# Fabri000/Maze-Solving-Agent-Gymnasium

Hardware: AMD Instinct MI355X
Metric: env steps/sec (whole node) + DQN win-rate, 40x40 r-prim mazes (higher is better)
Workload: dtype int32

## Files before the change

include/mazerl.h:

```cpp
#ifndef MAZERL_H
#define MAZERL_H
#include <stdint.h>

#ifdef __cplusplus
extern "C" {
#endif

#define MZ_OK 0
#define MZ_EINVAL (-1)
#define MZ_EINVAL_SHAPE (-2)
#define MZ_EHIP (-3)
#define MZ_ENOMEM (-4)
#define MZ_EALIGN (-5)

#define MZ_MAX_DIM 127
#define MZ_BANK_MAX_DIMS 64
#define MZ_MAX_CANDIDATES 64
#define MZ_WINDOW 15
#define MZ_WINDOW_BITS 675
#define MZ_WINDOW_WORDS 22

#define MZ_ALGO_RPRIM 0
#define MZ_ALGO_DFS 1
#define MZ_ALGO_PRIMKILL 2

typedef struct mz_handle mz_handle;

typedef struct {
  int32_t num_envs;
  int32_t max_dim;
  int32_t toroidal;
  int32_t enrich;
  int32_t device;
  int32_t reserved[7];
} mz_config;

typedef struct {
  float* reward;
  double* reward64;
  uint8_t* terminated;
  uint8_t* truncated;
  int32_t* pos;
  int32_t* best_dir;
  float* obs6;
  uint32_t* window_bits;
  float* window;
  int32_t* done_idx;
  int32_t* done_count;
} mz_step_out;

typedef struct {
  int32_t n, start_r, start_c, goal_r, goal_c, max_steps;
  int32_t r, c, steps, invalid_streak, nmoves, last_action, done;
} mz_env_info;

const char* mz_last_error(void);
int mz_device_count(int* n);

int mz_create(const mz_config* cfg, mz_handle** out);
int mz_destroy(mz_handle* h);

int mz_load_mazes(mz_handle* h, const uint8_t* grids_host, int32_t dim,
                  const int32_t* start_goal_host, const int32_t* env_ids_host, int32_t n,
                  void* stream);

int mz_generate(mz_handle* h, const int32_t* env_ids_dev, int32_t n, const uint8_t* algo_dev,
                int32_t algo_all, int32_t dim, uint64_t seed, void* stream);

int mz_generate_best(mz_handle* h, const int32_t* env_ids_dev, int32_t n, const uint8_t* algo_dev,
                     int32_t algo_all, int32_t dim, uint64_t seed, int32_t candidates,
                     void* stream);
int mz_select_stats(mz_handle* h, int32_t* out3_dev, int32_t reset, void* stream);
#define MZ_SELECT_STATS 5
int mz_select_stats_ex(mz_handle* h, int32_t* out_dev, int32_t n, int32_t reset, void* stream);
int mz_set_debug(mz_handle* h, int32_t flags);
int mz_set_regen_dims(mz_handle* h, const uint8_t* dims_dev);

#define MZ_RNG_PHILOX 0
#define MZ_RNG_CPYTHON 1
int mz_generate_ex(mz_handle* h, const int32_t* env_ids_dev, int32_t n, const uint8_t* algo_dev,
                   int32_t algo_all, int32_t dim, uint64_t seed, int32_t rng, void* stream);

int mz_generate_state(mz_handle* h, int32_t env, int32_t dim, int32_t algo, uint32_t* state_host,
                      void* stream);

int mz_reset_all(mz_handle* h, const mz_step_out* out, void* stream);
int mz_reset_list(mz_handle* h, const int32_t* idx_dev, const int32_t* count_dev,
                  int32_t max_count, int32_t regen_won, uint64_t seed, uint32_t epoch,
                  const mz_step_out* out, void* stream);

int mz_reset_done(mz_handle* h, int32_t regen_won, uint64_t seed, uint32_t epoch,
                  const mz_step_out* out, void* stream);

int mz_step(mz_handle* h, const int32_t* actions_dev, const mz_step_out* out, void* stream);

#define MZ_STEP_COUNT_ZEROED 1
#define MZ_STEP_AUTORESET 2
int mz_step_ex(mz_handle* h, const int32_t* actions_dev, const mz_step_out* out, int32_t flags,
               void* stream);

int mz_step_act(mz_handle* h, const float* eps_dev, float eps_all, const int64_t* greedy_dev,
                uint64_t seed, uint64_t counter, int32_t* actions_out_dev, const mz_step_out* out,
                int32_t flags, void* stream);

int mz_direction_mask(mz_handle* h, int32_t probs, float* out4_dev, void* stream);

int mz_act(mz_handle* h, const float* eps_dev, float eps_all, const int64_t* greedy_dev,
           uint64_t seed, uint64_t counter, int32_t* actions_dev, void* stream);

int mz_expand_window(const uint32_t* bits_dev, float* out_dev, int32_t n, void* stream);

int mz_bank_create(mz_handle* h, int32_t slots, int32_t dim, uint32_t algo_mask);
int mz_bank_create_dims(mz_handle* h, int32_t slots, const int32_t* dims, int32_t ndims,
                        uint32_t algo_mask);
int mz_bank_create_ex(mz_handle* h, int32_t slots, const int32_t* dims, int32_t ndims,
                      uint32_t algo_mask, int32_t candidates);
int mz_bank_fill(mz_handle* h, int32_t bank, uint64_t seed, void* stream);
int mz_bank_slot_grid(mz_handle* h, int32_t bank, int32_t algo, int32_t size_index, int32_t slot,
                      uint8_t* grid_host, int32_t* info4_host);
int mz_bank_use(mz_handle* h, int32_t bank);
int mz_bank_consumed(mz_handle* h, int32_t bank, int32_t* out3_dev, void* stream);

#define MZ_STATE_HEADER_BYTES 256
int mz_state_bytes(mz_handle* h, uint64_t* bytes_out);
int mz_state_save(mz_handle* h, void* dst_dev, uint64_t bytes, void* stream);
int mz_state_load(mz_handle* h, const void* src_dev, uint64_t bytes, void* stream);

int mz_q_front(const uint32_t* bits_dev, const float* obs6_dev, int32_t n, const float* conv_w_dev,
               const float* conv_b_dev, float drop_p, uint64_t seed, uint64_t counter,
               uint16_t* feat_dev, int32_t ld, void* stream);

int mz_q_front_rows(const uint32_t* bits_dev, const float* obs6_dev, const int32_t* rows_dev,
                    const int32_t* count_dev, int32_t n, const float* conv_w_dev,
                    const float* conv_b_dev, float drop_p, uint64_t seed, uint64_t counter,
                    uint16_t* feat_dev, int32_t ld, void* stream);

int mz_greedy_rows(const float* eps_dev, float eps_all, uint64_t seed, uint64_t counter, int32_t n,
                   int32_t* scratch_dev, int32_t* rows_dev, int32_t* count_dev,
                   int32_t* count_host, void* stream);

int mz_stem_forward(const uint32_t* bits_dev, const float* obs6_dev, int32_t n,
                    const float* conv_w_dev, const float* conv_b_dev, float drop_p,
                    const uint64_t* rng_dev, uint32_t salt, float* feat_dev, int32_t ld,
                    uint8_t* code_dev, void* stream);
int mz_stem_backward(const uint32_t* bits_dev, const uint8_t* code_dev, const float* gfeat_dev,
                     int32_t ld, int32_t n, float drop_p, float* partial_dev, float* dw_dev,
                     float* db_dev, void* stream);
int mz_stem_backward_ex(const uint32_t* bits_dev, const uint8_t* code_dev, const float* gfeat_dev,
                        int32_t ld, int32_t n, float drop_p, float* partial_dev, float* dw_dev,
                        float* db_dev, uint64_t* rng_advance_dev, void* stream);
int mz_stem_workspace_floats(int32_t n);

int mz_leaky_relu_bf16(uint16_t* x_dev, int64_t n, float slope, void* stream);

int mz_colsum_f32(const float* g_dev, int32_t n, int32_t m, int32_t ld, float* out_dev,
                  void* stream);

int mz_replay_gather(const int64_t* idx_dev, int32_t b, int64_t capacity,
                     const float* s6_dev, const int32_t* sw_dev, const int64_t* a_dev,
                     const float* r_dev, const float* s6n_dev, const int32_t* swn_dev,
                     float* out_s6_dev,
                     int32_t* out_sw_dev, int64_t* out_a_dev, float* out_r_dev, void* stream);

int mz_pair_surrogate(const float* lp_new_dev, const float* lp_old_dev, const float* adv_dev,
                      int32_t b, float clip, float* part_dev, float* dsum_dev, void* stream);

int mz_adamw_flat(float* param_dev, float* exp_avg_dev, float* exp_avg_sq_dev,
                  const float* const* grads_dev, const int64_t* seg_len, int32_t nseg,
                  const float* lr_dev, float* step_dev, double beta1, double beta2, double eps,
                  double weight_decay, float clamp, float grad_scale, int32_t write_grad,
                  void* stream);

int mz_set_algorithm(mz_handle* h, const uint8_t* algo_dev, int32_t algo_all, void* stream);

int mz_get_meta(mz_handle* h, int32_t* meta_dev, void* stream);

int mz_discounted_returns(const double* rew_dev, int32_t ld, const int32_t* rows_dev,
                          const int32_t* lens_dev, int32_t n, double gamma, float* out_dev,
                          int32_t ldo, void* stream);

int mz_difficulty(const uint8_t* grid_host, int32_t h, int32_t w, int32_t sr, int32_t sc,
                  int32_t gr, int32_t gc, double* out_host);

int mz_maze_complexity(const uint8_t* grid_host, int32_t h, int32_t w, int32_t sr, int32_t sc,
                       int32_t gr, int32_t gc, double* difficulty_out, double* complexity_out);

int mz_difficulty_batch(mz_handle* h, const int32_t* env_ids_dev, int32_t n, double* out_dev,
                        int32_t* status_dev, void* stream);
int mz_screen_batch(mz_handle* h, const int32_t* env_ids_dev, int32_t n, double* out_dev,
                    int32_t* status_dev, void* stream);

int mz_maze_metrics(mz_handle* h, const int32_t* env_ids_dev, int32_t n, double* out_dev,
                    void* stream);

int mz_query(mz_handle* h, int32_t env, mz_env_info* info_host);
int mz_get_grid(mz_handle* h, int32_t env, uint8_t* grid_host );

int mz_host_alloc(uint64_t bytes, int32_t device, void** host_out, void** dev_out);
int mz_host_free(void* host);


int mz_trainer_tick(const uint8_t* term_dev, const uint8_t* trunc_dev, float* steps_done_dev,
                    double eps_start, double eps_final, double eps_decay, float* eps_out_dev,
                    int64_t* wins_dev, int64_t* episodes_dev, uint64_t seed, uint64_t counter,
                    int32_t n, int32_t* scratch_dev, int32_t* rows_dev, int32_t* count_dev,
                    void* stream);

int mz_greedy_scatter(const uint16_t* q_dev, int32_t ldq, const int32_t* rows_dev,
                      const int32_t* count_dev, int32_t m, int64_t* greedy_dev, void* stream);

int mz_head_bf16(const float* w0, const float* b0, const float* w1, const float* b1,
                 const float* w2, const float* b2, int32_t out0, int32_t in0, int32_t out1,
                 int32_t in1, int32_t out2, int32_t in2, int32_t ld0, int32_t conv_out,
                 int32_t conv_ch, uint16_t* dw0, uint16_t* db0, uint16_t* dw1, uint16_t* db1,
                 uint16_t* dw2, uint16_t* db2, void* stream);

int mz_replay_push(int32_t n, int64_t capacity, int64_t ptr, const float* obs6_src,
                   const int32_t* bits_src, const int32_t* act_src, const float* rew_src,
                   const float* obs6n_src, const int32_t* bitsn_src, float* s6_dev,
                   int32_t* sw_dev, int64_t* a_dev, float* r_dev, float* s6n_dev,
                   int32_t* swn_dev, int32_t obs_dim, int32_t window_words, void* stream);

int mz_replay_sample_idx(uint64_t seed, uint64_t counter, int64_t newest, int64_t n_avail,
                         int64_t capacity, int64_t* out_dev, int32_t n, void* stream);

int mz_q_loss(const float* q_dev, int32_t ldq, const float* q_next_dev, int32_t ldn,
              const float* q_tgt_dev, int32_t ldt, const int64_t* action_dev,
              const float* reward_dev, double gamma, int32_t b, float* loss_dev, float* diff_dev,
              void* stream);

int mz_q_loss_backward(const float* grad_dev, const float* diff_dev, const int64_t* action_dev,
                       int32_t b, int32_t rows, float* dq_dev, void* stream);

int mz_head_loss_workspace_floats(int32_t b);
int mz_head_loss(const float* z2s_dev, int32_t lds, const float* w3s_dev, const float* b3s_dev,
                 const float* z2t_dev, int32_t ldt, const float* w3t_dev, const float* b3t_dev,
                 int32_t hidden, int32_t act, int32_t stacked, const int64_t* action_dev,
                 const float* reward_dev, double gamma, int32_t b, float* part_dev,
                 uint32_t* ticket_dev, float* loss_dev, float* diff_dev, void* stream);

int mz_head_loss_backward_workspace_floats(int32_t b, int32_t hidden);
int mz_head_loss_backward(const float* grad_dev, const float* diff_dev, const int64_t* action_dev,
                          int32_t b, const float* z2s_dev, int32_t lds, const float* w3s_dev,
                          int32_t hidden, int32_t act, float* dz2_dev, int32_t ldd,
                          float* part_dev, void* stream);

int mz_adamw_groups(float* param_dev, float* exp_avg_dev, float* exp_avg_sq_dev,
                    const float* const* grads_dev, const int64_t* seg_len,
                    const int32_t* seg_group, int32_t nseg, const float* lr_dev, float* step_dev,
                    double beta1, double beta2, double eps, double weight_decay, float max_norm,
                    float* scratch_dev, void* stream);


int mz_ppo_act(const float* logits_dev, int32_t ldl, const float* value_dev, int32_t ldv,
               const float* obs6_dev, const uint32_t* bits_dev, int32_t B, int32_t L, uint64_t seed,
               uint64_t counter, const int32_t* t_dev, float* rec_s6_dev, uint32_t* rec_w_dev,
               int64_t* rec_a_dev, float* rec_lp_dev, float* rec_v_dev, int32_t* act_out_dev,
               void* stream);

int mz_ppo_scan(const double* reward64_dev, const uint8_t* term_dev, const uint8_t* trunc_dev,
                int32_t B, int32_t L, int32_t* t_dev, double* rec_r_dev, int32_t* fin_id_dev,
                int64_t* fin_off_dev, int32_t* fin_len_dev, int32_t* fin_count_dev,
                int64_t* pool_fill_dev, int64_t* pool_total_dev, int64_t* stats_dev,
                void* stream);

int mz_ppo_finish(const double* rec_r_dev, const float* rec_s6_dev, const uint32_t* rec_w_dev,
                  const int64_t* rec_a_dev, const float* rec_lp_dev, const float* rec_v_dev,
                  int32_t B, int32_t L, const int32_t* fin_id_dev, const int64_t* fin_off_dev,
                  const int32_t* fin_len_dev, const int32_t* fin_count_dev, double gamma,
                  int64_t capacity, float* pool_s6_dev, uint32_t* pool_w_dev, int64_t* pool_a_dev,
                  float* pool_lp_dev, float* pool_adv_dev, float* pool_ret_dev, void* stream);

int mz_ppo_head_loss(const float* logits_dev, int32_t ldl, const float* value_dev, int32_t ldv,
                     const int64_t* action_dev, const float* lp_old_dev, const float* adv_dev,
                     const float* ret_dev, const float* coef_dev, int32_t b, float clip,
                     float* scratch_dev, float* loss_dev, float* dlogits_dev, int32_t ldg,
                     float* dvalue_dev, int32_t ldvg, void* stream);


int mz_rf_act(const float* logits_dev, int32_t ldl, float temperature, const float* obs6_dev,
              const uint32_t* bits_dev, int32_t B, int32_t L, uint64_t seed, uint64_t counter,
              const int32_t* t_dev, float* rec_s6_dev, uint32_t* rec_w_dev, int64_t* rec_a_dev,
              int32_t* act_out_dev, void* stream);

int mz_rf_finish(const double* rec_r_dev, const float* rec_s6_dev, const uint32_t* rec_w_dev,
                 const int64_t* rec_a_dev, int32_t B, int32_t L, const int32_t* fin_id_dev,
                 const int64_t* fin_off_dev, const int32_t* fin_len_dev,
                 const int32_t* fin_count_dev, double gamma, int64_t capacity, float* pool_s6_dev,
                 uint32_t* pool_w_dev, int64_t* pool_a_dev, float* pool_adv_dev,
                 int32_t* pool_len_dev, int32_t* episodes_dev, void* stream);

int mz_rf_head_loss(const float* logits_dev, int32_t ldl, const int64_t* action_dev,
                    const float* adv_dev, const int32_t* len_dev, const int32_t* episodes_dev,
                    int32_t b, float temperature, float entropy_coef, float* loss_dev,
                    float* dlogits_dev, int32_t ldg, void* stream);


int mz_drqn_act(const float* const* params_dev, int32_t hidden, const float* obs6_dev, int32_t B,
                int32_t L, float epsilon, int32_t explore_actions, uint64_t seed, uint64_t counter,
                const int32_t* t_dev, float* h_dev, float* c_dev, float* rec_x_dev,
                int32_t* rec_a_dev, int32_t* act_out_dev, float* q_out_dev, void* stream);

int mz_drqn_store(const float* obs6_dev, const uint8_t* term_dev, int32_t B, int32_t L,
                  const int32_t* fin_id_dev, const int32_t* fin_len_dev,
                  const int32_t* fin_count_dev, float* rec_x_dev, const int32_t* rec_a_dev,
                  const double* rec_r_dev, int64_t capacity, uint32_t* mem_dev,
                  int32_t* mem_len_dev, int32_t* mem_term_dev, int64_t* ring_dev, void* stream);

int mz_drqn_sample(uint64_t seed, uint64_t counter, int32_t E, int32_t L, int64_t capacity,
                   int64_t filled, const int64_t* ring_dev, const int32_t* mem_len_dev,
                   int32_t* dir_slot_dev, int32_t* dir_len_dev, int64_t* dir_off_dev,
                   int64_t* dir_tot_dev, void* stream);

int mz_drqn_seq_forward(const float* const* params_dev, int32_t hidden, int32_t target, int32_t E,
                        int32_t L, int64_t capacity, float gamma, const uint32_t* mem_dev,
                        const int32_t* mem_term_dev, const int32_t* dir_slot_dev,
                        const int32_t* dir_len_dev, const int64_t* dir_off_dev,
                        const int64_t* dir_tot_dev, float* qmax_dev, float* stash_dev,
                        float* qa_dev, float* y_dev, float* d_dev, double* ep_loss_dev,
                        void* stream);

int mz_drqn_seq_backward(const float* const* params_dev, int32_t hidden, int32_t E, int32_t L,
                         int64_t capacity, const uint32_t* mem_dev, const int32_t* dir_slot_dev,
                         const int32_t* dir_len_dev, const int64_t* dir_off_dev,
                         const int64_t* dir_tot_dev, const float* stash_dev, const float* d_dev,
                         const double* ep_loss_dev, float* gpart_dev, float* const* grads_dev,
                         float* loss_dev, void* stream);


int mz_qact_prepare(const float* fc1_w_dev, const float* fc2_w_dev, uint16_t* w1_hi_dev,
                    uint16_t* w1_lo_dev, uint16_t* w2_hi_dev, uint16_t* w2_lo_dev, void* stream);

int64_t mz_qact_workspace_floats(int32_t n);
int mz_qact(const uint32_t* bits_dev, const float* obs6_dev, const int32_t* rows_dev,
            const int32_t* count_dev, int32_t n, const float* conv_w_dev, const float* conv_b_dev,
            const uint16_t* w1_hi_dev, const uint16_t* w1_lo_dev, const float* b1_dev,
            const uint16_t* w2_hi_dev, const uint16_t* w2_lo_dev, const float* b2_dev,
            const float* w3_dev, const float* b3_dev, int32_t relu, float drop_p, uint64_t seed,
            uint64_t counter, float* h1_dev, int64_t* greedy_dev, float* q_out_dev, void* stream);


int mz_qtab_states(int32_t max_dim, int64_t* rows);

int mz_qtab_act(const float* obs6_dev, int32_t n, int32_t max_dim, const int32_t* table_of_dev,
                int32_t ntables, const uint8_t* active_dev, const double* q_dev,
                int64_t* steps_done_dev, const double* eps_init_dev, const double* eps_final_dev,
                const double* eps_decay_dev, uint64_t seed, uint64_t counter, int32_t* actions_dev,
                int64_t* sidx_dev, void* stream);

int mz_qtab_update(const float* obs6_dev, int32_t n, int32_t max_dim, const int32_t* table_of_dev,
                   int32_t ntables, double* q_dev, const int64_t* sidx_dev,
                   const int32_t* actions_dev, const double* reward64_dev,
                   const uint8_t* terminated_dev, const uint8_t* truncated_dev, double* gamma_dev,
                   const double* lr_dev, const double* eta_dev, double* cum_dev,
                   int64_t* episodes_dev, int64_t* wins_dev, double* td_dev, int32_t episode_end,
                   void* stream);


int mz_qtab_hash_act(const float* obs6_dev, int32_t n, int32_t max_dim,
                     const int32_t* table_of_dev, int32_t ntables, const uint8_t* active_dev,
                     const int32_t* keys_dev, const double* vals_dev, int64_t capacity,
                     int64_t* steps_done_dev, const double* eps_init_dev,
                     const double* eps_final_dev, const double* eps_decay_dev, uint64_t seed,
                     uint64_t counter, int32_t* actions_dev, int64_t* sidx_dev, void* stream);

int mz_qtab_hash_update(const float* obs6_dev, int32_t n, int32_t max_dim,
                        const int32_t* table_of_dev, int32_t ntables, int32_t* keys_dev,
                        double* vals_dev, int64_t capacity, int32_t* load_dev,
                        int64_t* overflow_dev, const int64_t* sidx_dev, const int32_t* actions_dev,
                        const double* reward64_dev, const uint8_t* terminated_dev,
                        const uint8_t* truncated_dev, double* gamma_dev, const double* lr_dev,
                        const double* eta_dev, double* cum_dev, int64_t* episodes_dev,
                        int64_t* wins_dev, double* td_dev, int32_t episode_end, void* stream);

// ... 80 lines not shown
```

maze-solving-agent-gymnasium_amd/csrc/mz_api.hip:

```cpp
#include <algorithm>
#include <cmath>
#include <cstdarg>
#include <cstdio>
#include <cstdlib>
#include <cstring>
#include <string>
#include <vector>

#include "../../include/mazerl.h"
#include "mz_archive.h"
#include "mz_common.h"
#include "mz_learner.h"
#include "mz_mcclendon.h"

struct MzHostFallback {
  int cap = 0, gstride = 0;
  uint8_t *grid_h = nullptr, *grid_d = nullptr;
  int32_t *info_h = nullptr, *info_d = nullptr;
  double *prod_h = nullptr, *prod_d = nullptr;
  int32_t *ok_h = nullptr, *ok_d = nullptr;
  int32_t* count_h = nullptr;
  int* count_d = nullptr;
  int32_t* map = nullptr;
};
// ... 735 lines not shown
  }
  b.epoch[bank] += 1;
  return MZ_OK;
}

int mz_bank_use(mz_handle* h, int32_t bank) {
  if (!h) return fail(MZ_EINVAL, "null handle");
  MzDev& d = h->d;
  if (bank < 0) {
    d.bk_K = 0;
    return MZ_OK;
  }
  const MzBankStore& b = h->bank;
  if (!b.K) return fail(MZ_EINVAL, "no maze bank (mz_bank_create)");
  if (bank > 1) return fail(MZ_EINVAL, "bank %d", bank);
  const size_t blk = (size_t)bank * b.nA * b.nD * b.K, P = (size_t)d.P;
  d.bk_K = b.K;
  d.bk_nd = b.nD;
  for (int i = 0; i < 128; ++i) d.bk_didx[i] = -1;
  for (int i = 0; i < b.nD; ++i) d.bk_didx[b.dims[i]] = (int8_t)i;
  d.bk_amask = b.amask;
  d.bk_cells = b.cells + blk * P * P;
  d.bk_planes = b.planes + blk * d.PW;
  d.bk_meta0 = b.meta0 + blk;
  d.bk_meta1 = b.meta1 + blk;
  d.bk_head = b.heads + 3 * bank * b.nD;
  d.bk_slot = b.slot;
  d.bk_code = b.code;
  d.bk_G = (d.B + 63) / 64;
  return MZ_OK;
}

int mz_bank_slot_grid(mz_handle* h, int32_t bank, int32_t algo, int32_t size_index, int32_t slot,
                      uint8_t* grid_host, int32_t* info4_host) {
  if (!h || !h->bank.K || !grid_host || !info4_host) return fail(MZ_EINVAL, "bad arguments");
  const MzBankStore& b = h->bank;
  if (bank < 0 || bank > 1 || algo < 0 || algo > 2 || !((b.amask >> algo) & 1u) ||
      size_index < 0 || size_index >= b.nD || slot < 0 || slot >= b.K)
    return fail(MZ_EINVAL, "no such bank slot");
  DeviceGuard g(h->cfg.device);
  MZ_HIP(hipDeviceSynchronize());
  const size_t P = (size_t)h->d.P;
  const size_t i = (((size_t)bank * b.nA + mz_bank_aidx(b.amask, algo)) * b.nD + size_index) * b.K + slot;
  uint32_t m0, m1;
  MZ_HIP(hipMemcpy(&m0, b.meta0 + i, 4, hipMemcpyDeviceToHost));
  MZ_HIP(hipMemcpy(&m1, b.meta1 + i, 4, hipMemcpyDeviceToHost));
  std::vector<uint32_t> cw(P * P);
  MZ_HIP(hipMemcpy(cw.data(), b.cells + i * P * P, 4 * cw.size(), hipMemcpyDeviceToHost));
  const int N = m0 & 0xFF, gr = m1 & 0xFF, gc = (m1 >> 8) & 0xFF;
  if (N < 5 || N > (int)P) return fail(MZ_EINVAL, "bank slot not built");
  for (int r = 0; r < N; ++r)
    for (int c = 0; c < N; ++c) {
      const bool open = (cw[(size_t)r * P + c] & MZ_CELL_OPEN) != 0;
      grid_host[r * N + c] = !open ? 0 : ((r == gr && c == gc) ? 2 : 1);
    }
  info4_host[0] = (m0 >> 16) & 0xFF;
  info4_host[1] = m0 >> 24;
  info4_host[2] = gr;
  info4_host[3] = gc;
  return MZ_OK;
}

int mz_set_regen_dims(mz_handle* h, const uint8_t* dims_dev) {
  if (!h) return fail(MZ_EINVAL, "null handle");
  h->d.regen_dim = dims_dev;
  return MZ_OK;
}

int mz_generate_best(mz_handle* h, const int32_t* env_ids_dev, int32_t n, const uint8_t* algo_dev,
                     int32_t algo_all, int32_t dim, uint64_t seed, int32_t candidates,
                     void* stream) {
  if (!h) return fail(MZ_EINVAL, "null handle");
  if (candidates < 1 || candidates > MZ_MAX_CANDIDATES)
    return fail(MZ_EINVAL, "candidates %d outside [1, %d]", candidates, MZ_MAX_CANDIDATES);
  if (candidates == 1)
    return mz_generate_ex(h, env_ids_dev, n, algo_dev, algo_all, dim, seed, MZ_RNG_PHILOX, stream);
  if (!env_ids_dev) n = h->d.B;
  if (n < 0 || n > h->d.B) return fail(MZ_EINVAL, "n out of range");
  if (!algo_dev && (algo_all < 0 || algo_all > 2)) return fail(MZ_EINVAL, "algorithm id %d", algo_all);
  int rc = check_dim(h, dim);
  if (rc) return rc;
  int mm = 0;
  if (mz_mcclendon_lds(h->d.P, h->d.toroidal != 0, &mm) > 160 * 1024)
    return fail(MZ_EINVAL_SHAPE, "best-of-%d generation scores with the difficulty kernel: maze "
                "pitch %d beyond its LDS plan", candidates, h->d.P);
  if (n == 0) return MZ_OK;
  DeviceGuard g(h->cfg.device);
  hipStream_t s = static_cast<hipStream_t>(stream);
  const int chunk = std::max(1, std::min(n, 49152 / candidates));
  if (h->gen.cap < chunk * candidates) {
    if (h->gen.cap) MZ_HIP(hipStreamSynchronize(s));
    if ((rc = cand_alloc(h, h->gen, chunk * candidates))) return rc;
  }
  for (int j0 = 0; j0 < n; j0 += chunk) {
    const int m = std::min(chunk, n - j0);
    const int32_t* ids = env_ids_dev ? env_ids_dev + j0 : nullptr;
    const uint8_t* al = algo_dev ? algo_dev + j0 : nullptr;
    if ((rc = bestof_run(h, h->gen, h->d, ids, j0, nullptr, m, candidates, al, algo_all, dim, seed,
                         0u, s)))
      return rc;
  }
  return MZ_OK;
}

int mz_select_stats(mz_handle* h, int32_t* out3_dev, int32_t reset, void* stream) {
  return mz_select_stats_ex(h, out3_dev, 3, reset, stream);
}

int mz_select_stats_ex(mz_handle* h, int32_t* out_dev, int32_t n, int32_t reset, void* stream) {
  if (!h || n < 0 || n > MZ_SELECT_STATS) return fail(MZ_EINVAL, "bad arguments");
  DeviceGuard g(h->cfg.device);
  hipStream_t s = static_cast<hipStream_t>(stream);
  if (out_dev && n) MZ_HIP(hipMemcpyAsync(out_dev, h->sel_stats, n * sizeof(int32_t), hipMemcpyDeviceToDevice, s));
  if (reset) MZ_HIP(hipMemsetAsync(h->sel_stats, 0, 8 * sizeof(int32_t), s));
  return MZ_OK;
}

int mz_set_debug(mz_handle* h, int32_t flags) {
  if (!h) return fail(MZ_EINVAL, "null handle");
  if (flags & ~7) return fail(MZ_EINVAL, "debug flags %d", flags);
  h->dbg = flags;
  return MZ_OK;
}

int mz_screen_batch(mz_handle* h, const int32_t* env_ids_dev, int32_t n, double* out_dev,
                    int32_t* status_dev, void* stream) {
  if (!h || !out_dev || !status_dev) return fail(MZ_EINVAL, "bad arguments");
  if (h->d.toroidal) return fail(MZ_EINVAL, "the screen scores euclidean mazes");
  if (!env_ids_dev) n = h->d.B;
  if (n < 0 || (!env_ids_dev && n > h->d.B)) return fail(MZ_EINVAL, "n out of range");
  if (n == 0) return MZ_OK;
  DeviceGuard g(h->cfg.device);
  hipStream_t s = static_cast<hipStream_t>(stream);
  if (h->scr_cap < n) {
    if (h->scr_cap) MZ_HIP(hipStreamSynchronize(s));
    int rc = compact_alloc(h, h->scr, n);
    if (rc) return rc;
    h->scr_cap = n;
  }
  MZ_HIP(mz_launch_compact_from_handle(h->d, env_ids_dev, n, h->scr, s));
  MZ_HIP(mz_launch_screen(h->scr, h->d.P, n, out_dev, status_dev, s));
  return MZ_OK;
}

int mz_bank_consumed(mz_handle* h, int32_t bank, int32_t* out3_dev, void* stream) {
  if (!h || !h->bank.K || !out3_dev || bank < 0 || bank > 1) return fail(MZ_EINVAL, "bad arguments");
  DeviceGuard g(h->cfg.device);
  const int nd = h->bank.nD;
  MZ_HIP(hipMemcpyAsync(out3_dev, h->bank.heads + 3 * bank * nd, 3 * nd * sizeof(int32_t),
                        hipMemcpyDeviceToDevice, static_cast<hipStream_t>(stream)));
  return MZ_OK;
}

}

namespace {

constexpr uint32_t kStateMagic = 0x54535A4Du;
constexpr uint32_t kStateVersion = 1u;
enum : int { SH_MAGIC, SH_VER, SH_B, SH_P, SH_TOR, SH_ENRICH, SH_NS, SH_PW, SH_BK_K, SH_BK_NA,
             SH_BK_ND, SH_BK_AMASK, SH_BK_ACTIVE, SH_BK_EPOCH0, SH_BK_EPOCH1, SH_DIMS = 16 };
static_assert(SH_DIMS * 4 + MZ_BANK_MAX_DIMS <= MZ_STATE_HEADER_BYTES, "header too small");

struct Section {
  void* p;
  size_t bytes;
};

std::vector<Section> state_sections(mz_handle* h) {
  const MzDev& d = h->d;
  const size_t B = (size_t)d.B, P = (size_t)d.P;
  std::vector<Section> s = {
      {d.cells, B * P * P * 4}, {d.planes, (B * (size_t)d.PW + 16) * 4}, {d.meta0, B * 4},
      {d.meta1, B * 4}, {d.posw, B * 4}, {d.stw, B * 4}, {d.curw, B * 4}, {d.algo, B},
      {d.last_term, B}};
  const MzBankStore& b = h->bank;
  if (b.K) {
    const size_t S = 2 * (size_t)b.nA * b.nD * b.K;
    s.push_back({b.cells, S * P * P * 4});
    s.push_back({b.planes, S * (size_t)d.PW * 4});
    s.push_back({b.meta0, S * 4});
    s.push_back({b.meta1, S * 4});
    s.push_back({b.heads, (size_t)6 * b.nD * 4});
  }
  return s;
}

size_t state_size(mz_handle* h) {
  size_t n = MZ_STATE_HEADER_BYTES;
  for (const Section& s : state_sections(h)) n += (s.bytes + 255) & ~(size_t)255;
  return n;
}

int active_bank(const mz_handle* h) {
  const MzDev& d = h->d;
  if (!d.bk_K || !h->bank.K) return -1;
  return d.bk_cells == h->bank.cells ? 0 : 1;
}

}

extern "C" {

int mz_state_bytes(mz_handle* h, uint64_t* bytes_out) {
  if (!h || !bytes_out) return fail(MZ_EINVAL, "bad arguments");
  *bytes_out = state_size(h);
  return MZ_OK;
}

int mz_state_save(mz_handle* h, void* dst_dev, uint64_t bytes, void* stream) {
  if (!h || !dst_dev) return fail(MZ_EINVAL, "bad arguments");
  if (bytes < state_size(h)) return fail(MZ_EINVAL, "state buffer of %llu bytes, %zu needed",
                                         (unsigned long long)bytes, state_size(h));
  DeviceGuard g(h->cfg.device);
  hipStream_t s = static_cast<hipStream_t>(stream);
  const MzDev& d = h->d;
  const MzBankStore& b = h->bank;
  uint32_t hdr[MZ_STATE_HEADER_BYTES / 4] = {};
  hdr[SH_MAGIC] = kStateMagic;
  hdr[SH_VER] = kStateVersion;
  hdr[SH_B] = (uint32_t)d.B;
  hdr[SH_P] = (uint32_t)d.P;
  hdr[SH_TOR] = (uint32_t)d.toroidal;
  hdr[SH_ENRICH] = (uint32_t)d.enrich;
  hdr[SH_NS] = (uint32_t)d.NS;
  hdr[SH_PW] = (uint32_t)d.PW;
  hdr[SH_BK_K] = (uint32_t)b.K;
  hdr[SH_BK_NA] = (uint32_t)b.nA;
  hdr[SH_BK_ND] = (uint32_t)b.nD;
  hdr[SH_BK_AMASK] = b.amask;
  hdr[SH_BK_ACTIVE] = (uint32_t)active_bank(h);
  hdr[SH_BK_EPOCH0] = b.epoch[0];
  hdr[SH_BK_EPOCH1] = b.epoch[1];
  uint8_t* dims = reinterpret_cast<uint8_t*>(hdr + SH_DIMS);
  for (int i = 0; i < b.nD; ++i) dims[i] = (uint8_t)b.dims[i];
  uint8_t* dst = static_cast<uint8_t*>(dst_dev);
  MZ_HIP(hipMemcpyAsync(dst, hdr, sizeof hdr, hipMemcpyHostToDevice, s));
  MZ_HIP(hipStreamSynchronize(s));
  size_t off = MZ_STATE_HEADER_BYTES;
  for (const Section& sec : state_sections(h)) {
    MZ_HIP(hipMemcpyAsync(dst + off, sec.p, sec.bytes, hipMemcpyDeviceToDevice, s));
    off += (sec.bytes + 255) & ~(size_t)255;
  }
  return MZ_OK;
}

int mz_state_load(mz_handle* h, const void* src_dev, uint64_t bytes, void* stream) {
  if (!h || !src_dev) return fail(MZ_EINVAL, "bad arguments");
  if (bytes < MZ_STATE_HEADER_BYTES) return fail(MZ_EINVAL, "state buffer too small");
  DeviceGuard g(h->cfg.device);
  hipStream_t s = static_cast<hipStream_t>(stream);
  uint32_t hdr[MZ_STATE_HEADER_BYTES / 4];
  MZ_HIP(hipMemcpyAsync(hdr, src_dev, sizeof hdr, hipMemcpyDeviceToHost, s));
  MZ_HIP(hipStreamSynchronize(s));
  const MzDev& d = h->d;
  MzBankStore& b = h->bank;
  if (hdr[SH_MAGIC] != kStateMagic || hdr[SH_VER] != kStateVersion)
    return fail(MZ_EINVAL, "not an env state (magic %08x version %u)", hdr[SH_MAGIC], hdr[SH_VER]);
  if (hdr[SH_B] != (uint32_t)d.B || hdr[SH_P] != (uint32_t)d.P ||
      hdr[SH_TOR] != (uint32_t)d.toroidal || hdr[SH_ENRICH] != (uint32_t)d.enrich ||
      hdr[SH_NS] != (uint32_t)d.NS || hdr[SH_PW] != (uint32_t)d.PW)
    return fail(MZ_EINVAL, "env state of %u instances, max_dim %u, toroidal %u, enrich %u does not "
                "fit this handle (%d, %d, %d, %d)", hdr[SH_B], hdr[SH_P], hdr[SH_TOR],
                hdr[SH_ENRICH], d.B, d.P, d.toroidal, d.enrich);
  const uint8_t* dims = reinterpret_cast<const uint8_t*>(hdr + SH_DIMS);
  bool same_bank = hdr[SH_BK_K] == (uint32_t)b.K && hdr[SH_BK_NA] == (uint32_t)b.nA &&
                   hdr[SH_BK_ND] == (uint32_t)b.nD && hdr[SH_BK_AMASK] == b.amask;
  for (int i = 0; same_bank && i < b.nD; ++i) same_bank = dims[i] == (uint8_t)b.dims[i];
  if (!same_bank)
    return fail(MZ_EINVAL, "env state has a maze bank of %u slots x %u algorithms x %u sizes "
                "(mask %u); this handle's is %d x %d x %d (mask %u)", hdr[SH_BK_K], hdr[SH_BK_NA],
                hdr[SH_BK_ND], hdr[SH_BK_AMASK], b.K, b.nA, b.nD, b.amask);
  if (bytes < state_size(h)) return fail(MZ_EINVAL, "state buffer of %llu bytes, %zu needed",
                                         (unsigned long long)bytes, state_size(h));
  const uint8_t* src = static_cast<const uint8_t*>(src_dev);
  size_t off = MZ_STATE_HEADER_BYTES;
  for (const Section& sec : state_sections(h)) {
    MZ_HIP(hipMemcpyAsync(sec.p, src + off, sec.bytes, hipMemcpyDeviceToDevice, s));
    off += (sec.bytes + 255) & ~(size_t)255;
  }
  if (b.K) {
    b.epoch[0] = hdr[SH_BK_EPOCH0];
    b.epoch[1] = hdr[SH_BK_EPOCH1];
  }
  return mz_bank_use(h, (int32_t)hdr[SH_BK_ACTIVE]);
}

int mz_maze_metrics(mz_handle* h, const int32_t* env_ids_dev, int32_t n, double* out_dev,
                    void* stream) {
  if (!h || !out_dev) return fail(MZ_EINVAL, "bad arguments");
  if (h->d.toroidal) return fail(MZ_EINVAL, "maze metrics are defined for euclidean mazes");
  if (!env_ids_dev) n = h->d.B;
  if (n < 0 || n > h->d.B) return fail(MZ_EINVAL, "n out of range");
  DeviceGuard g(h->cfg.device);
  MZ_HIP(mz_launch_metrics(h->d, env_ids_dev, n, out_dev, static_cast<hipStream_t>(stream)));
  return MZ_OK;
}

int mz_difficulty_batch(mz_handle* h, const int32_t* env_ids_dev, int32_t n, double* out_dev,
                        int32_t* status_dev, void* stream) {
  if (!h || !out_dev || !status_dev) return fail(MZ_EINVAL, "bad arguments");
  if (!env_ids_dev) n = h->d.B;
  if (n < 0 || (!env_ids_dev && n > h->d.B)) return fail(MZ_EINVAL, "n out of range");
  int mm = 0;
  if (mz_mcclendon_lds(h->d.P, h->d.toroidal != 0, &mm) > 160 * 1024)
    return fail(MZ_EINVAL_SHAPE, "maze pitch beyond the difficulty kernel's LDS plan");
// ... 7 lines not shown
  if (!h) return fail(MZ_EINVAL, "null handle");
  DeviceGuard g(h->cfg.device);
  hipStream_t s = static_cast<hipStream_t>(stream);
  if (algo_dev) MZ_HIP(hipMemcpyAsync(h->d.algo, algo_dev, h->d.B, hipMemcpyDeviceToDevice, s));
  else {
    if (algo_all < 0 || algo_all > 2) return fail(MZ_EINVAL, "algorithm id %d", algo_all);
    MZ_HIP(hipMemsetAsync(h->d.algo, algo_all, h->d.B, s));
  }
  return MZ_OK;
}

int mz_get_meta(mz_handle* h, int32_t* meta_dev, void* stream) {
  if (!h || !meta_dev) return fail(MZ_EINVAL, "bad arguments");
  DeviceGuard g(h->cfg.device);
  MZ_HIP(mz_launch_meta(h->d, meta_dev, static_cast<hipStream_t>(stream)));
  return MZ_OK;
}

int mz_discounted_returns(const double* rew_dev, int32_t ld, const int32_t* rows_dev,
                          const int32_t* lens_dev, int32_t n, double gamma, float* out_dev,
                          int32_t ldo, void* stream) {
  if (!rew_dev || !rows_dev || !lens_dev || !out_dev || n < 0) return fail(MZ_EINVAL, "bad arguments");
  StreamGuard g(stream);
  MZ_HIP(mz_launch_returns(rew_dev, ld, rows_dev, lens_dev, n, gamma, out_dev, ldo,
                           static_cast<hipStream_t>(stream)));
  return MZ_OK;
}

int mz_query(mz_handle* h, int32_t env, mz_env_info* info) {
  if (!h || !info || env < 0 || env >= h->d.B) return fail(MZ_EINVAL, "bad arguments");
  DeviceGuard g(h->cfg.device);
  MZ_HIP(hipDeviceSynchronize());
  uint32_t m0, m1, pw, sw;
  MZ_HIP(hipMemcpy(&m0, h->d.meta0 + env, 4, hipMemcpyDeviceToHost));
  MZ_HIP(hipMemcpy(&m1, h->d.meta1 + env, 4, hipMemcpyDeviceToHost));
  MZ_HIP(hipMemcpy(&pw, h->d.posw + env, 4, hipMemcpyDeviceToHost));
  MZ_HIP(hipMemcpy(&sw, h->d.stw + env, 4, hipMemcpyDeviceToHost));
  info->n = m0 & 0xFF;
  info->start_r = (m0 >> 16) & 0xFF; info->start_c = m0 >> 24;
  info->goal_r = m1 & 0xFF; info->goal_c = (m1 >> 8) & 0xFF; info->max_steps = m1 >> 16;
  info->r = pw & 0xFF; info->c = (pw >> 8) & 0xFF; info->nmoves = (pw >> 16) & 3;
  info->last_action = (pw >> 18) & 3; info->done = (pw >> 20) & 1;
  info->steps = sw & 0xFFFF; info->invalid_streak = (sw >> 16) & 0xFF;
  return MZ_OK;
}

int mz_get_grid(mz_handle* h, int32_t env, uint8_t* grid_host) {
  if (!h || !grid_host || env < 0 || env >= h->d.B) return fail(MZ_EINVAL, "bad arguments");
  mz_env_info info;
  int rc = mz_query(h, env, &info);
  if (rc) return rc;
  const int P = h->d.P, N = info.n;
  std::vector<uint32_t> cw((size_t)P * P);
  DeviceGuard g(h->cfg.device);
  MZ_HIP(hipMemcpy(cw.data(), h->d.cells + (size_t)env * P * P, 4 * cw.size(), hipMemcpyDeviceToHost));
  for (int r = 0; r < N; ++r)
    for (int c = 0; c < N; ++c) {
      const bool open = (cw[(size_t)r * P + c] & MZ_CELL_OPEN) != 0;
      grid_host[r * N + c] = !open ? 0 : ((r == info.goal_r && c == info.goal_c) ? 2 : 1);
    }
  return MZ_OK;
}

int mz_host_alloc(uint64_t bytes, int32_t device, void** host_out, void** dev_out) {
  if (!host_out || !dev_out || bytes == 0) return fail(MZ_EINVAL, "bad arguments");
  int ndev = 0;
  MZ_HIP(hipGetDeviceCount(&ndev));
  if (device < 0 || device >= ndev) return fail(MZ_EINVAL, "device %d not present", device);
  DeviceGuard g(device);
  void* hp = nullptr;
  MZ_HIP(hipHostMalloc(&hp, (size_t)bytes, hipHostMallocMapped | hipHostMallocCoherent));
  void* dp = nullptr;
  const hipError_t e = hipHostGetDevicePointer(&dp, hp, 0);
  if (e != hipSuccess) {
    (void)hipHostFree(hp);
    return fail(MZ_EHIP, "hipHostGetDevicePointer: %s", hipGetErrorString(e));
  }
  std::memset(hp, 0, (size_t)bytes);
  *host_out = hp;
  *dev_out = dp;
  return MZ_OK;
}

int mz_host_free(void* host) {
  if (!host) return MZ_OK;
  MZ_HIP(hipHostFree(host));
  return MZ_OK;
}

}


int mz_trainer_tick(const uint8_t* term_dev, const uint8_t* trunc_dev, float* steps_done_dev,
                    double eps_start, double eps_final, double eps_decay, float* eps_out_dev,
                    int64_t* wins_dev, int64_t* episodes_dev, uint64_t seed, uint64_t counter,
                    int32_t n, int32_t* scratch_dev, int32_t* rows_dev, int32_t* count_dev,
                    void* stream) {
  if (n < 0 || (n > 0 && (!term_dev || !trunc_dev || !steps_done_dev || !eps_out_dev ||
                          !scratch_dev || !rows_dev || !count_dev)))
    return fail(MZ_EINVAL, "bad arguments");
  if (!(eps_decay > 0.0)) return fail(MZ_EINVAL, "eps_decay %g", eps_decay);
  const float inv_decay = 1.0f / (float)eps_decay;
  MZ_HIP(mz_launch_tick(term_dev, trunc_dev, steps_done_dev, (float)eps_final,
                        (float)(eps_start - eps_final), inv_decay, eps_out_dev,
                        reinterpret_cast<unsigned long long*>(wins_dev),
                        reinterpret_cast<unsigned long long*>(episodes_dev), seed, counter, n,
                        scratch_dev, rows_dev, count_dev, static_cast<hipStream_t>(stream)));
  return MZ_OK;
}

int mz_greedy_scatter(const uint16_t* q_dev, int32_t ldq, const int32_t* rows_dev,
                      const int32_t* count_dev, int32_t m, int64_t* greedy_dev, void* stream) {
  if (m < 0 || ldq < 4 || (m > 0 && (!q_dev || !rows_dev || !count_dev || !greedy_dev)))
    return fail(MZ_EINVAL, "bad arguments");
  MZ_HIP(mz_launch_greedy_scatter(q_dev, ldq, rows_dev, count_dev, m, greedy_dev,
                                  static_cast<hipStream_t>(stream)));
  return MZ_OK;
}

int mz_head_bf16(const float* w0, const float* b0, const float* w1, const float* b1,
                 const float* w2, const float* b2, int32_t out0, int32_t in0, int32_t out1,
                 int32_t in1, int32_t out2, int32_t in2, int32_t ld0, int32_t conv_out,
                 int32_t conv_ch, uint16_t* dw0, uint16_t* db0, uint16_t* dw1, uint16_t* db1,
                 uint16_t* dw2, uint16_t* db2, void* stream) {
  if (!w0 || !b0 || !w1 || !b1 || !w2 || !b2 || !dw0 || !db0 || !dw1 || !db1 || !dw2 || !db2)
    return fail(MZ_EINVAL, "bad arguments");
  if (out0 <= 0 || out1 <= 0 || out2 <= 0 || in1 != out0 || in2 != out1 || in0 > ld0 ||
      conv_ch <= 0 || conv_out < 0 || conv_out > in0 || conv_out % conv_ch != 0 || in0 > 2048)
    return fail(MZ_EINVAL, "head shapes");
  MzHeadBf16 h{{w0, w1, w2}, {b0, b1, b2}, {dw0, dw1, dw2}, {db0, db1, db2},
               {out0, out1, out2}, {in0, in1, in2}, ld0, conv_out, conv_ch};
  MZ_HIP(mz_launch_head_bf16(h, static_cast<hipStream_t>(stream)));
  return MZ_OK;
}

int mz_replay_push(int32_t n, int64_t capacity, int64_t ptr, const float* obs6_src,
                   const int32_t* bits_src, const int32_t* act_src, const float* rew_src,
                   const float* obs6n_src, const int32_t* bitsn_src, float* s6_dev,
                   int32_t* sw_dev, int64_t* a_dev, float* r_dev, float* s6n_dev,
                   int32_t* swn_dev, int32_t obs_dim, int32_t window_words, void* stream) {
  if (n < 0 || n > capacity || ptr < 0 || ptr >= capacity || obs_dim <= 0 || window_words <= 0)
    return fail(MZ_EINVAL, "bad arguments");
  const void* src[6] = {obs6_src, bits_src, act_src, rew_src, obs6n_src, bitsn_src};
  void* dst[6] = {s6_dev, sw_dev, a_dev, r_dev, s6n_dev, swn_dev};
  for (int j = 0; j < 6; ++j)
    if (src[j] && !dst[j]) return fail(MZ_EINVAL, "replay array %d missing", j);
  MzReplayPush p{{src[0], src[1], src[2], src[3], src[4], src[5]},
                 {dst[0], dst[1], dst[2], dst[3], dst[4], dst[5]},
                 {obs_dim, window_words, 1, 1, obs_dim, window_words}, n, capacity, ptr};
  MZ_HIP(mz_launch_replay_push(p, static_cast<hipStream_t>(stream)));
  return MZ_OK;
}

int mz_replay_sample_idx(uint64_t seed, uint64_t counter, int64_t newest, int64_t n_avail,
                         int64_t capacity, int64_t* out_dev, int32_t n, void* stream) {
  if (n < 0 || capacity <= 0 || n_avail <= 0 || n_avail > capacity || (n > 0 && !out_dev))
    return fail(MZ_EINVAL, "bad arguments");
  MZ_HIP(mz_launch_replay_idx(seed, counter, newest, n_avail, capacity, out_dev, n,
                              static_cast<hipStream_t>(stream)));
  return MZ_OK;
}

int mz_q_loss(const float* q_dev, int32_t ldq, const float* q_next_dev, int32_t ldn,
              const float* q_tgt_dev, int32_t ldt, const int64_t* action_dev,
              const float* reward_dev, double gamma, int32_t b, float* loss_dev, float* diff_dev,
              void* stream) {
  if (b <= 0 || !q_dev || !q_tgt_dev || !action_dev || !reward_dev || !loss_dev || !diff_dev ||
      ldq < 4 || ldt < 4 || (q_next_dev && ldn < 4))
    return fail(MZ_EINVAL, "bad arguments");
  MZ_HIP(mz_launch_q_loss(q_dev, ldq, q_next_dev, ldn, q_tgt_dev, ldt, action_dev, reward_dev,
                          (float)gamma, b, loss_dev, diff_dev, static_cast<hipStream_t>(stream)));
  return MZ_OK;
}

int mz_q_loss_backward(const float* grad_dev, const float* diff_dev, const int64_t* action_dev,
                       int32_t b, int32_t rows, float* dq_dev, void* stream) {
  if (b <= 0 || rows < b || !grad_dev || !diff_dev || !action_dev || !dq_dev)
    return fail(MZ_EINVAL, "bad arguments");
  const float norm = (float)(2.0 / (double)b);
  MZ_HIP(mz_launch_q_loss_bwd(grad_dev, diff_dev, action_dev, b, rows, norm, dq_dev,
                              static_cast<hipStream_t>(stream)));
  return MZ_OK;
}

int mz_head_loss_workspace_floats(int32_t b) {
  return b <= 0 ? 0 : mz_head_loss_blocks(b);
}

int mz_head_loss(const float* z2s_dev, int32_t lds, const float* w3s_dev, const float* b3s_dev,
                 const float* z2t_dev, int32_t ldt, const float* w3t_dev, const float* b3t_dev,
                 int32_t hidden, int32_t act, int32_t stacked, const int64_t* action_dev,
                 const float* reward_dev, double gamma, int32_t b, float* part_dev,
                 uint32_t* ticket_dev, float* loss_dev, float* diff_dev, void* stream) {
  if (b <= 0 || hidden <= 0 || hidden % 4 || (act != 0 && act != 1) || !z2s_dev || !w3s_dev ||
      !b3s_dev || !z2t_dev || !w3t_dev || !b3t_dev || !action_dev || !reward_dev || !part_dev ||
      !loss_dev || !diff_dev || lds < hidden || ldt < hidden)
    return fail(MZ_EINVAL, "bad arguments");
  MzHeadLoss p{z2s_dev, w3s_dev, b3s_dev, z2t_dev, w3t_dev, b3t_dev, lds, ldt, stacked ? 1 : 0, b,
               hidden, act, action_dev, reward_dev, (float)gamma, part_dev, ticket_dev, loss_dev,
               diff_dev};
  MZ_HIP(mz_launch_head_loss(p, static_cast<hipStream_t>(stream)));
  return MZ_OK;
}

int mz_head_loss_backward_workspace_floats(int32_t b, int32_t hidden) {
  return b <= 0 ? 0 : mz_head_loss_bwd_blocks(b) * (4 * hidden + 4);
}

int mz_head_loss_backward(const float* grad_dev, const float* diff_dev, const int64_t* action_dev,
                          int32_t b, const float* z2s_dev, int32_t lds, const float* w3s_dev,
                          int32_t hidden, int32_t act, float* dz2_dev, int32_t ldd,
                          float* part_dev, void* stream) {
  if (b <= 0 || hidden <= 0 || hidden % 4 || (act != 0 && act != 1) || !grad_dev || !diff_dev ||
      !action_dev || !z2s_dev || !w3s_dev || !dz2_dev || !part_dev || lds < hidden || ldd < hidden)
    return fail(MZ_EINVAL, "bad arguments");
  const float norm = (float)(2.0 / (double)b);
  MZ_HIP(mz_launch_head_loss_bwd(grad_dev, diff_dev, action_dev, b, norm, z2s_dev, lds, w3s_dev,
                                 hidden, act, dz2_dev, ldd, part_dev,
                                 static_cast<hipStream_t>(stream)));
  return MZ_OK;
}

int mz_adamw_groups(float* param_dev, float* exp_avg_dev, float* exp_avg_sq_dev,
                    const float* const* grads_dev, const int64_t* seg_len,
                    const int32_t* seg_group, int32_t nseg, const float* lr_dev, float* step_dev,
                    double beta1, double beta2, double eps, double weight_decay, float max_norm,
                    float* scratch_dev, void* stream) {
  if (!param_dev || !exp_avg_dev || !exp_avg_sq_dev || !grads_dev || !seg_len || !seg_group ||
      !lr_dev || !step_dev || !scratch_dev)
    return fail(MZ_EINVAL, "bad arguments");
  if (nseg < 1 || nseg > MZ_OPT_MAX_SEGS) return fail(MZ_EINVAL, "segment count %d", nseg);
  const uintptr_t al = reinterpret_cast<uintptr_t>(param_dev) |
                       reinterpret_cast<uintptr_t>(exp_avg_dev) |
                       reinterpret_cast<uintptr_t>(exp_avg_sq_dev);
  if (al & 15) return fail(MZ_EALIGN, "flat buffers must be 16-byte aligned");
  for (int k = 0; k < nseg; ++k) {
    if (!grads_dev[k] || seg_len[k] <= 0 || (seg_len[k] & 3))
      return fail(MZ_EINVAL, "segment %d: length %lld (multiple of 4 required)", k,
                  (long long)seg_len[k]);
    if (reinterpret_cast<uintptr_t>(grads_dev[k]) & 15)
      return fail(MZ_EALIGN, "gradient %d must be 16-byte aligned", k);
    if (seg_group[k] < 0) return fail(MZ_EINVAL, "segment %d: group %d", k, seg_group[k]);
  }
  MZ_HIP(mz_launch_adamw_groups(param_dev, exp_avg_dev, exp_avg_sq_dev, grads_dev, seg_len,
                                seg_group, nseg, lr_dev, step_dev, beta1, beta2, eps,
                                weight_decay, max_norm, scratch_dev,
                                static_cast<hipStream_t>(stream)));
  return MZ_OK;
}

int mz_ppo_act(const float* logits_dev, int32_t ldl, const float* value_dev, int32_t ldv,
               const float* obs6_dev, const uint32_t* bits_dev, int32_t B, int32_t L, uint64_t seed,
               uint64_t counter, const int32_t* t_dev, float* rec_s6_dev, uint32_t* rec_w_dev,
               int64_t* rec_a_dev, float* rec_lp_dev, float* rec_v_dev, int32_t* act_out_dev,
               void* stream) {
  if (!logits_dev || !value_dev || !obs6_dev || !bits_dev || !t_dev || !rec_s6_dev || !rec_w_dev ||
      !rec_a_dev || !rec_lp_dev || !rec_v_dev || !act_out_dev || B < 0 || L < 1 || ldl < 4 ||
      ldv < 1)
    return fail(MZ_EINVAL, "bad arguments");
  StreamGuard g(stream);
  MzPpoAct q{logits_dev, ldl, value_dev, ldv, obs6_dev, bits_dev, B, L, seed, counter, t_dev,
             rec_s6_dev, rec_w_dev, rec_a_dev, rec_lp_dev, rec_v_dev, act_out_dev};
  MZ_HIP(mz_launch_ppo_act(q, static_cast<hipStream_t>(stream)));
  return MZ_OK;
}

int mz_ppo_scan(const double* reward64_dev, const uint8_t* term_dev, const uint8_t* trunc_dev,
                int32_t B, int32_t L, int32_t* t_dev, double* rec_r_dev, int32_t* fin_id_dev,
                int64_t* fin_off_dev, int32_t* fin_len_dev, int32_t* fin_count_dev,
                int64_t* pool_fill_dev, int64_t* pool_total_dev, int64_t* stats_dev,
                void* stream) {
  if (!reward64_dev || !term_dev || !trunc_dev || !t_dev || !rec_r_dev || !fin_id_dev ||
      !fin_off_dev || !fin_len_dev || !fin_count_dev || !pool_fill_dev || !pool_total_dev ||
      !stats_dev || B < 0 || L < 1)
    return fail(MZ_EINVAL, "bad arguments");
  StreamGuard g(stream);
  MzPpoScan q{reward64_dev, term_dev, trunc_dev, B, L, t_dev, rec_r_dev, fin_id_dev, fin_off_dev,
              fin_len_dev, fin_count_dev, pool_fill_dev, pool_total_dev,
              reinterpret_cast<long long*>(stats_dev)};
  MZ_HIP(mz_launch_ppo_scan(q, static_cast<hipStream_t>(stream)));
  return MZ_OK;
}

int mz_ppo_finish(const double* rec_r_dev, const float* rec_s6_dev, const uint32_t* rec_w_dev,
                  const int64_t* rec_a_dev, const float* rec_lp_dev, const float* rec_v_dev,
                  int32_t B, int32_t L, const int32_t* fin_id_dev, const int64_t* fin_off_dev,
                  const int32_t* fin_len_dev, const int32_t* fin_count_dev, double gamma,
                  int64_t capacity, float* pool_s6_dev, uint32_t* pool_w_dev, int64_t* pool_a_dev,
                  float* pool_lp_dev, float* pool_adv_dev, float* pool_ret_dev, void* stream) {
  if (!rec_r_dev || !rec_s6_dev || !rec_w_dev || !rec_a_dev || !rec_lp_dev || !rec_v_dev ||
      !fin_id_dev || !fin_off_dev || !fin_len_dev || !fin_count_dev || !pool_s6_dev ||
      !pool_w_dev || !pool_a_dev || !pool_lp_dev || !pool_adv_dev || !pool_ret_dev || B < 0 ||
      L < 1 || capacity < 0)
    return fail(MZ_EINVAL, "bad arguments");
  StreamGuard g(stream);
  MzPpoFinish q{rec_r_dev, rec_s6_dev, rec_w_dev, rec_a_dev, rec_lp_dev, rec_v_dev, L, fin_id_dev,
                fin_off_dev, fin_len_dev, fin_count_dev, gamma, capacity, pool_s6_dev, pool_w_dev,
                pool_a_dev, pool_lp_dev, pool_adv_dev, pool_ret_dev};
  MZ_HIP(mz_launch_ppo_finish(q, B, static_cast<hipStream_t>(stream)));
  return MZ_OK;
}

int mz_ppo_head_loss(const float* logits_dev, int32_t ldl, const float* value_dev, int32_t ldv,
                     const int64_t* action_dev, const float* lp_old_dev, const float* adv_dev,
                     const float* ret_dev, const float* coef_dev, int32_t b, float clip,
                     float* scratch_dev, float* loss_dev, float* dlogits_dev, int32_t ldg,
// ... 577 lines not shown
```

maze-solving-agent-gymnasium_amd/csrc/mz_env.hip:

```cpp
#include "mz_common.h"
#include "mz_kernels.h"
#include "mz_build.inc.h"

#include "../../include/mazerl.h"

#define WAVE 64
#ifndef MZ_IPW
#define MZ_IPW 16
#endif
#define IPW MZ_IPW
#ifndef MZ_SPW
#define MZ_SPW 1
#endif
#ifndef MZ_PROBE
#define MZ_PROBE 0
#endif
__host__ __device__ constexpr int cat_words(int ipw) { return ipw * 675 / 32 + 2; }

namespace {

__device__ inline uint32_t wrap_colmask(int col, int C0, int N) {
  uint32_t m = 0;
  for (int j = mz_wrapn(col - C0, N); j < 15; j += N) m |= 1u << j;
  return m;
// ... 755 lines not shown
  const int lane = threadIdx.x;
  for (int t = blockIdx.x; t < used * C; t += gridDim.x) {
    const bool decl = status[t] != 0 || ((dbg & MZ_DBG_DECLINE_EVEN) && ((t % C) & 1) == 0);
    if (!decl) {
      if (lane == 0) hmap[t] = -1;
      continue;
    }
    int slot = 0;
    if (lane == 0) slot = atomicAdd(hcount, 1);
    slot = __shfl(slot, 0);
    if (lane == 0) hmap[t] = slot < hcap ? slot : -1;
    if (slot >= hcap) continue;
    const bool tor = cd.toroidal;
    const int P = cd.P, o = tor ? 1 : 0;
    const uint32_t m0 = cd.meta0[t], m1 = cd.meta1[t];
    const int Nm = m0 & 0xFF, N = tor ? Nm + 2 : Nm;
    const int gr = (m1 & 0xFF) + o, gc = ((m1 >> 8) & 0xFF) + o;
    const uint32_t* cw = cd.cells + (size_t)t * P * P;
    uint8_t* g = hgrid + (size_t)slot * gstride;
    for (int q = lane; q < N * N; q += WAVE) {
      const int r = q / N, c = q - r * N;
      const bool in = r >= o && r < o + Nm && c >= o && c < o + Nm;
      const bool op = in && (cw[(r - o) * P + (c - o)] & MZ_CELL_OPEN);
      g[q] = !op ? 0 : ((r == gr && c == gc) ? 2 : 1);
    }
    if (lane == 0) {
      int32_t* in = hinfo + 5 * (size_t)slot;
      in[0] = N;
      in[1] = (int)((m0 >> 16) & 0xFF) + o;
      in[2] = (int)(m0 >> 24) + o;
      in[3] = gr;
      in[4] = gc;
    }
  }
}

__global__ __launch_bounds__(WAVE) void k_compact_from_handle(MzDev d, const int32_t* ids, int n,
                                                              MzCompact cc) {
  const int lane = threadIdx.x;
  for (int i = blockIdx.x; i < n; i += gridDim.x) {
    const int e = ids ? ids[i] : i;
    const uint32_t m0 = d.meta0[e], m1 = d.meta1[e];
    const int N = m0 & 0xFF, sr = (m0 >> 16) & 0xFF, sc = m0 >> 24, gr = m1 & 0xFF, gc = (m1 >> 8) & 0xFF;
    const int W = (N - 1) / 2, Q = W * W, P = d.P;
    const uint32_t* cw = d.cells + (size_t)e * P * P;
    auto open = [&](int r, int c) { return r >= 0 && c >= 0 && r < N && c < N && (cw[r * P + c] & MZ_CELL_OPEN); };
    bool lattice = !d.toroidal && (N & 1) && N < 128 && (sr & 1) && (sc & 1) && (gr & 1) && (gc & 1);
    uint8_t* gp = cc.pas + (size_t)i * cc.Qp;
    uint16_t* ga = cc.dist + (size_t)i * cc.Qp;
    uint32_t* gs = cc.sol + (size_t)i * cc.QWp;
    for (int q = lane; q < Q && lattice; q += WAVE) {
      const int r = 2 * (q / W) + 1, c = 2 * (q % W) + 1;
      gp[q] = (uint8_t)((open(r, c + 1) && c + 2 < N ? 1 : 0) | (open(r + 1, c) && r + 2 < N ? 2 : 0));
      ga[q] = (uint16_t)(cw[r * P + c] & MZ_CELL_D_MASK);
    }
    for (int k = lane; k < cc.QWp; k += WAVE) gs[k] = 0u;
    __syncthreads();
    if (lane == 0 && lattice) {
      int r = sr, c = sc;
      for (int it = 0; it <= N * N; ++it) {
        if ((r & 1) && (c & 1)) {
          const int q = (r >> 1) * W + (c >> 1);
          gs[q >> 5] |= 1u << (q & 31);
        }
        if (r == gr && c == gc) break;
        const int D = (int)(cw[r * P + c] & MZ_CELL_D_MASK);
        int nr = -1, nc = -1;
        for (int k = 0; k < 4; ++k) {
          const int rr = r + mz_dr(k), cc2 = c + mz_dc(k);
          if (open(rr, cc2) && (int)(cw[rr * P + cc2] & MZ_CELL_D_MASK) == D - 1) { nr = rr; nc = cc2; }
        }
        if (nr < 0) { lattice = false; break; }
        r = nr;
        c = nc;
      }
    }
    lattice = __shfl((int)lattice, 0) != 0;
    if (lane == 0)
      cc.meta[i] = (uint32_t)(N & 0x7F) | (lattice ? 0u : MZ_CMETA_NOSOL) |
                   ((uint32_t)((sr >> 1) * W + (sc >> 1)) << 8) | ((uint32_t)((gr >> 1) * W + (gc >> 1)) << 20);
    __syncthreads();
  }
}

__global__ __launch_bounds__(WAVE) void k_cand_select(MzDev cd, MzDev dst, const int32_t* dst_ids,
                                                      int base, const int* count, int n, int C,
                                                      const double* score, const int32_t* status,
                                                      int* stats, const int32_t* xlist,
                                                      const int32_t* hmap, const double* hprod,
                                                      const int32_t* hok, int hcap,
                                                      int count_groups, int dbg) {
  const int used = count ? min(*count, n) : n;
  const int lane = threadIdx.x;
  for (int j = blockIdx.x; j < used; j += gridDim.x) {
    const int t0 = j * C;
    bool ok = false, host = false;
    double p = 0.0;
    if (lane < C) {
      const int t = t0 + lane;
      const bool decl = status[t] != 0 || ((dbg & MZ_DBG_DECLINE_EVEN) && (lane & 1) == 0);
      if (!decl) {
        ok = true;
        p = score[2 * t];
      } else if (hmap) {
        const int h = hmap[t];
        if (h >= 0 && h < hcap && hok[h]) {
          ok = host = true;
          p = hprod[h];
        }
      }
    }
    const unsigned long long okm = __ballot(ok);
    const unsigned long long hostm = __ballot(host);
    int pick = 0;
    double best = 0.0;
    bool have = false;
    for (int c = 0; c < C; ++c) {
      if (!((okm >> c) & 1ull)) continue;
      const double pc = __shfl(p, c);
      if (!have || pc < best) { best = pc; pick = c; have = true; }
    }
    const bool near = ok && lane < pick && p != best && p <= best * (1.0 + 0x1p-40);
    const unsigned long long nearm = __ballot(near);
    if (lane == 0) {
      if (okm != ((C >= 64) ? ~0ull : ((1ull << C) - 1ull))) atomicAdd(stats + 0, 1);
      if (nearm) atomicAdd(stats + 1, 1);
      if (hostm) atomicAdd(stats + 4, __popcll(hostm));
      if (count_groups) atomicAdd(stats + 2, 1);
    }
    const size_t src = (size_t)(t0 + pick);
    const int jd = xlist ? xlist[j] : j;
    const size_t de = (size_t)(dst_ids ? dst_ids[jd] : base + jd);
    const size_t pp = (size_t)cd.P * cd.P, pw = (size_t)cd.PW;
    wave_copy(dst.cells + de * pp, cd.cells + src * pp, pp);
    wave_copy(dst.planes + de * pw, cd.planes + src * pw, pw);
    if (lane == 0) {
      dst.meta0[de] = cd.meta0[src];
      dst.meta1[de] = cd.meta1[src];
      dst.posw[de] = cd.posw[src];
      dst.stw[de] = cd.stw[src];
      dst.curw[de] = cd.curw[src];
      dst.last_term[de] = cd.last_term[src];
      dst.algo[de] = cd.algo[src];
    }
  }
}

__device__ __noinline__ void reset_build_cold(MzDev d, int e, bool tor, uint64_t seed, uint8_t* lds) {
  mz_build_one(d, e, tor, true, d.algo[e], seed, mz_regen_dim(d, e), nullptr, 0, 0, 0, 0, lds);
}

template <bool TOR, bool ENRICH>
__global__ __launch_bounds__(WAVE) void k_reset_done(MzDev d, int regen, uint64_t seed,
                                                     uint32_t epoch, MzOut o, int split) {
  extern __shared__ __align__(16) uint8_t lds[];
  __shared__ __align__(16) uint32_t wsh[32];
  const int grp = blockIdx.x / split, part = blockIdx.x - grp * split;
  const int lane = threadIdx.x, e = grp * WAVE + lane;
  const bool done = e < d.B && ((d.posw[e] >> 20) & 1u);
  bool win = regen && done && d.last_term[e] && mz_regen_dim(d, e) != 0;
  int cls = -1, slot = 0;
  if (regen && d.bk_K) {
    const int code = e < d.B ? (int)d.bk_code[e] : -2;
    win = code != -2;
    cls = code;
    if (cls < 0) cls = -1;
    unsigned long long pend = __ballot(cls >= 0);
    while (pend) {
      const int cj = __shfl(cls, __ffsll((long long)pend) - 1);
      const unsigned long long m = __ballot(cls == cj);
      if (cls == cj) slot = d.bk_slot[cj * d.bk_G + grp] + __popcll(m & ((1ull << lane) - 1ull));
      pend &= ~m;
    }
  }
  const int SH = WAVE / split;
  const unsigned long long share = (~0ull >> (WAVE - SH)) << (part * SH);
  unsigned long long bal = __ballot(done) & share;
  while (bal) {
    const int j = __ffsll((long long)bal) - 1;
    bal &= bal - 1;
    const int ej = grp * WAVE + j;
    const int cj = __shfl(cls, j), sj = __shfl(slot, j);
    uint2 meta;
    bool have_meta = false;
    if (__shfl((int)win, j)) {
      have_meta = bank_take(d, ej, cj, sj, meta);
      if (!have_meta)
        reset_build_cold(d, ej, TOR, seed + (uint64_t)ej + ((uint64_t)epoch << 32), lds);
      __syncthreads();
    }
    reset_one<TOR, ENRICH>(d, ej, o, wsh, have_meta ? &meta : nullptr);
    __syncthreads();
  }
}

__global__ __launch_bounds__(WAVE) void k_build(MzDev d, const int32_t* env_ids, int32_t n,
                                                int generate, const uint8_t* algo_list,
                                                int32_t algo_all, int32_t dim, uint64_t seed,
                                                const uint8_t* grids, const int32_t* sg,
                                                int pymode, uint32_t* py_state) {
  extern __shared__ __align__(16) uint8_t lds[];
  for (int j = blockIdx.x; j < n; j += gridDim.x) {
    const int e = env_ids ? env_ids[j] : j;
    if (generate) {
      const int algo = algo_list ? algo_list[j] : algo_all;
      if (threadIdx.x == 0) d.algo[e] = (uint8_t)algo;
      mz_build_one(d, e, d.toroidal, true, algo, seed + (uint64_t)e, dim, nullptr, 0, 0, 0, 0, lds,
                   pymode, py_state, d.ticket + MZ_TICKET_PYERR);
    } else {
      mz_build_one(d, e, d.toroidal, false, 0, 0, dim, grids + (size_t)j * dim * dim,
                   sg[4 * j], sg[4 * j + 1], sg[4 * j + 2], sg[4 * j + 3], lds);
    }
    __syncthreads();
  }
}

__global__ __launch_bounds__(WAVE) void k_regen_list(MzDev d, const int32_t* idx,
                                                     const int32_t* count, int32_t n_static,
                                                     uint64_t seed, uint32_t epoch) {
  extern __shared__ __align__(16) uint8_t lds[];
  const int n = count ? min(*count, n_static) : n_static;
  for (int j = blockIdx.x; j < n; j += gridDim.x) {
    const int e = idx ? idx[j] : j;
    const int dim = mz_regen_dim(d, e);
    if (!d.last_term[e] || dim == 0) continue;
    mz_build_one(d, e, d.toroidal, true, d.algo[e], seed + (uint64_t)e + ((uint64_t)epoch << 32),
                 dim, nullptr, 0, 0, 0, 0, lds);
    __syncthreads();
  }
}

__global__ void k_mask(MzDev d, int probs, float* out4) {
  const int e = blockIdx.x * blockDim.x + threadIdx.x;
  if (e >= d.B) return;
  float m[4];
  dir_mask(d.posw[e], d.curw[e], d.toroidal, probs, m);
  reinterpret_cast<float4*>(out4)[e] = make_float4(m[0], m[1], m[2], m[3]);
}

constexpr int GR_BLOCK = MZ_GR_BLOCK;
__device__ inline bool greedy_needed(const MzAct& ap, int e) {
  uint32_t u[4];
  act_u(ap, e, u);
  return act_greedy(u, ap.eps ? ap.eps[e] : ap.eps_all);
}

__global__ __launch_bounds__(GR_BLOCK) void k_greedy_count(MzAct ap, int n, int32_t* blk) {
  const int e = blockIdx.x * GR_BLOCK + threadIdx.x;
  const int c = __syncthreads_count(e < n && greedy_needed(ap, e));
  if (threadIdx.x == 0) blk[blockIdx.x] = c;
}

__global__ __launch_bounds__(GR_BLOCK) void k_greedy_list(MzAct ap, int n,
                                                          const int32_t* __restrict__ blk,
                                                          int32_t* rows, int32_t* count,
                                                          int32_t* count_host) {
  __shared__ int wsum[GR_BLOCK / WAVE];
  __shared__ int base;
  const int lane = threadIdx.x & (WAVE - 1), w = threadIdx.x / WAVE;
  const int e = blockIdx.x * GR_BLOCK + threadIdx.x;
  const bool need = e < n && greedy_needed(ap, e);
  const unsigned long long bal = __ballot(need);
  if (lane == 0) wsum[w] = __popcll(bal);
  if (w == 0) {
    int pre = 0, tot = 0;
    for (int i = lane; i < (int)gridDim.x; i += WAVE) {
      const int v = blk[i];
      pre += i < (int)blockIdx.x ? v : 0;
      tot += v;
    }
    for (int o = WAVE / 2; o; o >>= 1) {
      pre += __shfl_xor(pre, o);
      tot += __shfl_xor(tot, o);
    }
    if (lane == 0) {
      base = pre;
      if (blockIdx.x == 0) {
        *count = tot;
        if (count_host) *count_host = tot;
      }
    }
  }
  __syncthreads();
  int off = base;
  for (int i = 0; i < w; ++i) off += wsum[i];
  if (need) rows[off + __popcll(bal & ((1ull << lane) - 1ull))] = e;
}

__global__ void k_act(MzDev d, MzAct ap) {
  const int e = blockIdx.x * blockDim.x + threadIdx.x;
  if (e >= d.B) return;
  ap.act_out[e] = act_sample(ap, e, d.posw[e], d.curw[e], d.toroidal);
}

__global__ void k_expand(const uint32_t* bits, float* out, int n) {
  const long t = (long)blockIdx.x * blockDim.x + threadIdx.x;
  const long total = (long)n * 675;
  if (t >= total) return;
  const long i = t / 675, f = t - i * 675;
  out[t] = (float)((bits[i * MZ_WINDOW_WORDS + (f >> 5)] >> (f & 31)) & 1u);
}

__global__ void k_meta(MzDev d, int32_t* out) {
  const int e = blockIdx.x * blockDim.x + threadIdx.x;
  if (e >= d.B) return;
  const uint32_t m0 = d.meta0[e], m1 = d.meta1[e];
  int32_t* o = out + 6 * (size_t)e;
  o[0] = m0 & 0xFF; o[1] = (m0 >> 16) & 0xFF; o[2] = m0 >> 24;
  o[3] = m1 & 0xFF; o[4] = (m1 >> 8) & 0xFF; o[5] = m1 >> 16;
}

__global__ void k_returns(const double* rew, int ld, const int32_t* rows, const int32_t* lens,
                          int n, double gamma, float* out, int ldo) {
  const int k = blockIdx.x * blockDim.x + threadIdx.x;
  if (k >= n) return;
  const double* r = rew + (size_t)rows[k] * ld;
  float* o = out + (size_t)k * ldo;
  double acc = 0.0;
  for (int t = lens[k] - 1; t >= 0; --t) {
    acc = __dadd_rn(r[t], __dmul_rn(acc, gamma));
    o[t] = (float)acc;
  }
}

hipError_t mz_lds_attr(const void* fn, size_t bytes) {
  if (bytes <= 65536) return hipSuccess;
  return hipFuncSetAttribute(fn, hipFuncAttributeMaxDynamicSharedMemorySize, (int)bytes);
}

#ifndef MZ_LITE
#define MZ_LITE 1
#endif
#ifndef MZ_LITE_DFS
#define MZ_LITE_DFS 1
#endif

#ifndef MZ_PACK_DFS
#define MZ_PACK_DFS 1
#endif
#ifndef MZ_BANK_WGS
#define MZ_BANK_WGS 0
#endif
#ifndef MZ_LITE_WGS
#define MZ_LITE_WGS 1280
#endif
#ifndef MZ_EXPAND_WGS
#define MZ_EXPAND_WGS 0
#endif
size_t mz_build_lds_launch(int P, bool tor, bool generate, int pymode) {
  if (MZ_CELL_BUILD && generate && pymode == MZ_PY_PHILOX)
    return tor ? mz_torus_lds_bytes(P) : mz_cell_lds_bytes(P);
  return mz_build_lds_bytes_mode(P, generate ? pymode : 0);
}
int mz_build_grid(int n, size_t lds) {
  const int per_cu = (int)std::min<size_t>(32, std::max<size_t>(1, (160 * 1024) / std::max<size_t>(lds, 1)));
  return std::max(1, std::min(n, std::max(4096, 256 * per_cu)));
}

}

size_t mz_build_lds_size(int P) { return mz_build_lds_bytes(P); }
size_t mz_import_lds(int P, bool tor) { return mz_build_lds_launch(P, tor, false, MZ_PY_PHILOX); }
hipError_t mz_build_lds_attr(const void* fn, size_t bytes) { return mz_lds_attr(fn, bytes); }
int mz_build_launch_grid(int n, size_t lds) { return mz_build_grid(n, lds); }

hipError_t mz_launch_build(const MzDev& d, const int32_t* env_ids, int32_t n, bool generate,
                           const uint8_t* algo_list, int32_t algo_all, int32_t dim, uint64_t seed,
                           const uint8_t* grids, const int32_t* start_goal, int pymode,
                           uint32_t* py_state, hipStream_t s) {
  if (n <= 0) return hipSuccess;
  const size_t lds = mz_build_lds_launch(d.P, d.toroidal, generate, pymode);
  hipError_t ae = mz_lds_attr(reinterpret_cast<const void*>(k_build), lds);
  if (ae != hipSuccess) return ae;
  hipLaunchKernelGGL(k_build, dim3(mz_build_grid(n, lds)), dim3(WAVE), lds, s, d, env_ids, n,
                     (int)generate, algo_list, algo_all, dim, seed, grids, start_goal, pymode,
                     py_state);
  return hipGetLastError();
}

hipError_t mz_launch_regen(const MzDev& d, const int32_t* idx, const int32_t* count,
                           int32_t n_static, uint64_t seed, uint32_t epoch, hipStream_t s) {
  if (n_static <= 0) return hipSuccess;
  const size_t lds = mz_build_lds_launch(d.P, d.toroidal, true, MZ_PY_PHILOX);
  hipError_t ae = mz_lds_attr(reinterpret_cast<const void*>(k_regen_list), lds);
  if (ae != hipSuccess) return ae;
  hipLaunchKernelGGL(k_regen_list, dim3(mz_build_grid(n_static, lds)), dim3(WAVE), lds, s, d, idx,
                     count, n_static, seed, epoch);
  return hipGetLastError();
}

#ifndef MZ_SMALL_B
#define MZ_SMALL_B 16384
#endif
template <int I, bool T, bool E>
void launch_step_ite(const MzDev& d, const int32_t* act, const MzAct& a, bool has_act, bool ar,
                     const MzOut& o, hipStream_t s) {
  dim3 grid((d.B + I * MZ_SPW - 1) / (I * MZ_SPW)), block(WAVE * MZ_SPW);
  if (has_act) {
    if (ar) hipLaunchKernelGGL((k_step<I, T, E, true, true>), grid, block, 0, s, d, act, a, o);
    else hipLaunchKernelGGL((k_step<I, T, E, true, false>), grid, block, 0, s, d, act, a, o);
  } else {
    if (ar) hipLaunchKernelGGL((k_step<I, T, E, false, true>), grid, block, 0, s, d, act, a, o);
    else hipLaunchKernelGGL((k_step<I, T, E, false, false>), grid, block, 0, s, d, act, a, o);
  }
}

template <bool T, bool E>
void launch_step_te(const MzDev& d, const int32_t* act, const MzAct& a, bool has_act, bool ar,
                    const MzOut& o, hipStream_t s) {
  if (d.B <= MZ_SMALL_B) launch_step_ite<4, T, E>(d, act, a, has_act, ar, o, s);
  else launch_step_ite<IPW, T, E>(d, act, a, has_act, ar, o, s);
}

hipError_t mz_launch_step(const MzDev& d, const int32_t* act, const MzAct* ap, bool autoreset,
                          const MzOut& o0, hipStream_t s) {
  MzAct a{};
  if (ap) a = *ap;
  MzOut o = o0;
  o.window_nt = o.window && (size_t)d.B * 675 * sizeof(float) > MZ_WINDOW_NT_BYTES;
  if (d.toroidal) {
    if (d.enrich) launch_step_te<true, true>(d, act, a, ap != nullptr, autoreset, o, s);
    else launch_step_te<true, false>(d, act, a, ap != nullptr, autoreset, o, s);
  } else {
    if (d.enrich) launch_step_te<false, true>(d, act, a, ap != nullptr, autoreset, o, s);
    else launch_step_te<false, false>(d, act, a, ap != nullptr, autoreset, o, s);
  }
  return hipGetLastError();
}

hipError_t mz_launch_reset_list(const MzDev& d, const int32_t* idx, int32_t* count,
                                int32_t n_static, const MzOut& o, hipStream_t s) {
  if (n_static <= 0) return hipSuccess;
  const int blocks = n_static < 1024 ? n_static : 1024;
#define MZ_RL(T, E) \
  hipLaunchKernelGGL((k_reset_list<T, E>), dim3(blocks), dim3(WAVE), 0, s, d, idx, count, n_static, o)
  if (d.toroidal) { if (d.enrich) MZ_RL(true, true); else MZ_RL(true, false); }
  else { if (d.enrich) MZ_RL(false, true); else MZ_RL(false, false); }
#undef MZ_RL
  hipError_t e = hipGetLastError();
  if (e == hipSuccess && count) e = hipMemsetAsync(count, 0, sizeof(int32_t), s);
  return e;
}

hipError_t mz_launch_reset_done(const MzDev& d, int regen, uint64_t seed, uint32_t epoch,
                                const MzOut& o, hipStream_t s) {
  const int groups = (d.B + WAVE - 1) / WAVE;
  int split = 1;
  while (split < WAVE && groups * split < 1024) split <<= 1;
  const int blocks = groups * split;
  size_t lds = 0;
  hipError_t ae = hipSuccess;
  if (regen && d.bk_K) {
    ae = hipMemsetAsync(d.bk_slot, 0, sizeof(int) * 3 * (size_t)d.bk_nd * d.bk_G, s);
    if (ae != hipSuccess) return ae;
    hipLaunchKernelGGL(k_bank_count, dim3(d.bk_G), dim3(WAVE), 0, s, d);
    hipLaunchKernelGGL(k_bank_scan, dim3(3 * d.bk_nd), dim3(BS_T), 0, s, d);
  }
#define MZ_RD(T, E)                                                                           \
  do {                                                                                        \
    if (regen) {                                                                              \
      lds = mz_build_lds_launch(d.P, d.toroidal, true, MZ_PY_PHILOX);                         \
      ae = mz_lds_attr(reinterpret_cast<const void*>(k_reset_done<T, E>), lds);              \
      if (ae != hipSuccess) return ae;                                                        \
    }                                                                                         \
    hipLaunchKernelGGL((k_reset_done<T, E>), dim3(blocks), dim3(WAVE), lds, s, d, regen, seed, \
                       epoch, o, split);                                                      \
  } while (0)
  if (d.toroidal) { if (d.enrich) MZ_RD(true, true); else MZ_RD(true, false); }
  else { if (d.enrich) MZ_RD(false, true); else MZ_RD(false, false); }
#undef MZ_RD
  return hipGetLastError();
}

hipError_t mz_launch_cand_build(const MzDev& cd, const int32_t* ids, int base, const int* count, int n,
                                int C, const uint8_t* algo_list, int algo_all, int dim,
                                uint64_t seed, uint32_t epoch, hipStream_t s, int dbg) {
  if (n <= 0 || C <= 0) return hipSuccess;
  const bool packed = MZ_PACK > 1 && MZ_CELL_BUILD && !cd.toroidal && !algo_list &&
                      (algo_all == MZ_ALGO_RPRIM_DEV || (MZ_PACK_DFS && algo_all == MZ_ALGO_DFS_DEV));
  const size_t stride = packed ? mz_align16(mz_cell_lds_bytes(cd.P)) : 0;
  const size_t lds = packed ? MZ_PACK * stride : mz_build_lds_launch(cd.P, cd.toroidal, true, MZ_PY_PHILOX);
  const void* kfn = packed ? reinterpret_cast<const void*>(k_cand_build_packed)
                           : reinterpret_cast<const void*>(k_cand_build);
  hipError_t ae = mz_lds_attr(kfn, lds);
  if (ae != hipSuccess) return ae;
  const int total = packed ? (n * C + MZ_PACK - 1) / MZ_PACK : n * C;
  const int grid = std::max(1, MZ_BANK_WGS > 0 ? std::min(total, MZ_BANK_WGS) : mz_build_grid(total, lds));
  if (packed)
    hipLaunchKernelGGL(k_cand_build_packed, dim3(grid), dim3(WAVE), lds, s, cd, ids, base, count, n, C,
                       algo_all, dim, seed, epoch, (int)stride, dbg);
  else
    hipLaunchKernelGGL(k_cand_build, dim3(grid), dim3(WAVE), lds, s, cd, ids, base, count, n, C,
                       algo_list, algo_all, dim, seed, epoch, dbg);
  return hipGetLastError();
}

hipError_t mz_launch_cand_compact(const MzCompact& cc, int P, const int32_t* ids, int base,
                                  const int* count, int n, int C, const uint8_t* algo_list,
                                  int algo_all, int dim, uint64_t seed, uint32_t epoch, hipStream_t s,
                                  int dbg) {
  if (n <= 0 || C <= 0) return hipSuccess;
  if (dim > P || cc.Qp < mz_compact_qp(P)) return hipErrorInvalidValue;
  if (MZ_LITE && !algo_list &&
      (algo_all == MZ_ALGO_RPRIM_DEV || (MZ_LITE_DFS && algo_all == MZ_ALGO_DFS_DEV))) {
    const size_t stride = mz_align16(mz_lite_lds_bytes(P, algo_all) + (MZ_RING ? 4 * 4 * (WAVE / MZ_LPACK) : 0));
    const size_t lds = MZ_LPACK * stride + mz_lite_scratch_bytes(P);
    hipError_t ae = mz_lds_attr(reinterpret_cast<const void*>(k_cand_compact_lite), lds);
    if (ae != hipSuccess) return ae;
    const int total = (n * C + MZ_LPACK - 1) / MZ_LPACK;
    const int cap = MZ_BANK_WGS > 0 ? MZ_BANK_WGS : MZ_LITE_WGS;
    const int grid = std::max(1, cap > 0 ? std::min(total, cap) : mz_build_grid(total, lds));
    hipLaunchKernelGGL(k_cand_compact_lite, dim3(grid), dim3(WAVE), lds, s, cc, P, ids, base, count,
                       n, C, algo_all, dim, seed, epoch, (int)stride, dbg);
    return hipGetLastError();
  }
  const bool packed = MZ_PACK > 1 && !algo_list &&
                      (algo_all == MZ_ALGO_RPRIM_DEV || (MZ_PACK_DFS && algo_all == MZ_ALGO_DFS_DEV));
  const size_t stride = mz_align16(mz_cell_lds_bytes(P));
  const size_t lds = packed ? MZ_PACK * stride : stride;
  const void* kfn = packed ? reinterpret_cast<const void*>(k_cand_compact_packed)
                           : reinterpret_cast<const void*>(k_cand_compact);
  hipError_t ae = mz_lds_attr(kfn, lds);
  if (ae != hipSuccess) return ae;
  const int total = packed ? (n * C + MZ_PACK - 1) / MZ_PACK : n * C;
  const int grid = std::max(1, MZ_BANK_WGS > 0 ? std::min(total, MZ_BANK_WGS) : mz_build_grid(total, lds));
  if (packed)
    hipLaunchKernelGGL(k_cand_compact_packed, dim3(grid), dim3(WAVE), lds, s, cc, P, ids, base, count,
                       n, C, algo_all, dim, seed, epoch, (int)stride, dbg);
  else
    hipLaunchKernelGGL(k_cand_compact, dim3(grid), dim3(WAVE), lds, s, cc, P, ids, base, count, n, C,
                       algo_list, algo_all, dim, seed, epoch, dbg);
  return hipGetLastError();
}

hipError_t mz_launch_cand_pick(const int* count, int n, int C, const double* score,
                               const int32_t* status, int32_t* pick, int32_t* xlist, int* xcount,
                               int xcap, int* stats, hipStream_t s, int dbg) {
  if (n <= 0) return hipSuccess;
  if (C < 1 || C > WAVE) return hipErrorInvalidValue;
  hipLaunchKernelGGL(k_cand_pick, dim3(std::min(n, 4096)), dim3(WAVE), 0, s, count, n, C, score,
                     status, pick, xlist, xcount, xcap, stats, dbg);
  return hipGetLastError();
}

hipError_t mz_launch_cand_expand(const MzCompact& cc, const MzDev& dst, const int32_t* dst_ids,
                                 int base, const int* count, int n, int C, const int32_t* pick,
                                 const uint8_t* algo_list, int algo_all, hipStream_t s) {
  if (n <= 0) return hipSuccess;
  const size_t lds = mz_align16(mz_cell_lds_bytes(dst.P));
  hipError_t ae = mz_lds_attr(reinterpret_cast<const void*>(k_cand_expand), lds);
  if (ae != hipSuccess) return ae;
  const int eg = mz_build_grid(n, lds);
  hipLaunchKernelGGL(k_cand_expand, dim3(std::max(1, MZ_EXPAND_WGS > 0 ? std::min(eg, MZ_EXPAND_WGS) : eg)),
                     dim3(WAVE), lds, s, cc,
                     dst, dst_ids, base, count, n, C, pick, algo_list, algo_all);
  return hipGetLastError();
}

hipError_t mz_launch_cand_rebuild(const MzDev& cd, const int32_t* xlist, const int* xcount, int xcap,
                                  const int32_t* ids, int base, int C, const uint8_t* algo_list,
                                  int algo_all, int dim, uint64_t seed, uint32_t epoch, hipStream_t s,
                                  int dbg) {
  if (xcap <= 0 || C <= 0) return hipSuccess;
  const size_t lds = mz_build_lds_launch(cd.P, cd.toroidal, true, MZ_PY_PHILOX);
  hipError_t ae = mz_lds_attr(reinterpret_cast<const void*>(k_cand_rebuild), lds);
  if (ae != hipSuccess) return ae;
  const int grid = std::max(1, std::min(xcap * C, 1024));
  hipLaunchKernelGGL(k_cand_rebuild, dim3(grid), dim3(WAVE), lds, s, cd, xlist, xcount, xcap, ids, base,
                     C, algo_list, algo_all, dim, seed, epoch, dbg);
  return hipGetLastError();
}

hipError_t mz_launch_cand_gather(const MzDev& cd, const int* count, int n, int C,
                                 const int32_t* status, int32_t* hmap, uint8_t* hgrid,
                                 int32_t* hinfo, int* hcount, int hcap, int gstride, hipStream_t s,
                                 int dbg) {
  if (n <= 0 || C <= 0) return hipSuccess;
  hipLaunchKernelGGL(k_cand_gather, dim3(std::max(1, std::min(n * C, 1024))), dim3(WAVE), 0, s, cd,
                     count, n, C, status, hmap, hgrid, hinfo, hcount, hcap, gstride, dbg);
  return hipGetLastError();
}

hipError_t mz_launch_compact_from_handle(const MzDev& d, const int32_t* ids, int n, const MzCompact& cc,
                                        hipStream_t s) {
  if (n <= 0) return hipSuccess;
  if (cc.Qp < mz_compact_qp(d.P)) return hipErrorInvalidValue;
  hipLaunchKernelGGL(k_compact_from_handle, dim3(std::min(n, 4096)), dim3(WAVE), 0, s, d, ids, n, cc);
  return hipGetLastError();
}

hipError_t mz_launch_cand_select(const MzDev& cd, const MzDev& dst, const int32_t* dst_ids,
                                 int base, const int* count, int n, int C, const double* score,
                                 const int32_t* status, int* stats, hipStream_t s,
                                 const int32_t* xlist, const int32_t* hmap, const double* hprod,
                                 const int32_t* hok, int hcap, int count_groups, int dbg) {
  if (n <= 0) return hipSuccess;
  if (C < 1 || C > WAVE) return hipErrorInvalidValue;
  hipLaunchKernelGGL(k_cand_select, dim3(std::min(n, 4096)), dim3(WAVE), 0, s, cd, dst, dst_ids,
                     base, count, n, C, score, status, stats, xlist, hmap, hprod, hok, hcap,
                     count_groups, dbg);
  return hipGetLastError();
}

hipError_t mz_launch_meta(const MzDev& d, int32_t* out, hipStream_t s) {
  hipLaunchKernelGGL(k_meta, dim3((d.B + 255) / 256), dim3(256), 0, s, d, out);
  return hipGetLastError();
}

hipError_t mz_launch_returns(const double* rew, int ld, const int32_t* rows, const int32_t* lens,
                             int n, double gamma, float* out, int ldo, hipStream_t s) {
  if (n <= 0) return hipSuccess;
  hipLaunchKernelGGL(k_returns, dim3((n + 63) / 64), dim3(64), 0, s, rew, ld, rows, lens, n, gamma,
                     out, ldo);
  return hipGetLastError();
}

hipError_t mz_launch_mask(const MzDev& d, int probs, float* out4, hipStream_t s) {
  hipLaunchKernelGGL(k_mask, dim3((d.B + 255) / 256), dim3(256), 0, s, d, probs, out4);
  return hipGetLastError();
}

hipError_t mz_launch_greedy_list(const MzAct& ap, int n, const int32_t* blk, int32_t* rows,
                                 int32_t* count, int32_t* count_host, hipStream_t s) {
  const int blocks = (n + GR_BLOCK - 1) / GR_BLOCK;
  if (blocks == 0) return hipSuccess;
  hipLaunchKernelGGL(k_greedy_list, dim3(blocks), dim3(GR_BLOCK), 0, s, ap, n, blk, rows, count,
                     count_host);
  return hipGetLastError();
}

hipError_t mz_launch_greedy_rows(const MzAct& ap, int n, int32_t* blk, int32_t* rows,
                                 int32_t* count, int32_t* count_host, hipStream_t s) {
  const int blocks = (n + GR_BLOCK - 1) / GR_BLOCK;
  if (blocks == 0) return hipSuccess;
  hipLaunchKernelGGL(k_greedy_count, dim3(blocks), dim3(GR_BLOCK), 0, s, ap, n, blk);
  return mz_launch_greedy_list(ap, n, blk, rows, count, count_host, s);
}

hipError_t mz_launch_act(const MzDev& d, const MzAct& ap, hipStream_t s) {
  hipLaunchKernelGGL(k_act, dim3((d.B + 255) / 256), dim3(256), 0, s, d, ap);
  return hipGetLastError();
}

hipError_t mz_launch_expand(const uint32_t* bits, float* out, int n, hipStream_t s) {
  long total = (long)n * 675;
  if (total == 0) return hipSuccess;
  hipLaunchKernelGGL(k_expand, dim3((unsigned)((total + 255) / 256)), dim3(256), 0, s, bits, out, n);
  return hipGetLastError();
}
```

maze-solving-agent-gymnasium_amd/csrc/mz_kernels.h:

```cpp
#pragma once
#include "mz_common.h"
#include "mz_screen.h"

size_t mz_build_lds_size(int P);
hipError_t mz_launch_build(const MzDev& d, const int32_t* env_ids, int32_t n, bool generate,
                           const uint8_t* algo_list, int32_t algo_all, int32_t dim, uint64_t seed,
                           const uint8_t* grids, const int32_t* start_goal, int pymode,
                           uint32_t* py_state, hipStream_t s);
hipError_t mz_launch_regen(const MzDev& d, const int32_t* idx, const int32_t* count,
                           int32_t n_static, uint64_t seed, uint32_t epoch, hipStream_t s);
hipError_t mz_launch_step(const MzDev& d, const int32_t* act, const MzAct* ap, bool autoreset,
                          const MzOut& o, hipStream_t s);
hipError_t mz_launch_reset_list(const MzDev& d, const int32_t* idx, int32_t* count,
                                int32_t n_static, const MzOut& o, hipStream_t s);
hipError_t mz_launch_meta(const MzDev& d, int32_t* out, hipStream_t s);
hipError_t mz_launch_returns(const double* rew, int ld, const int32_t* rows, const int32_t* lens,
                             int n, double gamma, float* out, int ldo, hipStream_t s);
hipError_t mz_launch_reset_done(const MzDev& d, int regen, uint64_t seed, uint32_t epoch,
                                const MzOut& o, hipStream_t s);
hipError_t mz_launch_mask(const MzDev& d, int probs, float* out4, hipStream_t s);
hipError_t mz_launch_act(const MzDev& d, const MzAct& ap, hipStream_t s);
hipError_t mz_launch_greedy_rows(const MzAct& ap, int n, int32_t* blk, int32_t* rows,
                                 int32_t* count, int32_t* count_host, hipStream_t s);
hipError_t mz_launch_expand(const uint32_t* bits, float* out, int n, hipStream_t s);
hipError_t mz_launch_qfront(const uint32_t* bits, const float* obs6, const int32_t* rows,
                            const int32_t* count, int n, const float* w, const float* b,
                            float drop_p, uint64_t seed, uint64_t counter, uint16_t* out, int ld,
                            hipStream_t s);
hipError_t mz_launch_cand_build(const MzDev& cd, const int32_t* ids, int base, const int* count, int n,
                                int C, const uint8_t* algo_list, int algo_all, int dim,
                                uint64_t seed, uint32_t epoch, hipStream_t s, int dbg = 0);
hipError_t mz_launch_cand_compact(const MzCompact& cc, int P, const int32_t* ids, int base,
                                  const int* count, int n, int C, const uint8_t* algo_list,
                                  int algo_all, int dim, uint64_t seed, uint32_t epoch, hipStream_t s,
                                  int dbg);
hipError_t mz_launch_cand_pick(const int* count, int n, int C, const double* score,
                               const int32_t* status, int32_t* pick, int32_t* xlist, int* xcount,
                               int xcap, int* stats, hipStream_t s, int dbg);
hipError_t mz_launch_cand_expand(const MzCompact& cc, const MzDev& dst, const int32_t* dst_ids,
                                 int base, const int* count, int n, int C, const int32_t* pick,
                                 const uint8_t* algo_list, int algo_all, hipStream_t s);
hipError_t mz_launch_cand_rebuild(const MzDev& cd, const int32_t* xlist, const int* xcount, int xcap,
                                  const int32_t* ids, int base, int C, const uint8_t* algo_list,
                                  int algo_all, int dim, uint64_t seed, uint32_t epoch, hipStream_t s,
                                  int dbg);
hipError_t mz_launch_cand_gather(const MzDev& cd, const int* count, int n, int C,
                                 const int32_t* status, int32_t* hmap, uint8_t* hgrid,
                                 int32_t* hinfo, int* hcount, int hcap, int gstride, hipStream_t s,
                                 int dbg);
hipError_t mz_launch_compact_from_handle(const MzDev& d, const int32_t* ids, int n, const MzCompact& cc,
                                        hipStream_t s);
hipError_t mz_launch_cand_select(const MzDev& cd, const MzDev& dst, const int32_t* dst_ids,
                                 int base, const int* count, int n, int C, const double* score,
                                 const int32_t* status, int* stats, hipStream_t s,
                                 const int32_t* xlist = nullptr, const int32_t* hmap = nullptr,
                                 const double* hprod = nullptr, const int32_t* hok = nullptr,
                                 int hcap = 0, int count_groups = 1, int dbg = 0);
size_t mz_metrics_lds_bytes(int P);
hipError_t mz_launch_metrics(const MzDev& d, const int32_t* env_ids, int32_t n, double* out,
                             hipStream_t s);

constexpr int MZ_GR_BLOCK = 1024;
```

maze-solving-agent-gymnasium_amd/csrc/mz_trainer.hip:

```cpp
#include <hip/hip_runtime.h>
#include <math.h>
#include <stdint.h>

#include "mz_common.h"
#include "mz_learner.h"

namespace {

constexpr int TB = MZ_GR_BLOCK;
constexpr int W = 64;

__device__ inline float eps_of(float sd, float eps_final, float eps_span, float inv_decay) {
  const float x = __fmul_rn(-sd, inv_decay);
  return __fadd_rn(eps_final, __fmul_rn(eps_span, expf(x)));
}

__global__ __launch_bounds__(TB) void k_tick_count(const uint8_t* __restrict__ term,
                                                   const uint8_t* __restrict__ trunc,
                                                   float* __restrict__ steps_done, float eps_final,
                                                   float eps_span, float inv_decay,
                                                   float* __restrict__ eps_out,
                                                   unsigned long long* wins,
                                                   unsigned long long* episodes, uint64_t seed,
                                                   uint64_t counter, int n, int32_t* blk) {
  __shared__ int ws[TB / W], es[TB / W];
  const int e = blockIdx.x * TB + threadIdx.x;
  const int lane = threadIdx.x & (W - 1), w = threadIdx.x / W;
  bool need = false, won = false, done = false;
  if (e < n) {
    won = term[e] != 0;
    done = won || trunc[e] != 0;
    const float sd = won ? 0.0f : steps_done[e] + 1.0f;
    steps_done[e] = sd;
    const float ep = eps_of(sd, eps_final, eps_span, inv_decay);
    eps_out[e] = ep;
    uint32_t u[4];
    mz_philox(seed, MZ_ACT_STREAM ^ ((uint64_t)e << 32), counter, u);
    need = !((float)(u[0] >> 8) * (1.0f / 16777216.0f) < ep);
  }
  const int c = __syncthreads_count(need);
  const unsigned long long bw = __ballot(won), bd = __ballot(done);
  if (lane == 0) {
    ws[w] = __popcll(bw);
    es[w] = __popcll(bd);
  }
  __syncthreads();
  if (threadIdx.x == 0) {
    blk[blockIdx.x] = c;
    int sw = 0, se = 0;
    for (int i = 0; i < TB / W; ++i) {
      sw += ws[i];
      se += es[i];
    }
    if (wins && sw) atomicAdd(wins, (unsigned long long)sw);
    if (episodes && se) atomicAdd(episodes, (unsigned long long)se);
  }
}

__device__ inline float bf16f(uint16_t h) { return __uint_as_float((uint32_t)h << 16); }

__global__ void k_greedy_scatter(const uint16_t* __restrict__ q, int ldq,
                                 const int32_t* __restrict__ rows, const int32_t* __restrict__ count,
                                 int m, int64_t* __restrict__ greedy) {
  const int i = blockIdx.x * blockDim.x + threadIdx.x;
  const int k = min(*count, m);
  if (i >= k) return;
  const uint16_t* r = q + (size_t)i * ldq;
  int best = 0;
  float bv = bf16f(r[0]);
  for (int a = 1; a < 4; ++a) {
    const float v = bf16f(r[a]);
    if (!isnan(bv) && (v > bv || isnan(v))) {
      best = a;
      bv = v;
    }
  }
  greedy[rows[i]] = best;
}

__device__ inline uint16_t bf16_rne(float f) {
  const uint32_t u = __float_as_uint(f);
  if ((u & 0x7FFFFFFFu) > 0x7F800000u) return (uint16_t)((u >> 16) | 0x40u);
  return (uint16_t)((u + 0x7FFFu + ((u >> 16) & 1u)) >> 16);
}

constexpr int HEAD_MAX_IN = 2048;
__global__ __launch_bounds__(256) void k_head_bf16(MzHeadBf16 h) {
  __shared__ float row[HEAD_MAX_IN];
  if ((int)blockIdx.x < h.out[0]) {
    const int o = blockIdx.x;
    const float* src = h.w[0] + (size_t)o * h.in[0];
    for (int j = threadIdx.x; j < h.in[0]; j += blockDim.x) row[j] = src[j];
    __syncthreads();
    const int nq = h.conv_out / h.conv_ch;
    uint16_t* dst = h.dw[0] + (size_t)o * h.ld0;
    for (int j = threadIdx.x; j < h.ld0; j += blockDim.x) {
      float v = 0.0f;
      if (j < h.conv_out) v = row[(j % h.conv_ch) * nq + j / h.conv_ch];
      else if (j < h.in[0]) v = row[j];
      dst[j] = bf16_rne(v);
    }
    return;
  }
  const int64_t n1 = (int64_t)h.out[1] * h.in[1];
  const int64_t n2 = (int64_t)h.out[2] * h.in[2];
  const int64_t total = n1 + n2 + h.out[0] + h.out[1] + h.out[2];
  const int64_t nb = (int64_t)gridDim.x - h.out[0];
  for (int64_t t = ((int64_t)blockIdx.x - h.out[0]) * blockDim.x + threadIdx.x; t < total;
       t += nb * blockDim.x) {
    int64_t k = t;
    if (k < n1) { h.dw[1][k] = bf16_rne(h.w[1][k]); continue; }
    k -= n1;
    if (k < n2) { h.dw[2][k] = bf16_rne(h.w[2][k]); continue; }
    k -= n2;
    for (int l = 0; l < 3; ++l) {
      if (k < h.out[l]) { h.db[l][k] = bf16_rne(h.b[l][k]); break; }
      k -= h.out[l];
    }
  }
}

__global__ __launch_bounds__(256) void k_replay_push(MzReplayPush p) {
  const int64_t stride = (int64_t)gridDim.x * blockDim.x;
  const int64_t t0 = blockIdx.x * (int64_t)blockDim.x + threadIdx.x;
  for (int j = 0; j < 6; ++j) {
    if (!p.src[j]) continue;
    const int wds = p.words[j];
    const int64_t tot = (int64_t)p.n * wds;
    for (int64_t t = t0; t < tot; t += stride) {
      const int64_t r = t / wds, c = t - r * wds;
      int64_t dr = p.ptr + r;
      if (dr >= p.cap) dr -= p.cap;
      if (j == 2) {
        reinterpret_cast<int64_t*>(p.dst[j])[dr] = reinterpret_cast<const int32_t*>(p.src[j])[r];
      } else {
        reinterpret_cast<uint32_t*>(p.dst[j])[dr * wds + c] =
            reinterpret_cast<const uint32_t*>(p.src[j])[t];
      }
    }
  }
}

__global__ void k_replay_idx(uint64_t seed, uint64_t counter, int64_t newest, int64_t n_avail,
                             int64_t cap, int64_t* __restrict__ out, int n) {
  const int i = blockIdx.x * blockDim.x + threadIdx.x;
  if (i >= n) return;
  uint32_t u[4];
  mz_philox(seed, MZ_REPLAY_STREAM ^ ((uint64_t)i << 32), counter, u);
  const double x = (double)(((uint64_t)u[0] << 21) ^ (u[1] >> 11)) * (1.0 / 9007199254740992.0);
  int64_t r = newest - (int64_t)(x * (double)n_avail);
  r %= cap;
  if (r < 0) r += cap;
  out[i] = r;
}

__global__ __launch_bounds__(1024) void k_q_loss_fwd(const float* __restrict__ q, int ldq,
                                                    const float* __restrict__ qn, int ldn,
                                                    const float* __restrict__ qt, int ldt,
                                                    const int64_t* __restrict__ action,
                                                    const float* __restrict__ reward, float gamma,
                                                    int b, float* __restrict__ loss,
                                                    float* __restrict__ diff) {
  __shared__ float part[1024 / W];
  float acc = 0.0f;
  for (int i = threadIdx.x; i < b; i += blockDim.x) {
    const float* t = qt + (size_t)i * ldt;
    float v;
    if (qn) {
      const float* x = qn + (size_t)i * ldn;
      int best = 0;
      for (int k = 1; k < 4; ++k)
        if (!isnan(x[best]) && (isnan(x[k]) || x[k] > x[best])) best = k;
      v = t[best];
    } else {
      v = t[0];
      for (int k = 1; k < 4; ++k)
        if (!isnan(v) && (isnan(t[k]) || t[k] > v)) v = t[k];
    }
    const float expected = __fadd_rn(__fmul_rn(v, gamma), reward[i]);
    const float d = __fsub_rn(q[(size_t)i * ldq + (int)action[i]], expected);
    diff[i] = d;
    acc = __fadd_rn(acc, __fmul_rn(d, d));
  }
  for (int o = W / 2; o; o >>= 1) acc = __fadd_rn(acc, __shfl_xor(acc, o));
  if ((threadIdx.x & (W - 1)) == 0) part[threadIdx.x / W] = acc;
  __syncthreads();
  if (threadIdx.x == 0) {
// ... 273 lines not shown
```

maze-solving-agent-gymnasium_amd/mazerl/_native.py:

```python
import ctypes as C
import os

from . import _build

c_i32p = C.POINTER(C.c_int32)


class Config(C.Structure):
    _fields_ = [("num_envs", C.c_int32), ("max_dim", C.c_int32), ("toroidal", C.c_int32),
                ("enrich", C.c_int32), ("device", C.c_int32), ("reserved", C.c_int32 * 7)]


class StepOut(C.Structure):
    _fields_ = [("reward", C.c_void_p), ("reward64", C.c_void_p), ("terminated", C.c_void_p),
                ("truncated", C.c_void_p), ("pos", C.c_void_p), ("best_dir", C.c_void_p),
                ("obs6", C.c_void_p), ("window_bits", C.c_void_p), ("window", C.c_void_p),
                ("done_idx", C.c_void_p), ("done_count", C.c_void_p)]


class EnvInfo(C.Structure):
    _fields_ = [(k, C.c_int32) for k in ("n", "start_r", "start_c", "goal_r", "goal_c",
                                         "max_steps", "r", "c", "steps", "invalid_streak",
                                         "nmoves", "last_action", "done")]


MZ_STEP_COUNT_ZEROED = 1
MZ_STEP_AUTORESET = 2
MZ_RNG_PHILOX, MZ_RNG_CPYTHON = 0, 1
MZ_ERRORS = {-1: ValueError, -2: ValueError, -3: RuntimeError, -4: MemoryError, -5: ValueError}

EXPORTS = ["mz_last_error", "mz_device_count", "mz_create", "mz_destroy", "mz_load_mazes",
           "mz_generate", "mz_generate_ex", "mz_generate_state", "mz_reset_all", "mz_reset_list", "mz_reset_done", "mz_step", "mz_step_ex", "mz_direction_mask",
           "mz_act", "mz_step_act", "mz_expand_window", "mz_set_algorithm", "mz_query", "mz_get_grid",
           "mz_difficulty", "mz_maze_complexity", "mz_maze_metrics", "mz_difficulty_batch", "mz_get_meta", "mz_discounted_returns", "mz_q_front",
           "mz_bank_create", "mz_bank_create_dims", "mz_bank_create_ex", "mz_bank_fill", "mz_bank_use",
           "mz_bank_slot_grid", "mz_generate_best", "mz_select_stats", "mz_select_stats_ex",
           "mz_set_debug", "mz_screen_batch", "mz_set_regen_dims",
           "mz_bank_consumed", "mz_state_bytes", "mz_state_save", "mz_state_load",
           "mz_stem_forward", "mz_stem_backward", "mz_stem_backward_ex", "mz_stem_workspace_floats", "mz_adamw_flat",
           "mz_pair_surrogate", "mz_leaky_relu_bf16", "mz_colsum_f32",
           "mz_replay_gather", "mz_host_alloc", "mz_host_free", "mz_q_front_rows", "mz_greedy_rows",
           "mz_trainer_tick", "mz_greedy_scatter", "mz_head_bf16", "mz_replay_push",
           "mz_replay_sample_idx", "mz_q_loss", "mz_q_loss_backward", "mz_head_loss",
           "mz_head_loss_backward", "mz_head_loss_workspace_floats",
           "mz_head_loss_backward_workspace_floats", "mz_adamw_groups",
           "mz_ppo_act", "mz_ppo_scan", "mz_ppo_finish", "mz_ppo_head_loss", "mz_rf_act", "mz_rf_finish",
           "mz_rf_head_loss", "mz_drqn_act", "mz_drqn_store", "mz_drqn_sample",
           "mz_drqn_seq_forward", "mz_drqn_seq_backward", "mz_qact_prepare", "mz_qact",
           "mz_qact_workspace_floats", "mz_qtab_states", "mz_qtab_act", "mz_qtab_update",
           "mz_qtab_hash_act", "mz_qtab_hash_update", "mz_qtab_hash_rehash", "mz_qtab_hash_lookup",
           "mz_dqtab_act", "mz_dqtab_update", "mz_dqtab_hash_act", "mz_dqtab_hash_update",
           "mz_dqtab_hash_rehash", "mz_dqtab_hash_lookup",
           "mz_archive_words", "mz_archive_push", "mz_archive_load",
           "mz_archive_pool_span", "mz_archive_push_pool"]

_lib = None


def lib_path():
    return _build.LIB


def load(build_if_missing=True):
    global _lib
    if _lib is not None:
        return _lib
    path = os.environ.get("MZ_LIB_OVERRIDE") or _build.LIB
    if not os.path.exists(path):
        if not build_if_missing:
            raise RuntimeError(f"libmazerl.so not built ({path}); run mazerl._build.build()")
        _build.build()
    L = C.CDLL(path)
    vp = C.c_void_p
    L.mz_last_error.restype = C.c_char_p
    L.mz_device_count.argtypes = [c_i32p]
    L.mz_create.argtypes = [C.POINTER(Config), C.POINTER(vp)]
    L.mz_destroy.argtypes = [vp]
    L.mz_load_mazes.argtypes = [vp, vp, C.c_int32, vp, vp, C.c_int32, vp]
    L.mz_generate.argtypes = [vp, vp, C.c_int32, vp, C.c_int32, C.c_int32, C.c_uint64, vp]
    L.mz_generate_ex.argtypes = [vp, vp, C.c_int32, vp, C.c_int32, C.c_int32, C.c_uint64,
                                 C.c_int32, vp]
    L.mz_generate_state.argtypes = [vp, C.c_int32, C.c_int32, C.c_int32, vp, vp]
    L.mz_reset_all.argtypes = [vp, C.POINTER(StepOut), vp]
    L.mz_reset_list.argtypes = [vp, vp, vp, C.c_int32, C.c_int32, C.c_uint64, C.c_uint32,
                                C.POINTER(StepOut), vp]
    L.mz_reset_done.argtypes = [vp, C.c_int32, C.c_uint64, C.c_uint32, C.POINTER(StepOut), vp]
    L.mz_step.argtypes = [vp, vp, C.POINTER(StepOut), vp]
    L.mz_step_ex.argtypes = [vp, vp, C.POINTER(StepOut), C.c_int32, vp]
    L.mz_direction_mask.argtypes = [vp, C.c_int32, vp, vp]
    L.mz_act.argtypes = [vp, vp, C.c_float, vp, C.c_uint64, C.c_uint64, vp, vp]
    L.mz_step_act.argtypes = [vp, vp, C.c_float, vp, C.c_uint64, C.c_uint64, vp,
                              C.POINTER(StepOut), C.c_int32, vp]
    L.mz_expand_window.argtypes = [vp, vp, C.c_int32, vp]
    L.mz_set_algorithm.argtypes = [vp, vp, C.c_int32, vp]
    L.mz_query.argtypes = [vp, C.c_int32, C.POINTER(EnvInfo)]
    L.mz_get_grid.argtypes = [vp, C.c_int32, vp]
    L.mz_get_meta.argtypes = [vp, vp, vp]
    L.mz_discounted_returns.argtypes = [vp, C.c_int32, vp, vp, C.c_int32, C.c_double, vp,
                                        C.c_int32, vp]
    L.mz_difficulty.argtypes = [vp] + [C.c_int32] * 6 + [C.POINTER(C.c_double)]
    L.mz_maze_complexity.argtypes = [vp] + [C.c_int32] * 6 + [C.POINTER(C.c_double)] * 2
    L.mz_maze_metrics.argtypes = [vp, vp, C.c_int32, vp, vp]
    L.mz_difficulty_batch.argtypes = [vp, vp, C.c_int32, vp, vp, vp]
    L.mz_bank_create.argtypes = [vp, C.c_int32, C.c_int32, C.c_uint32]
    L.mz_bank_create_dims.argtypes = [vp, C.c_int32, vp, C.c_int32, C.c_uint32]
    L.mz_bank_create_ex.argtypes = [vp, C.c_int32, vp, C.c_int32, C.c_uint32, C.c_int32]
    L.mz_bank_fill.argtypes = [vp, C.c_int32, C.c_uint64, vp]
    L.mz_bank_slot_grid.argtypes = [vp, C.c_int32, C.c_int32, C.c_int32, C.c_int32, vp, vp]
    L.mz_generate_best.argtypes = [vp, vp, C.c_int32, vp, C.c_int32, C.c_int32, C.c_uint64,
                                   C.c_int32, vp]
    L.mz_select_stats.argtypes = [vp, vp, C.c_int32, vp]
    if hasattr(L, "mz_select_stats_ex") or not os.environ.get("MZ_LIB_OVERRIDE"):
        L.mz_select_stats_ex.argtypes = [vp, vp, C.c_int32, C.c_int32, vp]
        L.mz_set_debug.argtypes = [vp, C.c_int32]
        L.mz_screen_batch.argtypes = [vp, vp, C.c_int32, vp, vp, vp]
    L.mz_set_regen_dims.argtypes = [vp, vp]
    L.mz_bank_use.argtypes = [vp, C.c_int32]
    L.mz_bank_consumed.argtypes = [vp, C.c_int32, vp, vp]
    L.mz_state_bytes.argtypes = [vp, C.POINTER(C.c_uint64)]
    L.mz_state_save.argtypes = [vp, vp, C.c_uint64, vp]
    L.mz_state_load.argtypes = [vp, vp, C.c_uint64, vp]
    L.mz_q_front.argtypes = [vp, vp, C.c_int32, vp, vp, C.c_float, C.c_uint64, C.c_uint64, vp,
                             C.c_int32, vp]
    L.mz_q_front_rows.argtypes = [vp, vp, vp, vp, C.c_int32, vp, vp, C.c_float, C.c_uint64,
                                  C.c_uint64, vp, C.c_int32, vp]
    L.mz_greedy_rows.argtypes = [vp, C.c_float, C.c_uint64, C.c_uint64, C.c_int32, vp, vp, vp, vp,
                                 vp]
    L.mz_trainer_tick.argtypes = [vp, vp, vp, C.c_double, C.c_double, C.c_double, vp, vp, vp,
                                  C.c_uint64, C.c_uint64, C.c_int32, vp, vp, vp, vp]
    L.mz_greedy_scatter.argtypes = [vp, C.c_int32, vp, vp, C.c_int32, vp, vp]
    L.mz_head_bf16.argtypes = [vp] * 6 + [C.c_int32] * 9 + [vp] * 7
    L.mz_replay_push.argtypes = [C.c_int32, C.c_int64, C.c_int64] + [vp] * 12 + [C.c_int32,
                                                                                 C.c_int32, vp]
    L.mz_replay_sample_idx.argtypes = [C.c_uint64, C.c_uint64, C.c_int64, C.c_int64, C.c_int64,
                                       vp, C.c_int32, vp]
    L.mz_q_loss.argtypes = [vp, C.c_int32, vp, C.c_int32, vp, C.c_int32, vp, vp, C.c_double,
                            C.c_int32, vp, vp, vp]
    L.mz_q_loss_backward.argtypes = [vp, vp, vp, C.c_int32, C.c_int32, vp, vp]
    L.mz_head_loss.argtypes = [vp, C.c_int32, vp, vp, vp, C.c_int32, vp, vp, C.c_int32, C.c_int32,
                               C.c_int32, vp, vp, C.c_double, C.c_int32, vp, vp, vp, vp, vp]
    L.mz_head_loss_backward.argtypes = [vp, vp, vp, C.c_int32, vp, C.c_int32, vp, C.c_int32,
                                        C.c_int32, vp, C.c_int32, vp, vp]
    L.mz_head_loss_workspace_floats.argtypes = [C.c_int32]
    L.mz_head_loss_backward_workspace_floats.argtypes = [C.c_int32, C.c_int32]
    L.mz_stem_forward.argtypes = [vp, vp, C.c_int32, vp, vp, C.c_float, vp, C.c_uint32, vp,
                                  C.c_int32, vp, vp]
    L.mz_stem_backward.argtypes = [vp, vp, vp, C.c_int32, C.c_int32, C.c_float, vp, vp, vp, vp]
    if hasattr(L, "mz_stem_backward_ex"):
        L.mz_stem_backward_ex.argtypes = [vp, vp, vp, C.c_int32, C.c_int32, C.c_float, vp, vp, vp,
                                          vp, vp]
    L.mz_stem_workspace_floats.argtypes = [C.c_int32]
    L.mz_qact_workspace_floats.argtypes = [C.c_int32]
    L.mz_leaky_relu_bf16.argtypes = [vp, C.c_int64, C.c_float, vp]
    L.mz_colsum_f32.argtypes = [vp, C.c_int32, C.c_int32, C.c_int32, vp, vp]
    L.mz_replay_gather.argtypes = [vp, C.c_int32, C.c_int64] + [vp] * 11
    L.mz_pair_surrogate.argtypes = [vp, vp, vp, C.c_int32, C.c_float, vp, vp, vp]
    L.mz_adamw_flat.argtypes = [vp, vp, vp, vp, vp, C.c_int32, vp, vp, C.c_double, C.c_double,
                                C.c_double, C.c_double, C.c_float, C.c_float, C.c_int32, vp]
    L.mz_adamw_groups.argtypes = [vp, vp, vp, vp, vp, vp, C.c_int32, vp, vp, C.c_double,
                                  C.c_double, C.c_double, C.c_double, C.c_float, vp, vp]
    L.mz_ppo_act.argtypes = [vp, C.c_int32, vp, C.c_int32, vp, vp, C.c_int32, C.c_int32,
                             C.c_uint64, C.c_uint64] + [vp] * 8
    L.mz_ppo_scan.argtypes = [vp, vp, vp, C.c_int32, C.c_int32] + [vp] * 10
    L.mz_ppo_head_loss.argtypes = [vp, C.c_int32, vp, C.c_int32, vp, vp, vp, vp, vp, C.c_int32,
                                   C.c_float, vp, vp, vp, C.c_int32, vp, C.c_int32, vp]
    L.mz_ppo_finish.argtypes = [vp] * 6 + [C.c_int32, C.c_int32] + [vp] * 4 + \
        [C.c_double, C.c_int64] + [vp] * 7
    L.mz_rf_act.argtypes = [vp, C.c_int32, C.c_float, vp, vp, C.c_int32, C.c_int32, C.c_uint64,
                            C.c_uint64] + [vp] * 6
    L.mz_rf_finish.argtypes = [vp] * 4 + [C.c_int32, C.c_int32] + [vp] * 4 + \
        [C.c_double, C.c_int64] + [vp] * 7
    L.mz_rf_head_loss.argtypes = [vp, C.c_int32, vp, vp, vp, vp, C.c_int32, C.c_float, C.c_float,
                                  vp, vp, C.c_int32, vp]
    L.mz_drqn_act.argtypes = [vp, C.c_int32, vp, C.c_int32, C.c_int32, C.c_float, C.c_int32,
                              C.c_uint64, C.c_uint64] + [vp] * 8
    L.mz_drqn_store.argtypes = [vp, vp, C.c_int32, C.c_int32] + [vp] * 6 + [C.c_int64] + [vp] * 5
    L.mz_drqn_sample.argtypes = [C.c_uint64, C.c_uint64, C.c_int32, C.c_int32, C.c_int64,
                                 C.c_int64] + [vp] * 7
    L.mz_drqn_seq_forward.argtypes = [vp, C.c_int32, C.c_int32, C.c_int32, C.c_int32, C.c_int64,
                                      C.c_float] + [vp] * 13
    L.mz_drqn_seq_backward.argtypes = [vp, C.c_int32, C.c_int32, C.c_int32, C.c_int64] + [vp] * 12
    L.mz_qact_prepare.argtypes = [vp] * 7
    L.mz_qact.argtypes = [vp, vp, vp, vp, C.c_int32] + [vp] * 10 + [C.c_int32, C.c_float,
                                                                   C.c_uint64, C.c_uint64] + [vp] * 4
    L.mz_qtab_states.argtypes = [C.c_int32, C.POINTER(C.c_int64)]
    L.mz_qtab_act.argtypes = [vp, C.c_int32, C.c_int32, vp, C.c_int32, vp, vp, vp, vp, vp, vp,
                              C.c_uint64, C.c_uint64, vp, vp, vp]
    L.mz_qtab_update.argtypes = [vp, C.c_int32, C.c_int32, vp, C.c_int32] + [vp] * 13 + \
        [C.c_int32, vp]
    L.mz_qtab_hash_act.argtypes = [vp, C.c_int32, C.c_int32, vp, C.c_int32, vp, vp, vp, C.c_int64,
                                   vp, vp, vp, vp, C.c_uint64, C.c_uint64, vp, vp, vp]
    L.mz_qtab_hash_update.argtypes = [vp, C.c_int32, C.c_int32, vp, C.c_int32, vp, vp, C.c_int64] + \
        [vp] * 14 + [C.c_int32, vp]
    L.mz_qtab_hash_rehash.argtypes = [vp, vp, C.c_int64, vp, vp, C.c_int64, C.c_int32, vp, vp]
    L.mz_qtab_hash_lookup.argtypes = [vp, vp, C.c_int64, C.c_int32, vp, vp, C.c_int32, vp, vp, vp]
    dq_tail = [vp] * 4 + [C.c_uint64, C.c_uint64] + [vp] * 5
    L.mz_dqtab_act.argtypes = L.mz_qtab_act.argtypes
    L.mz_dqtab_update.argtypes = L.mz_qtab_update.argtypes[:-1] + dq_tail
    L.mz_dqtab_hash_act.argtypes = L.mz_qtab_hash_act.argtypes
    L.mz_dqtab_hash_update.argtypes = L.mz_qtab_hash_update.argtypes[:-1] + dq_tail
    L.mz_dqtab_hash_rehash.argtypes = L.mz_qtab_hash_rehash.argtypes
    L.mz_dqtab_hash_lookup.argtypes = L.mz_qtab_hash_lookup.argtypes
    L.mz_archive_words.argtypes = [C.c_int32, c_i32p]
    L.mz_archive_push.argtypes = [vp, vp, C.c_int32, C.c_int32, vp, vp, vp, vp, vp]
    L.mz_archive_load.argtypes = [vp, vp, C.c_int32, vp, C.c_int32, vp, vp, vp, vp, vp]
    L.mz_archive_pool_span.argtypes = [c_i32p]
    L.mz_archive_push_pool.argtypes = [vp, vp, C.c_int32, C.c_int32, vp, vp, vp, vp, vp, vp,
                                       C.c_int32, vp]
    L.mz_host_alloc.argtypes = [C.c_uint64, C.c_int32, C.POINTER(vp), C.POINTER(vp)]
    L.mz_host_free.argtypes = [vp]
    for f in EXPORTS:
        if f != "mz_last_error" and (hasattr(L, f) or not os.environ.get("MZ_LIB_OVERRIDE")):
            getattr(L, f).restype = C.c_int
    L.mz_qact_workspace_floats.restype = C.c_int64
    _lib = L
    return L


def check(rc):
    if rc != 0:
        msg = load().mz_last_error().decode(errors="replace")
        raise MZ_ERRORS.get(rc, RuntimeError)(f"libmazerl error {rc}: {msg}")
    return rc
```

maze-solving-agent-gymnasium_amd/mazerl/agents/dqn.py:

```python
import collections
import copy
import math
import os
import random

import numpy as np
import torch
import torch.nn.functional as F
import torch.optim as optim
from torch.optim import lr_scheduler

from ..replay import ReplayMemory, Transition
from .flat import copy_flat
from .nets import QNet


STACK_ROWS = True
K_BLOCK = os.environ.get("MZ_K_BLOCK", "1") != "0"
GRAPH_COLLECTIVES = os.environ.get("MZ_GRAPH_COLLECTIVES", "0") == "1"
FUSED_LOSS = os.environ.get("MZ_FUSED_LOSS", "1") != "0"
FUSED_HEAD = os.environ.get("MZ_FUSED_HEAD", "1") != "0"


class _QLossFn(torch.autograd.Function):
# ... 253 lines not shown
        action_batch = torch.tensor(batch.action).to(device)
        reward_batch = torch.tensor(batch.reward).to(device)
        loss = q_loss(self.source_net, self.target_net, state_batch, action_batch, reward_batch,
                      next_states, self.discount_factor, self.VARIANT == "ddqn")
        ret = loss.item()
        learner_update(self.source_net, self.optimizer, loss)
        return ret

    def scheduler_step(self):
        self.lr_scheduler.step()

    def has_to_update(self, episode):
        return episode % self.target_update_frequency == 0

    def update_target(self):
        self.target_net.load_state_dict(self.source_net.state_dict())

    def update_steps_done(self):
        self.steps_done = 0

    def update_hyperparameter(self, is_better):
        self.discount_factor = self.discount_factor + (self.eta if is_better else -self.eta)


class DQNAgent(_AgentBase):
    VARIANT, T_MAX = "dqn", 100


class DDQNAgent(_AgentBase):
    VARIANT, T_MAX = "ddqn", 150


class VectorDQNLearner:

    def __init__(self, num_envs, device, variant="ddqn", lr=1e-3, eps_start=0.95, eps_final=0.1,
                 eps_decay=8000.0, gamma=0.7, batch_size=128, capacity=1_000_000,
                 updates_per_step=1, target_every=100, hidden_dim=1024, h_channels=32,
                 act_bf16=True, t_max=150, updates_per_epoch=100, allreduce=None, seed=0,
                 use_graph=True, bit_stem=True, overlap=False, greedy_rows=True, acting="x3",
                 graph_collectives=None):
        self.device = torch.device(device)
        if self.device.type == "cuda":
            from ..gemm_tuning import enable as _tuned_gemms
            _tuned_gemms(self.device)
        torch.manual_seed(seed)
        self.variant = variant
        self.source = QNet(3, 6, 4, h_channels, hidden_dim, variant).to(self.device)
        self.target = QNet(3, 6, 4, h_channels, hidden_dim, variant).to(self.device)
        self.target.load_state_dict(self.source.state_dict())
        if variant == "ddqn" and self.device.type == "cuda" and bit_stem and \
                os.environ.get("MZ_STEM_COUNTER_FOLD", "1") != "0":
            ctr = torch.zeros(1, dtype=torch.int64, device=self.device)
            self.source._stem_rng, self.target._stem_rng = ctr, ctr
            self.source._stem_advance, self.target._stem_advance = "backward", "none"
        self.use_graph = bool(use_graph) and self.device.type == "cuda"
        gc = GRAPH_COLLECTIVES if graph_collectives is None else bool(graph_collectives)
        self.graph_collectives = gc and self.use_graph and allreduce is not None
        self.bit_stem = bool(bit_stem) and self.device.type == "cuda"
        if self.use_graph:
            from .flat import FlatAdamW, flatten_grads, flatten_params
            flatten_params(self.target)
            self.opt = FlatAdamW(self.source, lr, write_grad=False)
            flatten_grads(self.source)
        else:
            self.opt = optim.AdamW(self.source.parameters(), lr)
        self._graph = None
        self._graph_loss = None
        self._graphK = [None, None]
        self._graphK_loss = [None, None]
        self._eager_updates = 0
        self.sched = lr_scheduler.CosineAnnealingLR(self.opt, T_max=t_max, eta_min=1e-5)
        from ..replay import DeviceReplay
        self.replay = DeviceReplay(capacity, self.device)
        self.gamma, self.batch_size = gamma, batch_size
        self.eps_start, self.eps_final, self.eps_decay = eps_start, eps_final, eps_decay
        self.updates_per_step, self.target_every = updates_per_step, target_every
        self.updates_per_epoch = updates_per_epoch
        self.act_bf16 = act_bf16
        self.allreduce = allreduce
        if allreduce is not None and hasattr(allreduce, "attach"):
            allreduce.attach(self.source, self.opt)
        self.steps_done = torch.zeros(num_envs, dtype=torch.float32, device=self.device)
        self.n_updates = 0
        self.last_loss = torch.zeros((), device=self.device)
        self.fused = None
        self.greedy_rows = bool(greedy_rows)
        self._rows = None
        if acting not in ("x3", "bf16"):
            raise ValueError(f"acting {acting!r}: 'x3' or 'bf16'")
        self.acting = acting
        if self.device.type == "cuda" and act_bf16:
            self.fused = self._head(self.source, seed)
        self.overlap = bool(overlap) and self.use_graph and self.fused is not None
        self._async = False
        if self.overlap:
            self.side = torch.cuda.Stream(self.device,
                                          priority=int(os.environ.get("MZ_LEARNER_PRIORITY", "0")))
            from .flat import flatten_params
            self.actors = [copy.deepcopy(self.source) for _ in range(2)]
            for a in self.actors:
                flatten_params(a)
            self.actor_fused = [self._head(a, seed * 2 + 101 + k) for k, a in enumerate(self.actors)]
            self._published = collections.deque()
            self._acting = None
            self._idx = None
            self._par = 0
            self._sample_seed = 0x5A3B1E + 7919 * int(seed)
            self._sample_counter = 0

    def _head(self, net, seed):
        if self.acting == "x3":
            from .qact import QAct
            return QAct(net, seed=seed)
        from .fused import FusedQ
        return FusedQ(net, seed=seed)

    @property
    def supports_bits(self):
        return self.fused is not None

    def epsilon(self):
        return self.eps_final + (self.eps_start - self.eps_final) * torch.exp(-self.steps_done / self.eps_decay)

    @torch.no_grad()
    def greedy(self, obs6, window, bits=None, act=None):
        if bits is not None and self.fused is not None:
            f = self.actor_fused[self._acting_slot()] if self._async else self.fused
            if act is not None and self.greedy_rows:
                if self._rows is None:
                    from .fused import GreedyRows
                    self._rows = GreedyRows(bits.shape[0], self.device)
                return self._rows(f, obs6, bits, *act)
            if hasattr(f, "greedy"):
                return f.greedy(obs6, bits)
            return f(obs6, bits).float().argmax(1)
        if window is None:
            raise ValueError("greedy() needs the f32 window or window bits on the GPU")
        if self.act_bf16 and self.device.type == "cuda":
            with torch.autocast("cuda", dtype=torch.bfloat16):
                q = self.source((obs6, window))
        else:
            q = self.source((obs6, window))
        return q.float().argmax(1)

    def tick(self, term, trunc, wins, episodes, seed, counter):
        if self.fused is None or not self.greedy_rows:
            return None
        if self._rows is None:
            from .fused import GreedyRows
            self._rows = GreedyRows(self.steps_done.numel(), self.device)
        return self._rows.tick(term, trunc, self.steps_done, self.eps_start, self.eps_final,
                               self.eps_decay, wins, episodes, seed, counter)

    def prepare_greedy(self, eps, seed, counter):
        if self.fused is None or not self.greedy_rows:
            return
        if self._rows is None:
            from .fused import GreedyRows
            self._rows = GreedyRows(self.steps_done.numel(), self.device)
        self._rows.issue(eps, seed, counter)

    def update(self, expand, reserve=0):
        if len(self.replay) < self.batch_size:
            return None
        if self.overlap and self._graph is not None:
            return self._update_async(reserve)
        for _ in range(self.updates_per_step):
            if self.use_graph:
                self._graph_update(expand)
            else:
                self.last_loss = self._one_update(expand, static=False)
            self.n_updates += 1
            if self.n_updates % self.target_every == 0:
                self._sync_target()
            if self.n_updates % self.updates_per_epoch == 0:
                self.sched.step()
        if self.fused is not None:
            self.fused.invalidate()
        return self.last_loss

    @torch.no_grad()
    def _sync_target(self):
        if getattr(self.source, "_flat_params", None) is not None and \
                getattr(self.target, "_flat_params", None) is not None:
            copy_flat(self.target, self.source)
        else:
            self.target.load_state_dict(self.source.state_dict())

    def _acting_slot(self):
        M = torch.cuda.current_stream(self.device)
        while len(self._published) > 1 or (self._acting is None and self._published):
            slot, ev = self._published.popleft()
            M.wait_event(ev)
            self._acting = slot
        return self._acting

    def _start_async(self):
        M = torch.cuda.current_stream(self.device)
        with torch.no_grad():
            for a, f in zip(self.actors, self.actor_fused):
                copy_flat(a, self.source)
                f.refresh()
        K, b = self.updates_per_step, self.batch_size
        if getattr(self, "_idx", None) is None or tuple(self._idx[0].shape) != (K, b):
            self._idx = [torch.zeros(K, b, dtype=torch.int64, device=self.device) for _ in range(2)]
            self._graphK = [None, None]
        self._idx_ev = [None, None]
        self._acting, self._par = 0, 1
        self._published.clear()
        self.side.wait_stream(M)
        self._async = True

    def _update_async(self, reserve):
        if not self._async:
            self._start_async()
        M, S = torch.cuda.current_stream(self.device), self.side
        rp, K, slot = self.replay, self.updates_per_step, self._par
        n_avail = min(rp.size, rp.capacity - int(reserve))
        if n_avail < self.batch_size:
            raise ValueError("replay too small to exclude the next push from sampling")
        if self._idx_ev[slot] is not None:
            M.wait_event(self._idx_ev[slot])
        idx = self._idx[slot]
        from .. import _native as N
        N.check(N.load().mz_replay_sample_idx(self._sample_seed, self._sample_counter, rp.ptr - 1,
                                              n_avail, rp.capacity, idx.data_ptr(), idx.numel(),
                                              M.cuda_stream))
        self._sample_counter += 1
        if self._acting == slot:
            self._acting = None
        block = self._k_block_ok()
        if block and self._graphK[slot] is None:
            self._capture_k_block(slot)
        S.wait_stream(M)
        with torch.cuda.stream(S):
            if block:
                self._graphK[slot].replay()
                self.n_updates += K
                if self.n_updates % self.target_every == 0:
                    self._sync_target()
                if self.n_updates % self.updates_per_epoch == 0:
                    self.sched.step()
            for k in range(0 if block else K):
                rp.idx_static.copy_(idx[k])
                self._graph[0].replay()
                if len(self._graph) == 2:
                    self.allreduce.reduce()
                    self._graph[1].replay()
                    self.allreduce.gather(self.source)
                self.n_updates += 1
                if self.n_updates % self.target_every == 0:
                    self._sync_target()
                if self.n_updates % self.updates_per_epoch == 0:
                    self.sched.step()
            with torch.no_grad():
                copy_flat(self.actors[slot], self.source)
                self.actor_fused[slot].refresh()
            ev = torch.cuda.Event()
            ev.record(S)
        self._idx_ev[slot] = ev
        self._published.append((slot, ev))
        self._par ^= 1
        self.last_loss = self._graphK_loss[slot] if block else self._graph_loss
        return self.last_loss

    def _k_block_ok(self):
        K = self.updates_per_step
        if K < 2 or (self.allreduce is not None and not self.graph_collectives) or not K_BLOCK \
                or not self.bit_stem:
            return False
        n0 = self.n_updates
        return all((n0 + j) % self.target_every and (n0 + j) % self.updates_per_epoch
                   for j in range(1, K))

    def _capture_k_block(self, slot):
        rp, K = self.replay, self.updates_per_step
        g = torch.cuda.CUDAGraph()
        keep = rp.idx_static
        try:
            with torch.cuda.graph(g, capture_error_mode=self._capture_mode()):
                for k in range(K):
                    rp.idx_static = self._idx[slot][k]
                    loss = self._one_update(None, static=True)
        finally:
            rp.idx_static = keep
        self._graphK[slot] = g
        self._graphK_loss[slot] = loss

    def finish(self):
        if self._async:
            torch.cuda.current_stream(self.device).wait_stream(self.side)
            self._published.clear()
            self._async = False
            self.fused.invalidate()

    def state_dict(self):
        self.finish()
        rp, n = self.replay, self.replay.size
        opt = self.opt
        if hasattr(opt, "exp_avg"):
            ost = {"exp_avg": opt.exp_avg.clone(), "exp_avg_sq": opt.exp_avg_sq.clone(),
                   "step": opt._step_buf.clone(), "lr": float(opt.param_groups[0]["lr"]),
                   "shard": None if opt.shard is None else [int(x) for x in opt.shard]}
        else:
            ost = {"torch": opt.state_dict()}
        heads = [self.fused] + list(getattr(self, "actor_fused", []))
# ... 147 lines not shown
```

maze-solving-agent-gymnasium_amd/mazerl/agents/fused.py:

```python
import torch
import torch.nn as nn
import torch.nn.functional as F

from .. import _native as N

LD = 1600
CONV_OUT = 1568


def feature_perm(device=None):
    return torch.arange(CONV_OUT, device=device).view(32, 49).t().reshape(-1)


def _leaky_(h, slope):
    if h.is_cuda and h.dtype == torch.bfloat16 and h.is_contiguous() and h.numel() % 8 == 0 \
            and h.data_ptr() % 16 == 0:
        N.check(N.load().mz_leaky_relu_bf16(h.data_ptr(), h.numel(), float(slope),
                                            torch.cuda.current_stream(h.device).cuda_stream))
        return h
    return F.leaky_relu_(h, slope)


def _act_fn(m):
    if isinstance(m, nn.LeakyReLU):
# ... 72 lines not shown
        mods = list(conv_seq)
        self.conv = mods[0]
        assert isinstance(self.conv, nn.Conv2d) and tuple(self.conv.weight.shape) == (32, 3, 3, 3), \
            "the fused stem implements the reference's Conv2d(3, 32, 3, padding=1)"
        assert isinstance(mods[1], nn.LeakyReLU) and mods[1].negative_slope == 0.01
        self.dropout = next((m for m in mods if isinstance(m, nn.Dropout)), None)
        assert isinstance(mods[-1], nn.MaxPool2d)
        self.seed = seed
        self.counter = 0
        self.lib = N.load()

    def __call__(self, obs6, bits, rows=None, n=None, count=None, out=None):
        dev = bits.device
        if dev.type != "cuda":
            raise RuntimeError("the fused acting stem runs on the GPU only")
        assert bits.dtype == torch.int32 and bits.shape[1] == 22 and bits.is_contiguous()
        obs6 = obs6.contiguous()
        assert obs6.dtype == torch.float32 and obs6.shape == (bits.shape[0], 6)
        if rows is None:
            n = bits.shape[0]
        else:
            assert rows.dtype == torch.int32 and rows.is_contiguous() and rows.device == dev
            assert 0 <= n <= rows.numel()
        w = self.conv.weight.detach().contiguous()
        b = self.conv.bias.detach().contiguous()
        p = float(self.dropout.p) if (self.dropout is not None and self.dropout.training) else 0.0
        feat = torch.empty(n, LD, dtype=torch.bfloat16, device=dev) if out is None else out[:n]
        stream = torch.cuda.current_stream(dev).cuda_stream
        if rows is None:
            N.check(self.lib.mz_q_front(bits.data_ptr(), obs6.data_ptr(), n, w.data_ptr(),
                                        b.data_ptr(), p, self.seed, self.counter, feat.data_ptr(),
                                        LD, stream))
        else:
            N.check(self.lib.mz_q_front_rows(bits.data_ptr(), obs6.data_ptr(), rows.data_ptr(),
                                             count.data_ptr() if count is not None else None, n,
                                             w.data_ptr(), b.data_ptr(), p, self.seed, self.counter,
                                             feat.data_ptr(), LD, stream))
        self.counter += 1
        return feat


class FusedQ:

    def __init__(self, qnet, seed=0):
        self.stem = FusedStem(qnet.conv, seed)
        self.head = _Head(qnet.fc)

    def invalidate(self):
        self.head.invalidate()

    def refresh(self):
        self.head.refresh()

    @torch.no_grad()
    def __call__(self, obs6, bits):
        return self.head(self.stem(obs6, bits))

    @torch.no_grad()
    def rows(self, obs6, bits, rows, n):
        return self.head(self.stem(obs6, bits, rows, n))

    @torch.no_grad()
    def rows_stem(self, obs6, bits, rows, count, out):
        self.stem(obs6, bits, rows, out.shape[0], count=count, out=out)

    @torch.no_grad()
    def rows_head(self, feat):
        return self.head(feat)


class GreedyRows:

    BUCKET = 256

    def __init__(self, n, device):
        self.n = n
        self.rows = torch.zeros(n, dtype=torch.int32, device=device)
        self.scratch = torch.zeros((n + 1023) // 1024, dtype=torch.int32, device=device)
        self.count = torch.zeros(1, dtype=torch.int32, device=device)
        self.count_host = torch.zeros(1, dtype=torch.int32, pin_memory=True)
        self.greedy = torch.zeros(n, dtype=torch.int64, device=device)
        self.event = torch.cuda.Event()
        self.lib = N.load()
        self.last_count = None
        self.feat = None

    def issue(self, eps, seed, counter):
        stream = torch.cuda.current_stream(self.rows.device).cuda_stream
        eps_t = eps if torch.is_tensor(eps) else None
        if eps_t is not None:
            assert eps_t.dtype == torch.float32 and eps_t.is_contiguous() and eps_t.numel() == self.n
        N.check(self.lib.mz_greedy_rows(eps_t.data_ptr() if eps_t is not None else None,
                                        0.0 if eps_t is not None else float(eps),
                                        seed & 0xFFFFFFFFFFFFFFFF, counter & 0xFFFFFFFFFFFFFFFF,
                                        self.n, self.scratch.data_ptr(), self.rows.data_ptr(),
                                        self.count.data_ptr(), None, stream))
        self.count_host.copy_(self.count, non_blocking=True)
        self.event.record()
        self._issued = (eps_t.data_ptr() if eps_t is not None else float(eps), seed, counter)

    def select(self, eps, seed, counter):
        key = (eps.data_ptr() if torch.is_tensor(eps) else float(eps), seed, counter)
        if getattr(self, "_issued", None) != key:
            self.issue(eps, seed, counter)
        self._issued = None
        self.event.synchronize()
        self.last_count = int(self.count_host[0])
        return self.last_count

    @torch.no_grad()
    def __call__(self, fused, obs6, bits, eps, seed, counter):
        key = (eps.data_ptr() if torch.is_tensor(eps) else float(eps), seed, counter)
        if getattr(self, "_issued", None) != key:
            self.issue(eps, seed, counter)
        if hasattr(fused, "rows_greedy"):
            self._issued = None
            fused.rows_greedy(obs6, bits, self.rows, self.count, self.greedy)
            return self.greedy
        if self.feat is None:
            self.feat = torch.zeros(self.n, LD, dtype=torch.bfloat16, device=self.rows.device)
        fused.rows_stem(obs6, bits, self.rows, self.count, self.feat)
        k = self.select(eps, seed, counter)
        if k:
            m = min(self.n, -(-k // self.BUCKET) * self.BUCKET)
            q = fused.rows_head(self.feat[:m])
            assert q.dtype == torch.bfloat16 and q.is_contiguous() and q.shape == (m, 4)
            N.check(self.lib.mz_greedy_scatter(q.data_ptr(), 4, self.rows.data_ptr(),
                                               self.count.data_ptr(), m, self.greedy.data_ptr(),
                                               torch.cuda.current_stream(q.device).cuda_stream))
        return self.greedy

    def tick(self, term, trunc, steps_done, eps_start, eps_final, eps_decay, wins, episodes, seed,
             counter):
        if not hasattr(self, "eps"):
            self.eps = torch.empty(self.n, dtype=torch.float32, device=self.rows.device)
        for t in (term, trunc):
            assert t.dtype == torch.uint8 and t.is_contiguous() and t.numel() == self.n
        assert steps_done.dtype == torch.float32 and steps_done.is_contiguous()
        for t in (wins, episodes):
            assert t is None or (t.dtype == torch.int64 and t.numel() == 1)
        N.check(self.lib.mz_trainer_tick(
            term.data_ptr(), trunc.data_ptr(), steps_done.data_ptr(), float(eps_start),
            float(eps_final), float(eps_decay), self.eps.data_ptr(),
            wins.data_ptr() if wins is not None else None,
            episodes.data_ptr() if episodes is not None else None,
            seed & 0xFFFFFFFFFFFFFFFF, counter & 0xFFFFFFFFFFFFFFFF, self.n, self.scratch.data_ptr(),
            self.rows.data_ptr(), self.count.data_ptr(),
            torch.cuda.current_stream(self.rows.device).cuda_stream))
        self.count_host.copy_(self.count, non_blocking=True)
        self.event.record()
        self._issued = (self.eps.data_ptr(), seed, counter)
        return self.eps


class FusedActorCritic:

    def __init__(self, net, seed=0):
        self.stem = FusedStem(net.conv, seed)
        self.actor = _Head(net.actor_head)
        self.critic = _Head(net.critic_head)

    def invalidate(self):
        self.actor.invalidate()
        self.critic.invalidate()

    @torch.no_grad()
    def __call__(self, obs6, bits):
        feat = self.stem(obs6, bits)
        return self.actor(feat), self.critic(feat)
```

maze-solving-agent-gymnasium_amd/mazerl/replay.py:

```python
import random
from collections import deque, namedtuple

import torch

Transition = namedtuple("Transition", ("state", "action", "reward", "next_state"))


class ReplayMemory:
    def __init__(self, capacity):
        self.memory = deque([], maxlen=capacity)

    def push(self, *args):
        self.memory.append(Transition(*args))

    def sample(self, batch_size):
        return random.sample(self.memory, batch_size)

    def clear_memory(self):
        self.memory.clear()

    def __len__(self):
        return len(self.memory)


class DeviceReplay:
    def __init__(self, capacity, device, obs_dim=6, window_words=22):
        self.capacity = int(capacity)
        self.device = torch.device(device)
        C, kw = self.capacity, dict(device=self.device)
        self.s6 = torch.zeros(C, obs_dim, dtype=torch.float32, **kw)
        self.sw = torch.zeros(C, window_words, dtype=torch.int32, **kw)
        self.a = torch.zeros(C, dtype=torch.int64, **kw)
        self.r = torch.zeros(C, dtype=torch.float32, **kw)
        self.s6n = torch.zeros(C, obs_dim, dtype=torch.float32, **kw)
        self.swn = torch.zeros(C, window_words, dtype=torch.int32, **kw)
        self.ptr = 0
        self.size = 0
        self.size_dev = torch.zeros((), dtype=torch.float64, **kw)
        self.idx_static = None
        self._gen = torch.Generator(device=self.device)
        self._gen.manual_seed(0x5EED)

    def __len__(self):
        return self.size

    def nbytes(self):
        return sum(t.numel() * t.element_size() for t in (self.s6, self.sw, self.a, self.r, self.s6n, self.swn))

    def push(self, s6, sw, a, r, s6n, swn, mask=None):
        if mask is not None:
            keep = torch.nonzero(mask, as_tuple=False).flatten()
            s6, sw, a, r, s6n, swn = (t.index_select(0, keep) for t in (s6, sw, a, r, s6n, swn))
        n = a.shape[0]
        if n == 0:
            return
        if n > self.capacity:
            s6, sw, a, r, s6n, swn = (t[-self.capacity:] for t in (s6, sw, a, r, s6n, swn))
            n = self.capacity
        self._write(((self.s6, s6), (self.sw, sw), (self.a, a), (self.r, r), (self.s6n, s6n),
                     (self.swn, swn)), n)
        self.ptr = (self.ptr + n) % self.capacity
        size = min(self.size + n, self.capacity)
        if size != self.size:
            self.size_dev.fill_(float(size))
        self.size = size

    def _ring_push(self, n, s6=None, sw=None, a=None, r=None, s6n=None, swn=None):
        from . import _native as N
        if n > self.capacity:
            raise ValueError("a push larger than the ring")
        srcs = (s6, sw, a, r, s6n, swn)
        dts = (torch.float32, torch.int32, torch.int32, torch.float32, torch.float32, torch.int32)
        for t, dt in zip(srcs, dts):
            if t is not None:
                assert t.dtype == dt and t.is_contiguous() and t.shape[0] == n and t.is_cuda
        ptr = lambda t: t.data_ptr() if t is not None else None
        N.check(N.load().mz_replay_push(
            n, self.capacity, self.ptr, *[ptr(t) for t in srcs], self.s6.data_ptr(),
            self.sw.data_ptr(), self.a.data_ptr(), self.r.data_ptr(), self.s6n.data_ptr(),
            self.swn.data_ptr(), self.s6.shape[1], self.sw.shape[1],
            torch.cuda.current_stream(self.device).cuda_stream))

    def push_state(self, s6, sw):
        self._ring_push(s6.shape[0], s6=s6, sw=sw)

    def push_rest(self, a, r, s6n, swn):
        n = a.shape[0]
        self._ring_push(n, a=a, r=r, s6n=s6n, swn=swn)
        self.ptr = (self.ptr + n) % self.capacity
        size = min(self.size + n, self.capacity)
        if size != self.size:
            self.size_dev.fill_(float(size))
        self.size = size

    def _write(self, pairs, n):
        k = min(n, self.capacity - self.ptr)
        for dst, src in pairs:
            dst[self.ptr:self.ptr + k].copy_(src[:k])
            if k < n:
                dst[:n - k].copy_(src[k:n])

    def sample_indices(self, batch):
        return torch.randint(0, self.size, (batch,), device=self.device, generator=self._gen)

    def sample_indices_static(self, batch):
        u = torch.rand(batch, dtype=torch.float64, device=self.device)
        return (u * self.size_dev).to(torch.int64).clamp_(max=self.capacity - 1)

    def sample(self, batch, expand, static=False, idx_static=False):
        if idx_static:
            if self.idx_static is None or self.idx_static.numel() != batch:
                self.idx_static = self.sample_indices(batch)
            i = self.idx_static
        else:
            i = self.sample_indices_static(batch) if static else self.sample_indices(batch)
        if expand is None:
            if self.device.type == "cuda" and self.s6.shape[1] == 6 and self.sw.shape[1] == 22:
                return self._gather_stacked(i, batch)
            return ((self.s6.index_select(0, i), self.sw.index_select(0, i)), self.a.index_select(0, i),
                    self.r.index_select(0, i), (self.s6n.index_select(0, i), self.swn.index_select(0, i)))
        bits = torch.cat((self.sw.index_select(0, i), self.swn.index_select(0, i)), 0)
        w = expand(bits)
        return ((self.s6.index_select(0, i), w[:batch]), self.a.index_select(0, i),
                self.r.index_select(0, i), (self.s6n.index_select(0, i), w[batch:]))

    def _gather_stacked(self, i, batch):
        from . import _native as N
        dev = self.device
        i = i.contiguous()
        s6 = torch.empty(2 * batch, self.s6.shape[1], dtype=torch.float32, device=dev)
        sw = torch.empty(2 * batch, self.sw.shape[1], dtype=torch.int32, device=dev)
        a = torch.empty(batch, dtype=torch.int64, device=dev)
        r = torch.empty(batch, dtype=torch.float32, device=dev)
        N.check(N.load().mz_replay_gather(
            i.data_ptr(), batch, self.capacity, self.s6.data_ptr(), self.sw.data_ptr(),
            self.a.data_ptr(), self.r.data_ptr(), self.s6n.data_ptr(), self.swn.data_ptr(), s6.data_ptr(),
            sw.data_ptr(), a.data_ptr(), r.data_ptr(), torch.cuda.current_stream(dev).cuda_stream))
        return (s6[:batch], sw[:batch]), a, r, (s6[batch:], sw[batch:])
```

maze-solving-agent-gymnasium_amd/mazerl/trainers/vector_trainer.py:

```python
import os
import time

import torch

from ..archive import MazePool
from ..vector_env import ALGOS, VectorMazeEnv
from .schedule import enable_winner_bank, make_schedule, max_shape_stop


class VectorOffPolicyTrainer:

    def __init__(self, env, learner, seed=0, regen_won=True, curriculum=False, allreduce_stats=None,
                 bank=True, fused=True, growth=None, algorithm="r-prim", bank_candidates=1,
                 track_wins=False, archive=None):
        self.env, self.learner = env, learner
        self.track_wins = bool(track_wins)
        rule, self.schedule = make_schedule(env, curriculum, growth, learner, algorithm)
        if regen_won and bank:
            enable_winner_bank(env, rule, self.schedule, bank_candidates)
        self.archive = None
        if archive is not None:
            if isinstance(archive, MazePool):
                if archive.env is not env:
                    raise ValueError("the pool was built for another env")
                self.archive = archive
            else:
                self.archive = MazePool(env, archive)
            self.archive.record(stamp=0)
        self.seed = seed
        self.fused = bool(fused)
        self.regen_won = regen_won
        self.curriculum = rule
        self.allreduce_stats = allreduce_stats
        dev = env.device
        self.wins = torch.zeros((), dtype=torch.int64, device=dev)
        self.episodes = torch.zeros((), dtype=torch.int64, device=dev)
        self.inst_wins = torch.zeros(env.num_envs, dtype=torch.int32, device=dev)
        self.counter = 0
        self.stopped_at = None
        self._eps = None
        self.history = []

    @property
    def algo(self):
        return None if self.schedule is None else self.schedule.maze_algo

    def _expand(self, bits):
        return self.env.expand_window(bits)

    def vector_step(self):
        env, L = self.env, self.learner
        eps = self._eps if self._eps is not None else L.epsilon()
        self._eps = None
        greedy = L.greedy(env.obs6, env.window, env.window_bits, act=(eps, self.seed, self.counter))
        rp = L.replay
        ring = self.fused and hasattr(rp, "push_state") and env.window_bits is not None and \
            env.device.type == "cuda"
        if ring:
            rp.push_state(env.obs6, env.window_bits)
        else:
            s6, sw = env.obs6.clone(), env.window_bits.clone()
        env.step_act(eps=eps, greedy=greedy, seed=self.seed, counter=self.counter)
        self.counter += 1
        tick = getattr(L, "tick", None) if self.fused and not self.curriculum else None
        self._eps = tick(env.terminated, env.truncated, self.wins, self.episodes, self.seed,
                         self.counter) if tick is not None else None
        if self._eps is None:
            term = env.terminated.bool()
            L.steps_done += 1
            L.steps_done.masked_fill_(term, 0)
            if hasattr(L, "prepare_greedy"):
                self._eps = L.epsilon()
                L.prepare_greedy(self._eps, self.seed, self.counter)
            self.wins += term.sum()
            self.episodes += (term | env.truncated.bool()).sum()
        sch = self.schedule
        if sch is not None:
            won = env.terminated.bool()
            self.inst_wins += won.to(torch.int32)
            sch.before_reset(won)
        elif self.track_wins:
            self.inst_wins += env.terminated.to(torch.int32)
        if ring:
            rp.push_rest(env.actions, env.reward, env.obs6, env.window_bits)
        else:
            rp.push(s6, sw, env.actions, env.reward, env.obs6, env.window_bits)
        arch = self.archive if self.regen_won else None
        if arch is not None:
            rd = env._regen_dims
            new_maze = env.terminated.clone() if rd is None else \
                (env.terminated.bool() & (rd > 0)).to(torch.uint8)
        env.reset_done(regen_won=self.regen_won)
        if sch is not None:
            sch.after_reset(won)
        if arch is not None:
            arch.record(new_maze, stamp=self.counter)
        return L.update(self._expand, reserve=env.num_envs)

    def train(self, vector_steps, log_every=0, log=print):
        t0 = time.perf_counter()
        prio = os.environ.get("MZ_ACT_PRIORITY")
        if prio is None or self.env.device.type != "cuda":
            return self._train(vector_steps, log_every, log, t0)
        outer = torch.cuda.current_stream(self.env.device)
        if getattr(self, "_act_stream", None) is None:
            self._act_stream = torch.cuda.Stream(self.env.device, priority=int(prio))
        s = self._act_stream
        s.wait_stream(outer)
        with torch.cuda.stream(s):
            secs = self._train(vector_steps, log_every, log, t0)
        outer.wait_stream(s)
        return secs

    def state_dict(self):
        L = self.learner
        sd = {"format": "mazerl.VectorOffPolicyTrainer/2", "seed": self.seed,
              "counter": self.counter, "wins": self.wins.clone(), "episodes": self.episodes.clone(),
              "inst_wins": self.inst_wins.clone(), "curriculum": self.curriculum,
              "regen_won": self.regen_won, "history": list(self.history),
              "schedule": None if self.schedule is None else self.schedule.state_dict(),
              "learner": L.state_dict(), "env": self.env.state_dict()}
        if self.archive is not None:
            sd["archive"] = self.archive.state_dict()
        return sd

    def summary(self):
        out = {"vector_steps": self.counter, "stopped_at": self.stopped_at,
               "schedule": None if self.schedule is None else self.schedule.summary(),
               "archive": None}
        if self.archive is not None:
            a = self.archive
            count, held, dropped = torch.stack([a.count, a.held, a.dropped]).tolist()
            out["archive"] = {"capacity": a.capacity, "recorded": count, "held": held,
                              "dropped": dropped}
        return out

    def load_state_dict(self, sd):
        fmt = sd.get("format")
        if fmt == "mazerl.VectorOffPolicyTrainer/1":
            raise ValueError("a format-1 VectorOffPolicyTrainer checkpoint (before the win "
                             "schedule, round 5): not loadable by this version")
        if fmt != "mazerl.VectorOffPolicyTrainer/2":
            raise ValueError("not a VectorOffPolicyTrainer state_dict")
        if sd["curriculum"] != self.curriculum or bool(sd["regen_won"]) != bool(self.regen_won) \
                or (sd["schedule"] is None) != (self.schedule is None):
            raise ValueError("curriculum / growth / regen_won differ from the saved trainer's")
        if ("archive" in sd) != (self.archive is not None):
            raise ValueError("the saved trainer and this one differ in having an explored-maze "
                             "pool (archive=)")
        if self.archive is not None:
            self.archive.check_state_dict(sd["archive"])
        self.env.load_state_dict(sd["env"])
        self.learner.load_state_dict(sd["learner"])
        if self.schedule is not None:
            self.schedule.load_state_dict(sd["schedule"])
        self.seed, self.counter = int(sd["seed"]), int(sd["counter"])
        self.wins.copy_(sd["wins"])
        self.episodes.copy_(sd["episodes"])
        self.inst_wins.copy_(sd["inst_wins"])
        self.history = list(sd["history"])
        if self.archive is not None:
            self.archive.load_state_dict(sd["archive"])
        self._eps = None

    def _train(self, vector_steps, log_every, log, t0):
        self._eps = None
        rows = getattr(self.learner, "_rows", None)
        if rows is not None:
            rows._issued = None
        sch = self.schedule
        for k in range(vector_steps):
            loss = self.vector_step()
            if max_shape_stop(sch, k):
                self.stopped_at = k + 1
                break
            if log_every and (k + 1) % log_every == 0:
                torch.cuda.synchronize()
                rec = dict(step=k + 1, wins=int(self.wins), episodes=int(self.episodes),
                           loss=float(loss) if loss is not None else None,
                           eps_mean=float(self.learner.epsilon().mean()),
                           seconds=round(time.perf_counter() - t0, 2))
                self.history.append(rec)
                if log:
                    log(rec)
        if hasattr(self.learner, "finish"):
            self.learner.finish()
        torch.cuda.synchronize()
        return time.perf_counter() - t0


def make_env(num_envs, dims, toroidal=False, algorithm="r-prim", seed=0x5EED0000, device=None,
             max_dim=None, candidates=1, **kw):
    dims = [dims] if isinstance(dims, int) else list(dims)
    env = VectorMazeEnv(num_envs, dims[0], toroidal=toroidal, enrich=True, device=device,
                        max_dim=max(max(dims), int(max_dim or 0)), algorithm=algorithm, seed=seed,
                        generate=len(dims) == 1, candidates=candidates, **kw)
    env.dims_in_use = sorted(set(dims))
    if len(dims) > 1:
        ids = torch.arange(num_envs, device=env.device)
        for j, n in enumerate(dims):
            sel = ids[ids % len(dims) == j]
            if sel.numel():
                algo = algorithm if isinstance(algorithm, str) else torch.as_tensor(algorithm)[sel.cpu()]
                env.generate(env_ids=sel.to(torch.int32), algorithm=algo, dim=n, seed=seed,
                             candidates=candidates)
        env.set_algorithm(algorithm if isinstance(algorithm, str) else torch.as_tensor(algorithm).to(torch.uint8))
        env.reset()
    return env


def maze_algorithms(num_mazes, seed, algos=("r-prim", "prim&kill", "dfs")):
    import random
    rng = random.Random(seed)
    return [rng.choice(list(algos)) for _ in range(num_mazes)]


def best_of_mazes(num_mazes, dim, algorithm="r-prim", seed=0x7E57, device=None, candidates=6,
                  toroidal=False):
    import numpy as np
    from ..difficulty import difficulty_batch
    dims = [dim] if isinstance(dim, int) else list(dim)
    n, C = int(num_mazes), int(candidates)
    size_of = [dims[k % len(dims)] for k in range(n)]
    algo_of = [algorithm] * n if isinstance(algorithm, str) else list(algorithm)
    if len(algo_of) != n:
        raise ValueError("one algorithm per maze")
    cand = VectorMazeEnv(n * C, size_of[0], toroidal=toroidal, enrich=True, device=device,
                         max_dim=max(dims), algorithm=algo_of[0], seed=seed, done_list=False,
                         pos=False, window=False, window_bits=False,
                         generate=len(set(size_of)) == 1 and len(set(algo_of)) == 1)
    if len(set(size_of)) > 1 or len(set(algo_of)) > 1:
        groups = {}
        for k in range(n):
            groups.setdefault((size_of[k], algo_of[k]), []).extend(range(k * C, k * C + C))
        for (sz, al), ids in sorted(groups.items()):
            cand.generate(env_ids=torch.tensor(ids, dtype=torch.int32, device=cand.device),
                          algorithm=al, dim=sz, seed=seed)
    d = difficulty_batch(cand).reshape(n, C)
    pick = d.argmin(axis=1)
    D = max(dims)
# ... 130 lines not shown
```

maze-solving-agent-gymnasium_amd/mazerl/vector_env.py:

```python
import torch

from . import _native as N

ALGOS = {"r-prim": 0, "dfs": 1, "prim&kill": 2}


def _ptr(t):
    return None if t is None else t.data_ptr()


def bank_seed(env_seed):
    return (0xBA4C0000 + (int(env_seed) - 0x5EED0000) * 0x9E3779B97F4A7C15) & 0xFFFFFFFFFFFFFFFF


class VectorMazeEnv:
    def __init__(self, num_envs, maze_dim, toroidal=False, enrich=True, device=None,
                 max_dim=None, algorithm="r-prim", seed=0x5EED0000, generate=True,
                 window=True, window_bits=True, reward64=False, pos=True, done_list=True,
                 host_scalars=False, candidates=1):
        if not torch.cuda.is_available():
            raise RuntimeError("VectorMazeEnv needs a HIP GPU (libmazerl.so has no CPU path)")
        self.lib = N.load()
        self.device = torch.device(device if device is not None else f"cuda:{torch.cuda.current_device()}")
        self.num_envs = int(num_envs)
# ... 63 lines not shown
        self._host = hp
        raw = np.ctypeslib.as_array((N.C.c_uint8 * total).from_address(hp.value))
        for name in ("reward64", "pos", "best_dir"):
            setattr(self, name, None)
        for (name, dt, shape), off in offs:
            n = int(np.prod(shape)) * np.dtype(dt).itemsize
            t = torch.from_numpy(raw[off:off + n].view(dt).reshape(shape))
            setattr(self, name, t)
            self._dptr[t.data_ptr()] = dpp.value + off

    def _dev_ptr(self, t):
        if t is None:
            return None
        return self._dptr.get(t.data_ptr(), t.data_ptr())

    def close(self):
        if getattr(self, "_h", None):
            self.lib.mz_destroy(self._h)
            self._h = None
        if getattr(self, "_host", None) is not None:
            for name in ("actions", "reward", "reward64", "terminated", "truncated", "pos", "best_dir"):
                setattr(self, name, None)
            self.lib.mz_host_free(self._host)
            self._host = None

    def __del__(self):
        try:
            self.close()
        except Exception:
            pass

    def generate(self, env_ids=None, algorithm="r-prim", dim=None, seed=None, rng="philox",
                 candidates=1):
        dim = int(dim or self.maze_dim)
        seed = self.seed if seed is None else int(seed)
        ids = None if env_ids is None else torch.as_tensor(env_ids, dtype=torch.int32, device=self.device)
        n = self.num_envs if ids is None else int(ids.numel())
        algo_t, algo_all = None, 0
        if isinstance(algorithm, str):
            algo_all = ALGOS[algorithm]
            self.algos_in_use.add(algo_all)
        elif isinstance(algorithm, int):
            algo_all = int(algorithm)
            self.algos_in_use.add(algo_all)
        else:
            algo_t = torch.as_tensor(algorithm, dtype=torch.uint8, device=self.device)
            if algo_t.numel() != n:
                raise ValueError("per-instance algorithm ids must match the env list")
            self.algos_in_use.update(ALGOS.values())
        mode = {"philox": N.MZ_RNG_PHILOX, "cpython": N.MZ_RNG_CPYTHON}[rng]
        if int(candidates) > 1:
            if mode != N.MZ_RNG_PHILOX:
                raise ValueError("best-of-C generation draws Philox candidates (rng='philox')")
            N.check(self.lib.mz_generate_best(self._h, _ptr(ids), n, _ptr(algo_t), algo_all, dim,
                                              seed & 0xFFFFFFFFFFFFFFFF, int(candidates),
                                              self._stream()))
            return self
        N.check(self.lib.mz_generate_ex(self._h, _ptr(ids), n, _ptr(algo_t), algo_all, dim,
                                        seed & 0xFFFFFFFFFFFFFFFF, mode, self._stream()))
        return self

    def select_stats(self, reset=False):
        out = torch.zeros(5, dtype=torch.int32, device=self.device)
        if hasattr(self.lib, "mz_select_stats_ex"):
            N.check(self.lib.mz_select_stats_ex(self._h, out.data_ptr(), 5, int(bool(reset)),
                                                self._stream()))
        else:
            N.check(self.lib.mz_select_stats(self._h, out.data_ptr(), int(bool(reset)),
                                             self._stream()))
        u, t, g, x, hs = (int(x) for x in out.cpu())
        return {"unresolved": u, "near_ties": t, "groups": g, "exact": x, "host_scored": hs}

    def set_debug(self, flags):
        N.check(self.lib.mz_set_debug(self._h, int(flags)))

    def set_regen_dims(self, dims):
        if dims is None:
            self._regen_dims = None
            N.check(self.lib.mz_set_regen_dims(self._h, None))
            return
        t = torch.as_tensor(dims, device=self.device).to(torch.uint8).contiguous()
        if t.numel() != self.num_envs:
            raise ValueError("one size per instance")
        self._regen_dims = t
        N.check(self.lib.mz_set_regen_dims(self._h, t.data_ptr()))

    def generate_from_random(self, env_id=0, algorithm="r-prim", dim=None, rnd=None):
        import random as _random
        import numpy as np
        rnd = _random if rnd is None else rnd
        dim = int(dim or self.maze_dim)
        algo = ALGOS[algorithm] if isinstance(algorithm, str) else int(algorithm)
        self.algos_in_use.add(algo)
        version, words, gauss = rnd.getstate()
        st = np.array(words, dtype=np.uint32)
        N.check(self.lib.mz_generate_state(self._h, int(env_id), dim, algo, st.ctypes.data,
                                           self._stream()))
        rnd.setstate((version, tuple(int(x) for x in st), gauss))
        return self

    def load_mazes(self, grids, start_goal, env_ids=None):
        import numpy as np
        g = np.ascontiguousarray(grids, dtype=np.uint8)
        sg = np.ascontiguousarray(start_goal, dtype=np.int32)
        ids = None if env_ids is None else np.ascontiguousarray(env_ids, dtype=np.int32)
        n, dim = g.shape[0], g.shape[1]
        N.check(self.lib.mz_load_mazes(self._h, g.ctypes.data, dim, sg.ctypes.data,
                                       None if ids is None else ids.ctypes.data, n,
                                       self._stream()))
        return self

    def set_algorithm(self, algorithm):
        if isinstance(algorithm, str):
            N.check(self.lib.mz_set_algorithm(self._h, None, ALGOS[algorithm], self._stream()))
            self.algos_in_use = {ALGOS[algorithm]}
        else:
            t = torch.as_tensor(algorithm, dtype=torch.uint8, device=self.device)
            N.check(self.lib.mz_set_algorithm(self._h, _ptr(t), 0, self._stream()))
            self.algos_in_use = set(ALGOS.values())

    def _host_sync(self):
        if self._host is not None:
            torch.cuda.current_stream(self.device).synchronize()

    def reset(self):
        N.check(self.lib.mz_reset_all(self._h, N.C.byref(self._out), self._stream()))
        self._host_sync()
        return self.obs(), {}

    def reset_list(self, idx, count=None, regen_won=False, seed=None):
        idx = torch.as_tensor(idx, dtype=torch.int32, device=self.device)
        if regen_won:
            self.epoch += 1
        N.check(self.lib.mz_reset_list(self._h, _ptr(idx), _ptr(count), int(idx.numel()),
                                       int(bool(regen_won)),
                                       (self.seed if seed is None else int(seed)) & 0xFFFFFFFFFFFFFFFF,
                                       self.epoch & 0xFFFFFFFF, N.C.byref(self._out),
                                       self._stream()))
        if count is not None and count.data_ptr() == self.done_count.data_ptr():
            self._count_zero = True
        self._host_sync()

    def reset_done(self, regen_won=False, seed=None):
        if regen_won:
            self.epoch += 1
        N.check(self.lib.mz_reset_done(self._h, int(bool(regen_won)),
                                       (self.seed if seed is None else int(seed)) & 0xFFFFFFFFFFFFFFFF,
                                       self.epoch & 0xFFFFFFFF, N.C.byref(self._out),
                                       self._stream()))
        if regen_won and self._bank is not None:
            self._bank_tick()
        self._host_sync()

    def enable_bank(self, slots=None, swap_every=8, algorithms=None, seed=None, dims=None,
                    candidates=1):
        if self._bank is not None:
            return
        if seed is None:
            seed = bank_seed(self.seed)
        dims = [self.maze_dim] if dims is None else sorted({int(d) for d in dims})
        K = int(slots or max(64 // len(dims) if len(dims) > 1 else 64,
                             self.num_envs // 8 // len(dims), 16))
        if algorithms is None:
            mask = sum(1 << i for i in self.algos_in_use) or 7
        else:
            ids = [ALGOS[a] if isinstance(a, str) else int(a) for a in algorithms]
            mask = sum(1 << i for i in set(ids))
        arr = (N.C.c_int32 * len(dims))(*dims)
        N.check(self.lib.mz_bank_create_ex(self._h, K, arr, len(dims), mask, int(candidates)))
        self._bank = dict(K=K, dims=dims, swap=int(swap_every), calls=0, cur=0, seed=int(seed),
                          side=torch.cuda.Stream(self.device), ready=[None, None],
                          candidates=int(candidates))
        st = self._stream()
        for b in (0, 1):
            N.check(self.lib.mz_bank_fill(self._h, b, self._bank["seed"], st))
        N.check(self.lib.mz_bank_use(self._h, 0))

    def _bank_tick(self):
        bk = self._bank
        bk["calls"] += 1
        if bk["calls"] % bk["swap"]:
            return
        old, new = bk["cur"], 1 - bk["cur"]
        main = torch.cuda.current_stream(self.device)
        if bk["ready"][new] is not None:
            main.wait_event(bk["ready"][new])
        N.check(self.lib.mz_bank_use(self._h, new))
        bk["cur"] = new
        consumed = torch.cuda.Event()
        consumed.record(main)
        side = bk["side"]
        side.wait_event(consumed)
        N.check(self.lib.mz_bank_fill(self._h, old, bk["seed"], side.cuda_stream))
        ev = torch.cuda.Event()
        ev.record(side)
        bk["ready"][old] = ev

    def bank_slot(self, bank, algorithm, dim, slot):
        import numpy as np
        a = ALGOS[algorithm] if isinstance(algorithm, str) else int(algorithm)
        di = self._bank["dims"].index(int(dim))
        g = np.zeros((self.max_dim, self.max_dim), np.uint8)
        info = np.zeros(4, np.int32)
        N.check(self.lib.mz_bank_slot_grid(self._h, int(bank), a, di, int(slot), g.ctypes.data,
                                           info.ctypes.data))
        n = int(dim)
        return g.reshape(-1)[:n * n].reshape(n, n).copy(), tuple(int(x) for x in info)

    def bank_consumed(self, bank=None):
        nd = len(self._bank["dims"])
        out = torch.zeros(3 * nd, dtype=torch.int32, device=self.device)
        b = self._bank["cur"] if bank is None else int(bank)
        N.check(self.lib.mz_bank_consumed(self._h, b, out.data_ptr(), self._stream()))
        return out if nd == 1 else out.view(3, nd)

    _OUTPUTS = ("reward", "reward64", "terminated", "truncated", "pos", "best_dir", "actions",
                "obs6", "window", "window_bits", "done_idx", "done_count")

    def state_dict(self):
        main = torch.cuda.current_stream(self.device)
        if self._bank is not None:
            for ev in self._bank["ready"]:
                if ev is not None:
                    main.wait_event(ev)
        n = N.C.c_uint64()
        N.check(self.lib.mz_state_bytes(self._h, N.C.byref(n)))
        blob = torch.empty(n.value, dtype=torch.uint8, device=self.device)
        N.check(self.lib.mz_state_save(self._h, blob.data_ptr(), n.value, self._stream()))
        out = {k: getattr(self, k).clone() for k in self._OUTPUTS if getattr(self, k) is not None}
        bank = None
        if self._bank is not None:
            bank = {k: self._bank[k] for k in ("K", "dims", "swap", "calls", "cur", "seed",
                                               "candidates")}
        return {"format": "mazerl.VectorMazeEnv/1", "num_envs": self.num_envs,
                "maze_dim": self.maze_dim, "max_dim": self.max_dim, "toroidal": self.toroidal,
                "enrich": self.enrich, "seed": self.seed, "epoch": self.epoch,
                "count_zero": self._count_zero, "algos_in_use": sorted(self.algos_in_use),
                "device_state": blob, "outputs": out, "bank": bank,
                "regen_dims": None if self._regen_dims is None else self._regen_dims.clone()}

    def load_state_dict(self, sd):
        if sd.get("format") != "mazerl.VectorMazeEnv/1":
            raise ValueError("not a VectorMazeEnv state_dict")
        bank = sd.get("bank")
        if (bank is None) != (self._bank is None) or (bank is not None and (
                bank["K"] != self._bank["K"] or list(bank["dims"]) != list(self._bank["dims"])
                or int(bank.get("candidates", 1)) != self._bank["candidates"])):
            raise ValueError("maze bank mismatch: call enable_bank() with the saved geometry "
                             "(or not at all) before load_state_dict()")
        blob = sd["device_state"].to(device=self.device, dtype=torch.uint8).contiguous()
        if self._bank is not None:
            main = torch.cuda.current_stream(self.device)
            for ev in self._bank["ready"]:
                if ev is not None:
                    main.wait_event(ev)
        N.check(self.lib.mz_state_load(self._h, blob.data_ptr(), blob.numel(), self._stream()))
        for k, v in sd["outputs"].items():
            dst = getattr(self, k, None)
            if dst is None or tuple(dst.shape) != tuple(v.shape):
                raise ValueError(f"output {k!r}: this env's buffer does not match the saved one")
            dst.copy_(v)
        self.seed, self.epoch = int(sd["seed"]), int(sd["epoch"])
        self._count_zero = bool(sd["count_zero"])
        self.algos_in_use = set(sd.get("algos_in_use", ()))
        self.set_regen_dims(sd.get("regen_dims"))
        if bank is not None:
            self._bank.update(swap=int(bank["swap"]), calls=int(bank["calls"]),
                              cur=int(bank["cur"]), seed=int(bank["seed"]), ready=[None, None])
            self._bank["side"].wait_stream(torch.cuda.current_stream(self.device))
        self._host_sync()

    def reset_done_list(self, regen_won=False, seed=None):
        self.reset_list(self.done_idx, self.done_count, regen_won=regen_won, seed=seed)

    def step_host(self, action, env=0):
        if self._host is None:
            raise RuntimeError("step_host needs VectorMazeEnv(host_scalars=True)")
        self.actions[env] = int(action)
        N.check(self.lib.mz_step_ex(self._h, self._dev_ptr(self.actions), N.C.byref(self._out), 0,
                                    self._stream()))
        self._count_zero = False
        torch.cuda.current_stream(self.device).synchronize()

    def sync(self):
        torch.cuda.current_stream(self.device).synchronize()

    def step(self, actions, autoreset=False):
        a = actions if (actions.dtype == torch.int32 and actions.device == self.device) else \
            actions.to(device=self.device, dtype=torch.int32)
        a = a.contiguous()
        flags = N.MZ_STEP_AUTORESET if autoreset else 0
        N.check(self.lib.mz_step_ex(self._h, self._dev_ptr(a), N.C.byref(self._out), flags,
                                    self._stream()))
        self._count_zero = False
        self._host_sync()
        return self.obs(), self.reward, self.truncated, self.terminated, {}

    def step_act(self, eps=1.0, greedy=None, seed=0, counter=0, actions_out=None, autoreset=False):
        out = self.actions if actions_out is None else actions_out
        out_p = self._dev_ptr(out)
        eps_t = eps if torch.is_tensor(eps) else None
        g = None if greedy is None else greedy.to(dtype=torch.int64).contiguous()
        flags = N.MZ_STEP_COUNT_ZEROED if self._count_zero else 0
        if autoreset:
            flags |= N.MZ_STEP_AUTORESET
        N.check(self.lib.mz_step_act(self._h, _ptr(eps_t), float(eps) if eps_t is None else 0.0,
                                     _ptr(g), seed & 0xFFFFFFFFFFFFFFFF,
                                     counter & 0xFFFFFFFFFFFFFFFF, out_p,
                                     N.C.byref(self._out), flags, self._stream()))
        self._count_zero = False
        self._host_sync()
        return self.obs(), self.reward, self.truncated, self.terminated, {}

    def obs(self):
        o = {"obs6": self.obs6}
        if self.pos is not None:
            o["agent"], o["best dir"] = self.pos, self.best_dir
        if self.window is not None:
            o["window"] = self.window
        if self.window_bits is not None:
            o["window_bits"] = self.window_bits
        return o

    def direction_mask(self, probs=False, out=None):
        out = out if out is not None else torch.empty(self.num_envs, 4, dtype=torch.float32, device=self.device)
        N.check(self.lib.mz_direction_mask(self._h, int(bool(probs)), out.data_ptr(), self._stream()))
        return out

    def act(self, eps=1.0, greedy=None, seed=0, counter=0, out=None):
        out = out if out is not None else self.actions
        eps_t = eps if torch.is_tensor(eps) else None
        g = None if greedy is None else greedy.to(dtype=torch.int64).contiguous()
        N.check(self.lib.mz_act(self._h, _ptr(eps_t), float(eps) if eps_t is None else 0.0,
                                _ptr(g), seed & 0xFFFFFFFFFFFFFFFF, counter & 0xFFFFFFFFFFFFFFFF,
                                self._dev_ptr(out), self._stream()))
        if out is self.actions:
            self._host_sync()
        return out

    def expand_window(self, bits, out=None):
        n = bits.shape[0]
        out = out if out is not None else torch.empty(n, 3, 15, 15, dtype=torch.float32, device=bits.device)
        N.check(self.lib.mz_expand_window(bits.data_ptr(), out.data_ptr(), n, self._stream()))
        return out

    def meta(self, out=None):
        out = out if out is not None else torch.empty(self.num_envs, 6, dtype=torch.int32, device=self.device)
        N.check(self.lib.mz_get_meta(self._h, out.data_ptr(), self._stream()))
        return out

    def maze_metrics(self, env_ids=None, out=None):
        ids = None if env_ids is None else torch.as_tensor(env_ids, dtype=torch.int32, device=self.device)
        n = self.num_envs if ids is None else int(ids.numel())
        out = out if out is not None else torch.empty(n, 6, dtype=torch.float64, device=self.device)
        N.check(self.lib.mz_maze_metrics(self._h, _ptr(ids), n, out.data_ptr(), self._stream()))
        return out

    def query(self, i):
        info = N.EnvInfo()
        N.check(self.lib.mz_query(self._h, int(i), N.C.byref(info)))
        return {k: getattr(info, k) for k, _ in N.EnvInfo._fields_}

    def grid(self, i):
        import numpy as np
        n = self.query(i)["n"]
        g = np.zeros((n, n), np.uint8)
        N.check(self.lib.mz_get_grid(self._h, int(i), g.ctypes.data))
# ... 2 lines not shown
```

Baseline: 1.999 billion.

## Fuse post-step tick, replay push and bank counting into one tail kernel

Adds a step-tail path that merges several per-step kernels into one launch sequence. One kernel updates epsilon, counts wins and episodes, builds the greedy block counts, writes the replay ring rows and fills the per-group bank class counts. It is followed by the greedy list build and a reset kernel that now derives bank slot offsets by scanning the group counts in place, replacing the separate memset and count launches. The aim is fewer launches and less host orchestration per vector step, at the cost of a larger fused kernel and a redundant prefix scan per wave in the reset kernel.

```diff
diff --git a/include/mazerl.h b/include/mazerl.h
--- a/include/mazerl.h
+++ b/include/mazerl.h
@@ -120,6 +120,7 @@
                       uint8_t* grid_host, int32_t* info4_host);
 int mz_bank_use(mz_handle* h, int32_t bank);
 int mz_bank_consumed(mz_handle* h, int32_t bank, int32_t* out3_dev, void* stream);
+int mz_bank_codes(mz_handle* h, int8_t* out_dev, void* stream);
 
 #define MZ_STATE_HEADER_BYTES 256
 int mz_state_bytes(mz_handle* h, uint64_t* bytes_out);
@@ -220,6 +221,14 @@
                    const float* obs6n_src, const int32_t* bitsn_src, float* s6_dev,
                    int32_t* sw_dev, int64_t* a_dev, float* r_dev, float* s6n_dev,
                    int32_t* swn_dev, int32_t obs_dim, int32_t window_words, void* stream);
+
+int mz_step_tail(mz_handle* h, const mz_step_out* out, const int32_t* actions_dev,
+                 float* steps_done_dev, double eps_start, double eps_final, double eps_decay,
+                 float* eps_out_dev, int64_t* wins_dev, int64_t* episodes_dev, uint64_t act_seed,
+                 uint64_t counter, int32_t* scratch_dev, int32_t* rows_dev, int32_t* count_dev,
+                 int64_t capacity, int64_t ptr, int64_t* a_dev, float* r_dev, float* s6n_dev,
+                 int32_t* swn_dev, int32_t obs_dim, int32_t window_words, int32_t regen_won,
+                 uint64_t seed, uint32_t epoch, void* stream);
 
 int mz_replay_sample_idx(uint64_t seed, uint64_t counter, int64_t newest, int64_t n_avail,
                          int64_t capacity, int64_t* out_dev, int32_t n, void* stream);
diff --git a/maze-solving-agent-gymnasium_amd/csrc/mz_api.hip b/maze-solving-agent-gymnasium_amd/csrc/mz_api.hip
--- a/maze-solving-agent-gymnasium_amd/csrc/mz_api.hip
+++ b/maze-solving-agent-gymnasium_amd/csrc/mz_api.hip
@@ -911,6 +911,14 @@
   return MZ_OK;
 }
 
+int mz_bank_codes(mz_handle* h, int8_t* out_dev, void* stream) {
+  if (!h || !h->bank.K || !out_dev) return fail(MZ_EINVAL, "bad arguments");
+  DeviceGuard g(h->cfg.device);
+  MZ_HIP(hipMemcpyAsync(out_dev, h->bank.code, (size_t)h->d.B, hipMemcpyDeviceToDevice,
+                        static_cast<hipStream_t>(stream)));
+  return MZ_OK;
+}
+
 }
 
 namespace {
@@ -1224,6 +1232,41 @@
   return MZ_OK;
 }
 
+int mz_step_tail(mz_handle* h, const mz_step_out* out, const int32_t* actions_dev,
+                 float* steps_done_dev, double eps_start, double eps_final, double eps_decay,
+                 float* eps_out_dev, int64_t* wins_dev, int64_t* episodes_dev, uint64_t act_seed,
+                 uint64_t counter, int32_t* scratch_dev, int32_t* rows_dev, int32_t* count_dev,
+                 int64_t capacity, int64_t ptr, int64_t* a_dev, float* r_dev, float* s6n_dev,
+                 int32_t* swn_dev, int32_t obs_dim, int32_t window_words, int32_t regen_won,
+                 uint64_t seed, uint32_t epoch, void* stream) {
+  if (!h) return fail(MZ_EINVAL, "null handle");
+  if (!out || !out->reward || !out->terminated || !out->truncated || !out->obs6 ||
+      !out->window_bits)
+    return fail(MZ_EINVAL, "the step outputs (reward, terminated, truncated, obs6, window_bits)");
+  int rc = check_out(out);
+  if (rc) return rc;
+  if (!actions_dev || !steps_done_dev || !eps_out_dev || !scratch_dev || !rows_dev || !count_dev)
+    return fail(MZ_EINVAL, "bad arguments");
+  if (!(eps_decay > 0.0)) return fail(MZ_EINVAL, "eps_decay %g", eps_decay);
+  if (!a_dev || !r_dev || !s6n_dev || !swn_dev) return fail(MZ_EINVAL, "replay array missing");
+  if (obs_dim != 6 || window_words != MZ_WINDOW_WORDS)
+    return fail(MZ_EINVAL, "replay rows of %d + %d words, the step writes 6 + %d", obs_dim,
+                window_words, MZ_WINDOW_WORDS);
+  if (capacity < h->d.B || ptr < 0 || ptr >= capacity)
+    return fail(MZ_EINVAL, "replay ring: capacity %lld, ptr %lld for %d rows", (long long)capacity,
+                (long long)ptr, h->d.B);
+  DeviceGuard g(h->cfg.device);
+  MzTail t{steps_done_dev, (float)eps_final, (float)(eps_start - eps_final),
+           1.0f / (float)eps_decay,
+           eps_out_dev, reinterpret_cast<unsigned long long*>(wins_dev),
+           reinterpret_cast<unsigned long long*>(episodes_dev), act_seed, counter, scratch_dev,
+           rows_dev, count_dev, actions_dev, a_dev, r_dev, reinterpret_cast<uint32_t*>(s6n_dev),
+           reinterpret_cast<uint32_t*>(swn_dev), capacity, ptr};
+  MZ_HIP(mz_launch_step_tail(h->d, t, regen_won ? 1 : 0, seed, epoch, to_dev(out),
+                             static_cast<hipStream_t>(stream)));
+  return MZ_OK;
+}
+
 int mz_replay_sample_idx(uint64_t seed, uint64_t counter, int64_t newest, int64_t n_avail,
                          int64_t capacity, int64_t* out_dev, int32_t n, void* stream) {
   if (n < 0 || capacity <= 0 || n_avail <= 0 || n_avail > capacity || (n > 0 && !out_dev))
diff --git a/maze-solving-agent-gymnasium_amd/csrc/mz_env.hip b/maze-solving-agent-gymnasium_amd/csrc/mz_env.hip
--- a/maze-solving-agent-gymnasium_amd/csrc/mz_env.hip
+++ b/maze-solving-agent-gymnasium_amd/csrc/mz_env.hip
@@ -931,7 +931,7 @@
 
 template <bool TOR, bool ENRICH>
 __global__ __launch_bounds__(WAVE) void k_reset_done(MzDev d, int regen, uint64_t seed,
-                                                     uint32_t epoch, MzOut o, int split) {
+                                                     uint32_t epoch, MzOut o, int split, int scan) {
   extern __shared__ __align__(16) uint8_t lds[];
   __shared__ __align__(16) uint32_t wsh[32];
   const int grp = blockIdx.x / split, part = blockIdx.x - grp * split;
@@ -948,7 +948,24 @@
     while (pend) {
       const int cj = __shfl(cls, __ffsll((long long)pend) - 1);
       const unsigned long long m = __ballot(cls == cj);
-      if (cls == cj) slot = d.bk_slot[cj * d.bk_G + grp] + __popcll(m & ((1ull << lane) - 1ull));
+      int first;
+      if (scan) {
+        const int* cnt = d.bk_slot + (size_t)cj * d.bk_G;
+        int pre = 0, tot = 0;
+        for (int i = lane; i < d.bk_G; i += WAVE) {
+          const int v = cnt[i];
+          pre += i < grp ? v : 0;
+          tot += v;
+        }
+        for (int x = WAVE / 2; x; x >>= 1) {
+          pre += __shfl_xor(pre, x);
+          tot += __shfl_xor(tot, x);
+        }
+        first = d.bk_head[cj] - tot + pre;
+      } else {
+        first = d.bk_slot[cj * d.bk_G + grp];
+      }
+      if (cls == cj) slot = first + __popcll(m & ((1ull << lane) - 1ull));
       pend &= ~m;
     }
   }
@@ -1066,6 +1083,93 @@
   if (need) rows[off + __popcll(bal & ((1ull << lane) - 1ull))] = e;
 }
 
+template <int WDS>
+__device__ inline void tail_rows(uint32_t* __restrict__ dst, const uint32_t* __restrict__ src,
+                                 int e0, int nb, int64_t ptr, int64_t cap) {
+  constexpr int U = 8;
+  const int tot = nb * WDS;
+  const uint32_t* sp = src + (size_t)e0 * WDS;
+  for (int i = threadIdx.x; i < tot; i += U * GR_BLOCK) {
+    uint32_t v[U];
+#pragma unroll
+    for (int u = 0; u < U; ++u) v[u] = i + u * GR_BLOCK < tot ? sp[i + u * GR_BLOCK] : 0u;
+#pragma unroll
+    for (int u = 0; u < U; ++u) {
+      const int t = i + u * GR_BLOCK;
+      if (t < tot) {
+        const int r = t / WDS, c = t - r * WDS;
+        int64_t dr = ptr + e0 + r;
+        if (dr >= cap) dr -= cap;
+        dst[dr * WDS + c] = v[u];
+      }
+    }
+  }
+}
+
+__global__ __launch_bounds__(GR_BLOCK) void k_step_tail(MzDev d, MzTail t, MzOut o, int bank) {
+  __shared__ int ws[GR_BLOCK / WAVE], es[GR_BLOCK / WAVE];
+  const int e0 = blockIdx.x * GR_BLOCK, e = e0 + threadIdx.x, n = d.B;
+  const int lane = threadIdx.x & (WAVE - 1), w = threadIdx.x / WAVE;
+  bool need = false, won = false, done = false;
+  if (e < n) {
+    won = o.terminated[e] != 0;
+    done = won || o.truncated[e] != 0;
+    const float sd = won ? 0.0f : t.steps_done[e] + 1.0f;
+    t.steps_done[e] = sd;
+    const float ep = mz_eps_of(sd, t.eps_final, t.eps_span, t.inv_decay);
+    t.eps_out[e] = ep;
+    uint32_t u[4];
+    mz_philox(t.seed, MZ_ACT_STREAM ^ ((uint64_t)e << 32), t.counter, u);
+    need = act_greedy(u, ep);
+    int64_t dr = t.ptr + e;
+    if (dr >= t.cap) dr -= t.cap;
+    t.r_a[dr] = t.act[e];
+    t.r_r[dr] = o.reward[e];
+  }
+  const int c = __syncthreads_count(need);
+  const unsigned long long bw = __ballot(won), bd = __ballot(done);
+  if (lane == 0) {
+    ws[w] = __popcll(bw);
+    es[w] = __popcll(bd);
+  }
+  __syncthreads();
+  if (threadIdx.x == 0) {
+    t.blk[blockIdx.x] = c;
+    int sw = 0, se = 0;
+    for (int i = 0; i < GR_BLOCK / WAVE; ++i) {
+      sw += ws[i];
+      se += es[i];
+    }
+    if (t.wins && sw) atomicAdd(t.wins, (unsigned long long)sw);
+    if (t.episodes && se) atomicAdd(t.episodes, (unsigned long long)se);
+  }
+  const int g = e / WAVE;
+  if (bank && g < d.bk_G) {
+    const bool win = regen_winner(d, e);
+    const int cls = win ? bank_class(d, e) : -1;
+    if (e < n) d.bk_code[e] = (int8_t)(win ? cls : -2);
+    const int ncls = 3 * d.bk_nd;
+    for (int base = 0; base < ncls; base += WAVE) {
+      const int mine = base + lane;
+      int v = 0;
+      unsigned long long pend = __ballot(cls >= base && cls < base + WAVE);
+      while (pend) {
+        const int cj = __shfl(cls, __ffsll((long long)pend) - 1);
+        const unsigned long long m = __ballot(cls == cj);
+        if (mine == cj) v = __popcll(m);
+        pend &= ~m;
+      }
+      if (mine < ncls) {
+        d.bk_slot[(size_t)mine * d.bk_G + g] = v;
+        if (v) atomicAdd(&d.bk_head[mine], v);
+      }
+    }
+  }
+  const int nb = min(GR_BLOCK, n - e0);
+  tail_rows<6>(t.r_s6n, reinterpret_cast<const uint32_t*>(o.obs6), e0, nb, t.ptr, t.cap);
+  tail_rows<MZ_WINDOW_WORDS>(t.r_swn, o.window_bits, e0, nb, t.ptr, t.cap);
+}
+
 __global__ void k_act(MzDev d, MzAct ap) {
   const int e = blockIdx.x * blockDim.x + threadIdx.x;
   if (e >= d.B) return;
@@ -1221,15 +1325,16 @@
   return e;
 }
 
-hipError_t mz_launch_reset_done(const MzDev& d, int regen, uint64_t seed, uint32_t epoch,
-                                const MzOut& o, hipStream_t s) {
+static hipError_t launch_reset_done(const MzDev& d, int regen, uint64_t seed, uint32_t epoch,
+                                    const MzOut& o, hipStream_t s, bool tail) {
   const int groups = (d.B + WAVE - 1) / WAVE;
   int split = 1;
   while (split < WAVE && groups * split < 1024) split <<= 1;
   const int blocks = groups * split;
   size_t lds = 0;
   hipError_t ae = hipSuccess;
-  if (regen && d.bk_K) {
+  const int scan = tail && regen && d.bk_K;
+  if (regen && d.bk_K && !tail) {
     ae = hipMemsetAsync(d.bk_slot, 0, sizeof(int) * 3 * (size_t)d.bk_nd * d.bk_G, s);
     if (ae != hipSuccess) return ae;
     hipLaunchKernelGGL(k_bank_count, dim3(d.bk_G), dim3(WAVE), 0, s, d);
@@ -1243,12 +1348,17 @@
       if (ae != hipSuccess) return ae;                                                        \
     }                                                                                         \
     hipLaunchKernelGGL((k_reset_done<T, E>), dim3(blocks), dim3(WAVE), lds, s, d, regen, seed, \
-                       epoch, o, split);                                                      \
+                       epoch, o, split, scan);                                                \
   } while (0)
   if (d.toroidal) { if (d.enrich) MZ_RD(true, true); else MZ_RD(true, false); }
   else { if (d.enrich) MZ_RD(false, true); else MZ_RD(false, false); }
 #undef MZ_RD
   return hipGetLastError();
+}
+
+hipError_t mz_launch_reset_done(const MzDev& d, int regen, uint64_t seed, uint32_t epoch,
+                                const MzOut& o, hipStream_t s) {
+  return launch_reset_done(d, regen, seed, epoch, o, s, false);
 }
 
 hipError_t mz_launch_cand_build(const MzDev& cd, const int32_t* ids, int base, const int* count, int n,
@@ -1427,3 +1537,15 @@
   hipLaunchKernelGGL(k_expand, dim3((unsigned)((total + 255) / 256)), dim3(256), 0, s, bits, out, n);
   return hipGetLastError();
 }
+
+hipError_t mz_launch_step_tail(const MzDev& d, const MzTail& t, int regen, uint64_t seed,
+                               uint32_t epoch, const MzOut& o, hipStream_t s) {
+  const int blocks = (d.B + GR_BLOCK - 1) / GR_BLOCK;
+  if (blocks == 0) return hipSuccess;
+  const int bank = regen && d.bk_K;
+  hipLaunchKernelGGL(k_step_tail, dim3(blocks), dim3(GR_BLOCK), 0, s, d, t, o, bank);
+  MzAct ap{t.eps_out, 0.0f, nullptr, t.seed, t.counter, nullptr};
+  hipError_t e = mz_launch_greedy_list(ap, d.B, t.blk, t.rows, t.count, nullptr, s);
+  if (e != hipSuccess) return e;
+  return launch_reset_done(d, regen, seed, epoch, o, s, true);
+}
diff --git a/maze-solving-agent-gymnasium_amd/csrc/mz_kernels.h b/maze-solving-agent-gymnasium_amd/csrc/mz_kernels.h
--- a/maze-solving-agent-gymnasium_amd/csrc/mz_kernels.h
+++ b/maze-solving-agent-gymnasium_amd/csrc/mz_kernels.h
@@ -61,3 +61,28 @@
                              hipStream_t s);
 
 constexpr int MZ_GR_BLOCK = 1024;
+
+__device__ inline float mz_eps_of(float sd, float eps_final, float eps_span, float inv_decay) {
+  const float x = __fmul_rn(-sd, inv_decay);
+  return __fadd_rn(eps_final, __fmul_rn(eps_span, expf(x)));
+}
+
+struct MzTail {
+  float* steps_done;
+  float eps_final, eps_span, inv_decay;
+  float* eps_out;
+  unsigned long long* wins;
+  unsigned long long* episodes;
+  uint64_t seed, counter;
+  int32_t* blk;
+  int32_t* rows;
+  int32_t* count;
+  const int32_t* act;
+  int64_t* r_a;
+  float* r_r;
+  uint32_t* r_s6n;
+  uint32_t* r_swn;
+  int64_t cap, ptr;
+};
+hipError_t mz_launch_step_tail(const MzDev& d, const MzTail& t, int regen, uint64_t seed,
+                               uint32_t epoch, const MzOut& o, hipStream_t s);
diff --git a/maze-solving-agent-gymnasium_amd/csrc/mz_trainer.hip b/maze-solving-agent-gymnasium_amd/csrc/mz_trainer.hip
--- a/maze-solving-agent-gymnasium_amd/csrc/mz_trainer.hip
+++ b/maze-solving-agent-gymnasium_amd/csrc/mz_trainer.hip
@@ -9,11 +9,6 @@
 
 constexpr int TB = MZ_GR_BLOCK;
 constexpr int W = 64;
-
-__device__ inline float eps_of(float sd, float eps_final, float eps_span, float inv_decay) {
-  const float x = __fmul_rn(-sd, inv_decay);
-  return __fadd_rn(eps_final, __fmul_rn(eps_span, expf(x)));
-}
 
 __global__ __launch_bounds__(TB) void k_tick_count(const uint8_t* __restrict__ term,
                                                    const uint8_t* __restrict__ trunc,
@@ -32,7 +27,7 @@
     done = won || trunc[e] != 0;
     const float sd = won ? 0.0f : steps_done[e] + 1.0f;
     steps_done[e] = sd;
-    const float ep = eps_of(sd, eps_final, eps_span, inv_decay);
+    const float ep = mz_eps_of(sd, eps_final, eps_span, inv_decay);
     eps_out[e] = ep;
     uint32_t u[4];
     mz_philox(seed, MZ_ACT_STREAM ^ ((uint64_t)e << 32), counter, u);
diff --git a/maze-solving-agent-gymnasium_amd/mazerl/_native.py b/maze-solving-agent-gymnasium_amd/mazerl/_native.py
--- a/maze-solving-agent-gymnasium_amd/mazerl/_native.py
+++ b/maze-solving-agent-gymnasium_amd/mazerl/_native.py
@@ -36,11 +36,11 @@
            "mz_bank_create", "mz_bank_create_dims", "mz_bank_create_ex", "mz_bank_fill", "mz_bank_use",
            "mz_bank_slot_grid", "mz_generate_best", "mz_select_stats", "mz_select_stats_ex",
            "mz_set_debug", "mz_screen_batch", "mz_set_regen_dims",
-           "mz_bank_consumed", "mz_state_bytes", "mz_state_save", "mz_state_load",
+           "mz_bank_consumed", "mz_bank_codes", "mz_state_bytes", "mz_state_save", "mz_state_load",
            "mz_stem_forward", "mz_stem_backward", "mz_stem_backward_ex", "mz_stem_workspace_floats", "mz_adamw_flat",
            "mz_pair_surrogate", "mz_leaky_relu_bf16", "mz_colsum_f32",
            "mz_replay_gather", "mz_host_alloc", "mz_host_free", "mz_q_front_rows", "mz_greedy_rows",
-           "mz_trainer_tick", "mz_greedy_scatter", "mz_head_bf16", "mz_replay_push",
+           "mz_trainer_tick", "mz_greedy_scatter", "mz_head_bf16", "mz_replay_push", "mz_step_tail",
            "mz_replay_sample_idx", "mz_q_loss", "mz_q_loss_backward", "mz_head_loss",
            "mz_head_loss_backward", "mz_head_loss_workspace_floats",
            "mz_head_loss_backward_workspace_floats", "mz_adamw_groups",
@@ -117,6 +117,7 @@
     L.mz_set_regen_dims.argtypes = [vp, vp]
     L.mz_bank_use.argtypes = [vp, C.c_int32]
     L.mz_bank_consumed.argtypes = [vp, C.c_int32, vp, vp]
+    L.mz_bank_codes.argtypes = [vp, vp, vp]
     L.mz_state_bytes.argtypes = [vp, C.POINTER(C.c_uint64)]
     L.mz_state_save.argtypes = [vp, vp, C.c_uint64, vp]
     L.mz_state_load.argtypes = [vp, vp, C.c_uint64, vp]
@@ -132,6 +133,10 @@
     L.mz_head_bf16.argtypes = [vp] * 6 + [C.c_int32] * 9 + [vp] * 7
     L.mz_replay_push.argtypes = [C.c_int32, C.c_int64, C.c_int64] + [vp] * 12 + [C.c_int32,
                                                                                  C.c_int32, vp]
+    L.mz_step_tail.argtypes = [vp, C.POINTER(StepOut), vp, vp, C.c_double, C.c_double, C.c_double,
+                               vp, vp, vp, C.c_uint64, C.c_uint64, vp, vp, vp, C.c_int64,
+                               C.c_int64, vp, vp, vp, vp, C.c_int32, C.c_int32, C.c_int32,
+                               C.c_uint64, C.c_uint32, vp]
     L.mz_replay_sample_idx.argtypes = [C.c_uint64, C.c_uint64, C.c_int64, C.c_int64, C.c_int64,
                                        vp, C.c_int32, vp]
     L.mz_q_loss.argtypes = [vp, C.c_int32, vp, C.c_int32, vp, C.c_int32, vp, vp, C.c_double,
diff --git a/maze-solving-agent-gymnasium_amd/mazerl/agents/dqn.py b/maze-solving-agent-gymnasium_amd/mazerl/agents/dqn.py
--- a/maze-solving-agent-gymnasium_amd/mazerl/agents/dqn.py
+++ b/maze-solving-agent-gymnasium_amd/mazerl/agents/dqn.py
@@ -429,6 +429,18 @@
         return self._rows.tick(term, trunc, self.steps_done, self.eps_start, self.eps_final,
                                self.eps_decay, wins, episodes, seed, counter)
 
+    @property
+    def step_tail_ok(self):
+        return self.fused is not None and bool(self.greedy_rows)
+
+    def step_tail(self, env, regen_won, wins, episodes, seed, counter):
+        assert self.step_tail_ok
+        if self._rows is None:
+            from .fused import GreedyRows
+            self._rows = GreedyRows(self.steps_done.numel(), self.device)
+        return self._rows.step_tail(env, self.replay, regen_won, self.steps_done, self.eps_start,
+                                    self.eps_final, self.eps_decay, wins, episodes, seed, counter)
+
     def prepare_greedy(self, eps, seed, counter):
         if self.fused is None or not self.greedy_rows:
             return
diff --git a/maze-solving-agent-gymnasium_amd/mazerl/agents/fused.py b/maze-solving-agent-gymnasium_amd/mazerl/agents/fused.py
--- a/maze-solving-agent-gymnasium_amd/mazerl/agents/fused.py
+++ b/maze-solving-agent-gymnasium_amd/mazerl/agents/fused.py
@@ -248,6 +248,25 @@
         self._issued = (self.eps.data_ptr(), seed, counter)
         return self.eps
 
+    def step_tail(self, env, replay, regen_won, steps_done, eps_start, eps_final, eps_decay, wins,
+                  episodes, seed, counter):
+        if not hasattr(self, "eps"):
+            self.eps = torch.empty(self.n, dtype=torch.float32, device=self.rows.device)
+        assert steps_done.dtype == torch.float32 and steps_done.is_contiguous()
+        assert steps_done.numel() == self.n == env.num_envs
+        for t in (wins, episodes):
+            assert t is None or (t.dtype == torch.int64 and t.numel() == 1)
+        env.step_tail((steps_done.data_ptr(), float(eps_start), float(eps_final), float(eps_decay),
+                       self.eps.data_ptr(), wins.data_ptr() if wins is not None else None,
+                       episodes.data_ptr() if episodes is not None else None,
+                       seed & 0xFFFFFFFFFFFFFFFF, counter & 0xFFFFFFFFFFFFFFFF,
+                       self.scratch.data_ptr(), self.rows.data_ptr(), self.count.data_ptr()),
+                      replay, regen_won)
+        self.count_host.copy_(self.count, non_blocking=True)
+        self.event.record()
+        self._issued = (self.eps.data_ptr(), seed, counter)
+        return self.eps
+
 
 class FusedActorCritic:
 
diff --git a/maze-solving-agent-gymnasium_amd/mazerl/replay.py b/maze-solving-agent-gymnasium_amd/mazerl/replay.py
--- a/maze-solving-agent-gymnasium_amd/mazerl/replay.py
+++ b/maze-solving-agent-gymnasium_amd/mazerl/replay.py
@@ -87,6 +87,13 @@
     def push_rest(self, a, r, s6n, swn):
         n = a.shape[0]
         self._ring_push(n, a=a, r=r, s6n=s6n, swn=swn)
+        self.pushed(n)
+
+    def tail_args(self):
+        return (self.capacity, self.ptr, self.a.data_ptr(), self.r.data_ptr(), self.s6n.data_ptr(),
+                self.swn.data_ptr(), self.s6.shape[1], self.sw.shape[1])
+
+    def pushed(self, n):
         self.ptr = (self.ptr + n) % self.capacity
         size = min(self.size + n, self.capacity)
         if size != self.size:
diff --git a/maze-solving-agent-gymnasium_amd/mazerl/trainers/vector_trainer.py b/maze-solving-agent-gymnasium_amd/mazerl/trainers/vector_trainer.py
--- a/maze-solving-agent-gymnasium_amd/mazerl/trainers/vector_trainer.py
+++ b/maze-solving-agent-gymnasium_amd/mazerl/trainers/vector_trainer.py
@@ -29,6 +29,7 @@
             self.archive.record(stamp=0)
         self.seed = seed
         self.fused = bool(fused)
+        self.step_tail = self.fused and os.environ.get("MZ_STEP_TAIL", "1") != "0"
         self.regen_won = regen_won
         self.curriculum = rule
         self.allreduce_stats = allreduce_stats
@@ -63,6 +64,21 @@
         env.step_act(eps=eps, greedy=greedy, seed=self.seed, counter=self.counter)
         self.counter += 1
         tick = getattr(L, "tick", None) if self.fused and not self.curriculum else None
+        sch = self.schedule
+        arch = self.archive if self.regen_won else None
+        if self.step_tail and ring and tick is not None and sch is None and \
+                getattr(L, "step_tail_ok", False):
+            if self.track_wins:
+                self.inst_wins += env.terminated.to(torch.int32)
+            if arch is not None:
+                rd = env._regen_dims
+                new_maze = env.terminated.clone() if rd is None else \
+                    (env.terminated.bool() & (rd > 0)).to(torch.uint8)
+            self._eps = L.step_tail(env, self.regen_won, self.wins, self.episodes, self.seed,
+                                    self.counter)
+            if arch is not None:
+                arch.record(new_maze, stamp=self.counter)
+            return L.update(self._expand, reserve=env.num_envs)
         self._eps = tick(env.terminated, env.truncated, self.wins, self.episodes, self.seed,
                          self.counter) if tick is not None else None
         if self._eps is None:
@@ -74,7 +90,6 @@
                 L.prepare_greedy(self._eps, self.seed, self.counter)
             self.wins += term.sum()
             self.episodes += (term | env.truncated.bool()).sum()
-        sch = self.schedule
         if sch is not None:
             won = env.terminated.bool()
             self.inst_wins += won.to(torch.int32)
@@ -85,7 +100,6 @@
             rp.push_rest(env.actions, env.reward, env.obs6, env.window_bits)
         else:
             rp.push(s6, sw, env.actions, env.reward, env.obs6, env.window_bits)
-        arch = self.archive if self.regen_won else None
         if arch is not None:
             rd = env._regen_dims
             new_maze = env.terminated.clone() if rd is None else \
diff --git a/maze-solving-agent-gymnasium_amd/mazerl/vector_env.py b/maze-solving-agent-gymnasium_amd/mazerl/vector_env.py
--- a/maze-solving-agent-gymnasium_amd/mazerl/vector_env.py
+++ b/maze-solving-agent-gymnasium_amd/mazerl/vector_env.py
@@ -239,6 +239,20 @@
             self._bank_tick()
         self._host_sync()
 
+    def step_tail(self, tick_args, replay, regen_won=False):
+        if regen_won:
+            self.epoch += 1
+        sd, e0, e1, ed, eps, wins, episodes, aseed, counter, scratch, rows, count = tick_args
+        N.check(self.lib.mz_step_tail(
+            self._h, N.C.byref(self._out), self._dev_ptr(self.actions), sd, e0, e1, ed, eps, wins,
+            episodes, aseed, counter, scratch, rows, count, *replay.tail_args(),
+            int(bool(regen_won)), self.seed & 0xFFFFFFFFFFFFFFFF, self.epoch & 0xFFFFFFFF,
+            self._stream()))
+        replay.pushed(self.num_envs)
+        if regen_won and self._bank is not None:
+            self._bank_tick()
+        self._host_sync()
+
     def enable_bank(self, slots=None, swap_every=8, algorithms=None, seed=None, dims=None,
                     candidates=1):
         if self._bank is not None:
@@ -300,6 +314,11 @@
         b = self._bank["cur"] if bank is None else int(bank)
         N.check(self.lib.mz_bank_consumed(self._h, b, out.data_ptr(), self._stream()))
         return out if nd == 1 else out.view(3, nd)
+
+    def bank_codes(self):
+        out = torch.empty(self.num_envs, dtype=torch.int8, device=self.device)
+        N.check(self.lib.mz_bank_codes(self._h, out.data_ptr(), self._stream()))
+        return out
 
     _OUTPUTS = ("reward", "reward64", "terminated", "truncated", "pos", "best_dir", "actions",
                 "obs6", "window", "window_bits", "done_idx", "done_count")
diff --git a/profiles/tail_span.py b/profiles/tail_span.py
--- /dev/null
+++ b/profiles/tail_span.py
@@ -0,0 +1,68 @@
+#!/usr/bin/env python3
+import argparse
+import bisect
+import collections
+import csv
+import json
+
+
+def main():
+    ap = argparse.ArgumentParser()
+    ap.add_argument("trace")
+    ap.add_argument("--skip", type=int, default=50)
+    ap.add_argument("--step-kernel", default="k_step<16, false, true, true, false>")
+    ap.add_argument("--end-kernel", default="k_reset_done")
+    a = ap.parse_args()
+    rows = list(csv.DictReader(open(a.trace)))
+    steps = sorted((int(r["Start_Timestamp"]), int(r["End_Timestamp"]), r["Stream_Id"])
+                   for r in rows if a.step_kernel in r["Kernel_Name"])
+    if len(steps) <= a.skip + 1:
+        raise SystemExit("not enough training steps in the trace")
+    sid = collections.Counter(s[2] for s in steps).most_common(1)[0][0]
+    steps = [s for s in steps if s[2] == sid][a.skip:]
+    ks = sorted((int(r["Start_Timestamp"]), int(r["End_Timestamp"]),
+                 r["Kernel_Name"].replace("(anonymous namespace)::", "")) for r in rows
+                if r["Stream_Id"] == sid)
+    starts = [k[0] for k in ks]
+    span = busy = launches = n = 0
+    names = collections.defaultdict(lambda: [0, 0.0])
+    for i, (s0, e0, _) in enumerate(steps[:-1]):
+        nxt = steps[i + 1][0]
+        j = bisect.bisect_right(starts, s0)
+        end, seg = None, []
+        while j < len(ks) and ks[j][0] < nxt:
+            seg.append(ks[j])
+            if a.end_kernel in ks[j][2]:
+                end = ks[j][1]
+                break
+            j += 1
+        if end is None:
+            continue
+        n += 1
+        span += end - e0
+        launches += len(seg)
+        cur = e0
+        for s, e, name in seg:
+            busy += max(0, e - max(s, cur))
+            cur = max(cur, e)
+            key = name[5:] if name.startswith("void ") else name
+            key = key.split("(")[0][:60]
+            names[key][0] += 1
+            names[key][1] += e - s
+    per_step = collections.Counter()
+    for s, e, name in ks:
+        if steps[0][0] <= s < steps[-1][0]:
+            per_step["n"] += 1
+    print(json.dumps({
+        "vector_steps": n, "stream": sid,
+        "us_per_vector_step": (steps[-1][0] - steps[0][0]) / (len(steps) - 1) / 1e3,
+        "stream_launches_per_step": per_step["n"] / (len(steps) - 1),
+        "tail_span_us": span / n / 1e3, "tail_busy_us": busy / n / 1e3,
+        "tail_gap_us": (span - busy) / n / 1e3, "tail_launches": launches / n,
+        "tail_kernels": {k: {"per_step": round(c / n, 3), "us": round(t / max(c, 1) / 1e3, 2)}
+                         for k, (c, t) in sorted(names.items(), key=lambda kv: -kv[1][1])}},
+        indent=1))
+
+
+if __name__ == "__main__":
+    main()
```

New measurement: 1.999 billion. Within noise of the previous version (-0.0%).
